# jcribeiro98/V-GAN

Hardware: AMD Instinct MI355X
Metric: V-GAN train steps/sec (batch=1024, d=784) (higher is better)
Workload: dtype f32; MMD contractions of `value`: split-bf16 x3 on the bf16 MFMA with fp32 accumulation (centred operand); the same step with the fp32 MFMA is timed in `fp32_mode`; 1 GPU; configs[2]: MNIST-pixels-as-features stand-in, d=784, batch=1024 (VGAN_no_kl step); global_batch=1024, features=784, latent=49, rows_per_gpu=1024, parallelism=dp1 (row-sharded Gram, replicated front), hip_graph=True, generator=collapsed, chain_association=depth, mmd_precision=bf16x3, gram_tile=64

## Files before the change

include/vgan_hip.h:

```cpp
#ifndef VGAN_HIP_H
#define VGAN_HIP_H

#include <stdint.h>

#ifdef __cplusplus
extern "C" {
#endif

#define VGAN_OK 0
#define VGAN_ERR_ARG 1
#define VGAN_ERR_HIP 2

#define VGAN_ABI_VERSION 11

typedef void* vgan_stream_t;

int vgan_abi_version(void);
const char* vgan_last_error(void);

int vgan_linear_forward(const float* x, int ldx, int x_nslabs, int64_t x_slab_stride, const float* W,
                        int ldw, const float* b, float* y, int ldy, int n, int in, int out,
                        vgan_stream_t stream);
int vgan_linear_backward_input(const float* dy, int lddy, const float* W, int ldw,
                               float* dx, int lddx, int n, int in, int out, vgan_stream_t stream);
int vgan_linear_backward_params(const float* dy, int lddy, const float* x, int ldx, int x_nslabs,
                                int64_t x_slab_stride, float* dW, int lddw, float* db, int n, int in,
                                int out, int splits, int64_t slab_stride, vgan_stream_t stream);
struct vgan_xx_job;
int vgan_linear_backward_params_xx_supported(int n, int in, int out);
int vgan_linear_backward_params_xx(const float* dy, int lddy, const float* x, int ldx, float* dW, int lddw, int n, int in,
                                   int out, const struct vgan_xx_job* xx, vgan_stream_t stream);
int vgan_reduce_slabs(const float* src, int64_t slab_stride, int nslabs, float* dst, int64_t count,
                      vgan_stream_t stream);

typedef struct vgan_logits_chain {
    const float* za;
    const float* At4;
    int32_t ldza, ldat, e0, pad;
} vgan_logits_chain;
int vgan_mask_project_forward(const float* logits, int ldl, const float* data, int ldd,
                              const int32_t* rows, const uint64_t* row_cursor, int row_batches,
                              int row_stride, int row_offset, float* S, float* U, float* Zx, float* Zy,
                              int ldz, float* sqx, float* sqy, int n, int d, const float* center,
                              int norm_split, const vgan_logits_chain* chain, vgan_stream_t stream);
int vgan_col_mean(const float* data, int ldd, int rows, int d, float* out, vgan_stream_t stream);
int vgan_gather_rows(const float* data, int ldd, const int32_t* rows, const uint64_t* row_cursor,
                     int row_batches, int row_stride, int row_offset, float* out, int ldo,
                     float* sq, int n, int d, vgan_stream_t stream);
int vgan_gather_rows_split(const float* data, int ldd, const int32_t* rows, const uint64_t* row_cursor,
                           int row_batches, int row_stride, int row_offset, const float* center, float* out,
                           int ldo, float* sq, int norm_split, uint16_t* Zh, uint16_t* Zl, int kp, int n, int d,
                           vgan_stream_t stream);
int vgan_mask_backward(const float* gU, int ldg, int nslabs, int64_t slab_stride, const float* S,
                       int lds, const uint64_t* colkey, float pen_weight, int row_offset,
                       float* dlogits, int ldo, int n, int d, vgan_stream_t stream);
int vgan_colmax_chunks(int n);
int vgan_colmax(const float* S, int lds, int from_softmax, int row_offset, uint64_t* part,
                uint64_t* colkey, int n, int d, vgan_stream_t stream);
int vgan_colmax_partial(const float* S, int lds, int from_softmax, int row_offset, uint64_t* part,
                        int n, int d, vgan_stream_t stream);
int vgan_mask_from_softmax(const float* S, int lds, float* U, int ldu, int n, int d, vgan_stream_t stream);
int vgan_upper_softmax_forward(const float* logits, int ldl, float* S, float* U, int n, int d,
                               vgan_stream_t stream);

#define VGAN_TILE 64
#define VGAN_TILE_INTS 8
#define VGAN_TF_SLOT_MASK 3
#define VGAN_TF_TWICE 4
#define VGAN_TF_STORE 8
#define VGAN_TF_MIRROR 16
#define VGAN_TF_NEG 32

int vgan_mmd_build_tiles(int n, int grad_mode, int rank, int world, int tile, int32_t* out, int cap);
int vgan_mmd_order_tiles(int32_t* tiles, int count, int tile);

int vgan_mmd_gram(const float* Z, int ldz, const float* sq, int n, int p, const float* bw,
                  const int32_t* tiles, int ntiles, int calibrate,
                  float* Wg, int ldw, int wrow0, float* partial, vgan_stream_t stream);
#define VGAN_RBF_MAX_KERNELS 8
int vgan_mmd_gram_general(const float* Z, int ldz, const float* sq, int n, int p, const float* bw,
                          const int32_t* tiles, int ntiles, const float* multipliers, int n_kernels,
                          float* Wg, int ldw, int wrow0, float* partial, vgan_stream_t stream);
int vgan_mmd_gram_colmax(const float* Z, int ldz, const float* sq, int n, int p, const float* bw,
                         const int32_t* tiles, int ntiles, float* Wg, int ldw, int wrow0, float* partial,
                         const float* S, int lds, int from_softmax, int row_offset, uint64_t* colpart,
                         int nrows, int d, vgan_stream_t stream);
int vgan_mmd_reduce(const float* partial, const int32_t* tiles, int ntiles, double* stats,
                    int zero_first, vgan_stream_t stream);
int vgan_mmd_set_bandwidth(const double* stats, int n, float* bw, vgan_stream_t stream);
int vgan_mmd_loss(const double* stats, const uint64_t* colkey, int n, int d, float weight,
                  float* loss, float* loss_accum, float accum_scale, uint64_t* step_counter,
                  vgan_stream_t stream);
int vgan_mmd_finalize(const float* partial, const int32_t* tiles, int ntiles, const uint64_t* colpart,
                      int chunks, uint64_t* colkey, int n, int d, float weight, double* stats,
                      float* loss, float* loss_accum, float accum_scale, uint64_t* step_counter,
                      vgan_stream_t stream);
typedef struct vgan_finalize_job {
    const float* partial;
    const int32_t* tiles;
    const uint64_t* colpart;
    uint64_t* colkey;
    double* stats;
    float* loss;
    float* loss_accum;
    uint64_t* step_counter;
    int32_t ntiles, chunks, n, d;
    float weight, accum_scale;
    int32_t mode, ntiles_main;
} vgan_finalize_job;
int vgan_mmd_backward(const float* Wg, int ldw, const float* Z, int ldz, int wrow0, int nr,
                      int ncols, int p, const float* mul, int ldmul, const float* mul_shift, float* out,
                      int ldo, int splits, int64_t slab_stride, const vgan_finalize_job* finalize,
                      vgan_stream_t stream);
int vgan_mmd_bf3_prepare(const float* Z, int ldz, int rows, int p, uint16_t* Zh, uint16_t* Zl, int kp,
                         uint16_t* ZTh, uint16_t* ZTl, int kn, vgan_stream_t stream);
int64_t vgan_mmd_gram_bf3_tail_ws_bytes(void);
int vgan_mmd_gram_bf3(const uint16_t* Zh, const uint16_t* Zl, int kp, const float* sq, int n, const float* bw,
                      const int32_t* tiles, int ntiles, int tile, uint16_t* Wh, uint16_t* Wl, int ldw,
                      int wrow0, float* partial, const float* S, int lds, int from_softmax, int row_offset,
                      uint64_t* colpart, int nrows, int d, void* tail_ws, int64_t tail_ws_bytes,
                      float* rs_part, int ldrs, vgan_stream_t stream);
int vgan_mmd_backward_bf3_tile(int nr, int p, int splits, int tile);
int vgan_mmd_backward_bf3(const uint16_t* Wh, const uint16_t* Wl, int ldw, const uint16_t* ZTh,
                          const uint16_t* ZTl, int kn, int kp, const float* Z, int ldz, int wrow0, int nr,
                          int p, const float* mul, int ldmul, const float* mul_shift, float* out, int ldo,
                          int splits, int64_t slab_stride, int tile, const vgan_finalize_job* finalize,
                          vgan_stream_t stream);
int vgan_mmd_backward_bf3_rm(const uint16_t* Wh, const uint16_t* Wl, int ldw, int kn, const uint16_t* Zh,
                             const uint16_t* Zl, int kp, int zrows, const float* Z, int ldz, int wrow0, int nr,
                             int p, const float* mul, int ldmul, const float* mul_shift, float* out, int ldo,
                             int splits, int64_t slab_stride, int tile, const vgan_finalize_job* finalize,
                             const float* rs_part, int ldrs, vgan_stream_t stream);
int vgan_mmd_backward_bf3_rm_xx(const uint16_t* Wh, const uint16_t* Wl, int ldw, int kn, const uint16_t* Zh,
                                const uint16_t* Zl, int kp, int zrows, const float* Z, int ldz, int wrow0, int nr,
                                int p, const float* mul, int ldmul, const float* mul_shift, float* out, int ldo,
                                int splits, int64_t slab_stride, const vgan_finalize_job* finalize,
                                const struct vgan_xx_job* xx, vgan_stream_t stream);
typedef struct vgan_bwd_rebuild {
    const float* data;
    const int32_t* xrow;
    const float* S;
    const float* center;
    int32_t ldd, lds;
} vgan_bwd_rebuild;
int vgan_mmd_backward_bf3_rm_rebuild(const uint16_t* Wh, const uint16_t* Wl, int ldw, int kn, const uint16_t* Zh,
                                     const uint16_t* Zl, int kp, int zrows, int nr, int p,
                                     const vgan_bwd_rebuild* rebuild, float* out, int ldo, int splits,
                                     int64_t slab_stride, const vgan_finalize_job* finalize,
                                     const struct vgan_xx_job* xx, vgan_stream_t stream);
#define VGAN_GEMM_MAX_GROUP 4
#define VGAN_GEMM_NN 0
#define VGAN_GEMM_NT 1
#define VGAN_GEMM_TN 2
#define VGAN_GEMM_NT_NT 3
typedef struct vgan_gemm_problem {
    const float* a;
    const float* b;
    float* c;
    int32_t kind, m, n, k, lda, ldb, ldc, splitk;
    const float* d;
    float* scratch;
    int32_t ldd, k2;
} vgan_gemm_problem;
int vgan_gemm_grouped(const vgan_gemm_problem* problems, int count, vgan_stream_t stream);
typedef struct vgan_adadelta_layer {
    float* w_packed;
    int64_t off_w, off_b;
    int32_t ldp, out, in, pad;
} vgan_adadelta_layer;
typedef struct vgan_grouped_extras {
    const float* copy_src;
    float* copy_dst;
    int64_t copy_count;
    int32_t adadelta, pad;
    float* p;
    float* sq_avg;
    float* acc_delta;
    float lr, rho, eps, weight_decay, grad_scale;
    int32_t ld_extra;
    vgan_adadelta_layer layer[VGAN_GEMM_MAX_GROUP + 1];
    const float* g_extra;
    float* next_noise;
    int32_t noise_rows, noise_cols, noise_ld, noise_ones_col;
    uint64_t seed;
    const uint64_t* step_counter;
    const vgan_finalize_job* fold;
} vgan_grouped_extras;
int vgan_gemm_grouped_ex(const vgan_gemm_problem* problems, int count, const vgan_grouped_extras* extras,
                         vgan_stream_t stream);

typedef struct vgan_xx_job {
    const uint16_t* Dh;
    const uint16_t* Dl;
    const float* dsq;
    const int32_t* tiles;
    const float* bw;
    float* partial;
    int32_t ldd, ntiles;
} vgan_xx_job;
int vgan_mask_project_forward_bf3(const float* logits, int ldl, const float* data, int ldd, const int32_t* rows,
                                  const uint64_t* row_cursor, int row_batches, int row_stride, float* S, float* Z,
                                  int ldz, float* sq, uint16_t* Zh, uint16_t* Zl, int kp, uint16_t* ZTh,
                                  uint16_t* ZTl, int kn, int n, int d, const float* center, int write_x,
                                  const vgan_xx_job* xx, const vgan_logits_chain* chain, vgan_stream_t stream);
int vgan_mask_project_forward_bf3_ex(const float* logits, int ldl, const float* data, int ldd, const int32_t* rows,
                                     const uint64_t* row_cursor, int row_batches, int row_stride, float* S, float* Z,
                                     int ldz, float* sq, uint16_t* Zh, uint16_t* Zl, int kp, uint16_t* ZTh,
                                     uint16_t* ZTl, int kn, int n, int d, const float* center, int write_x,
                                     const vgan_xx_job* xx, const vgan_logits_chain* chain, int write_z, int32_t* xrow,
                                     vgan_stream_t stream);
int vgan_row_sqnorm(const float* Z, int ldz, float* sq, int rows, int p, vgan_stream_t stream);

int vgan_adadelta_step(float* p, const float* g, int nslabs, int64_t slab_stride, float* sq_avg,
                       float* acc_delta, int64_t count, float lr, float rho, float eps,
                       float weight_decay, float grad_scale, vgan_stream_t stream);

int vgan_noise_normal(float* z, int rows, int cols, int ld, int ones_col, uint64_t seed,
                      const uint64_t* step_counter, uint64_t stream_id, vgan_stream_t stream);

int vgan_homogeneous_pack(const int64_t* desc, int count, int max_elems, int unpack, vgan_stream_t stream);
int vgan_adadelta_step_packed(float* p, const int32_t* pmap, const float* g_packed, float* w_packed,
                              float* sq_avg, float* acc_delta, int64_t count, float lr, float rho,
                              float eps, float weight_decay, float grad_scale, float* next_noise,
                              int noise_rows, int noise_cols, int noise_ld, int noise_ones_col,
                              uint64_t seed, const uint64_t* step_counter, vgan_stream_t stream);

int vgan_mse(const float* a, int lda, const float* b, int ldb, int n, int d, float scale,
             float* out, int accumulate, vgan_stream_t stream);

int vgan_mse_grad(const float* target, int ldt, const float* pred, int ldp, int n, int d, float gscale,
                  double* part, float* g, int ldg, vgan_stream_t stream);
int vgan_sum_f64(const double* in, int count, double scale, float* out, int accumulate, vgan_stream_t stream);

#define VGAN_DP_ID_BYTES 128
typedef struct vgan_dp_comm vgan_dp_comm;
int vgan_dp_unique_id(uint8_t* id );
int vgan_dp_comm_create(vgan_dp_comm** comm, int nranks, const uint8_t* id, int rank);
int vgan_dp_allreduce_sum(vgan_dp_comm* comm, float* buf, int64_t count, vgan_stream_t stream);
int vgan_dp_allgather(vgan_dp_comm* comm, void* buf, int64_t bytes_per_rank, vgan_stream_t stream);
int vgan_dp_comm_destroy(vgan_dp_comm* comm);

int vgan_shuffle_epoch(int32_t* perm, int64_t count, int64_t train_size, uint64_t seed, uint64_t epoch,
                       vgan_stream_t stream);
int64_t vgan_shuffle_index(int64_t i, int64_t train_size, uint64_t seed, uint64_t epoch);
int vgan_mask_unique(const uint8_t* masks, int ldm, int n, int d, uint64_t* keys, int32_t* work,
                     int32_t* out_row, int32_t* out_count, vgan_stream_t stream);

int vgan_rbf_kernel_matrix(const float* Z, int ldz, int m, int p, const float* sq, float alpha, float* K, int ldk,
                           vgan_stream_t stream);
int vgan_rbf_multi_kernel_matrix(const float* Z, int ldz, int m, int p, const float* sq, const float* bw,
                                 const float* multipliers, int n_kernels, float* K, int ldk, float* dK, int lddk,
                                 vgan_stream_t stream);
int vgan_rows_dot(const float* A, int lda, const float* B, int ldb, double* out, int rows, int cols,
                  vgan_stream_t stream);

#define VGAN_OUTLIER_MAX_K 32
#define VGAN_OUTLIER_ENGINE_EXACT 0
#define VGAN_OUTLIER_ENGINE_GRAM 1
#define VGAN_OUTLIER_KNN_LARGEST 0
#define VGAN_OUTLIER_KNN_MEAN 1
#define VGAN_OUTLIER_KNN_MEDIAN 2
#define VGAN_OUTLIER_LRD 3
#define VGAN_OUTLIER_LOF 4
#define VGAN_OUTLIER_KDE_MAX_ROWS 8388607
int vgan_outlier_pack(const float* X, int ldx, int n, int d, const float* center, const int32_t* feat,
                      const int32_t* feat_off, const int64_t* col_off, int first, int count, float* packed, float* sq,
                      vgan_stream_t stream);
int vgan_outlier_knn(const float* Pq, const float* sq_q, int nq, const float* Pr, const float* sq_r, int nr,
                     const int32_t* feat_off, const int64_t* col_off, int first, int count, int k, int exclude_self,
                     int engine, int splits, float* part_d, int32_t* part_i, int32_t* nbr, vgan_stream_t stream);
int vgan_outlier_refine(const float* Xq, int ldq, int nq, const float* Xr, int ldr, int nr, int d, const int32_t* feat,
                        const int32_t* feat_off, int first, int count, const int32_t* nbr, int k, int32_t* out_idx,
                        float* out_dist, float* kdist, vgan_stream_t stream);
int vgan_outlier_score(const int32_t* idx, const float* dist, int nq, int k, int count, int method, const float* kdist_ref,
                       const double* lrd_ref, int nr, float* score, const int32_t* score_row, int ld_score, double* lrd_out,
                       vgan_stream_t stream);
int vgan_outlier_kde(const float* Pq, const float* sq_q, int nq, const float* Pr, const float* sq_r, int nr,
                     const int32_t* feat_off, const int64_t* col_off, int first, int count, const double* bandwidth,
                     int exclude_self, int engine, int splits, uint32_t* pivot, uint64_t* acc, float* score,
                     const int32_t* score_row, int ld_score, vgan_stream_t stream);
int vgan_outlier_combine(const float* score, int ld, int S, int n, const double* weights, double* out,
                         vgan_stream_t stream);
int vgan_outlier_abod(const float* Xq, int ldq, int nq, const float* Xr, int ldr, int nr, int d, const int32_t* feat,
                      const int32_t* feat_off, int first, int count, const int32_t* idx, int k, float* score,
                      const int32_t* score_row, int ld_score, vgan_stream_t stream);
int vgan_outlier_abod_floor(float* score, int ld, int S, int n, int fit, double* score_floor, int32_t* n_degenerate,
                            vgan_stream_t stream);
#define VGAN_OUTLIER_NORM_ZSCORE 1
#define VGAN_OUTLIER_NORM_ROBUST 2
#define VGAN_OUTLIER_NORM_MINMAX 3
#define VGAN_OUTLIER_COMBINE_SUM 0
#define VGAN_OUTLIER_COMBINE_MAX 1
int64_t vgan_outlier_score_stats_ws_bytes(int S, int n, int mode);
int vgan_outlier_score_stats(const float* score, int ld, int S, int n, int mode, double* center, double* scale,
                             void* workspace, int64_t workspace_bytes, vgan_stream_t stream);
int vgan_outlier_combine_normalized(const float* score, int ld, int S, int n, const double* center, const double* scale,
                                    const double* weights, int combination, double* out, vgan_stream_t stream);

#define VGAN_CLUSTER_MAX_CLUSTERS 64
#define VGAN_CLUSTER_SLICE_ROWS 1024
int64_t vgan_cluster_lloyd_ws_bytes(int n, int n_clusters, int count, int total_dims);
int vgan_cluster_image(const double* centers, int n_clusters, const int32_t* feat, const int32_t* feat_off,
                       const int64_t* col_off, int first, int count, const float* col_center, float* img, float* img_sq,
                       vgan_stream_t stream);
int vgan_cluster_lloyd(const float* Pq, const float* sq_q, const float* X, int ldx, int n, int d, const int32_t* feat,
                       const int32_t* feat_off, const int64_t* col_off, int first, int count, int total_dims, int max_dims,
                       int n_clusters, int engine, const float* col_center, const double* tol_var, double* centers,
                       float* img, float* img_sq, int32_t* label, int32_t* changed, int32_t* done, int32_t* n_iter,
                       void* workspace, int64_t workspace_bytes, int iterations, vgan_stream_t stream);
int vgan_cluster_final(const float* Xq, int ldq, int nq, int d, const int32_t* feat, const int32_t* feat_off, int S,
                       int n_clusters, const double* centers, const int32_t* large, int64_t* sizes, int use_weights,
                       int32_t* label, double* inertia_part, double* inertia, float* score, const int32_t* score_row,
                       int ld_score, vgan_stream_t stream);

#ifdef __cplusplus
}
#endif
#endif
```

v-gan_amd/csrc/gemm_core.hpp:

```cpp
#pragma once
#include <type_traits>

#include "vgan_common.hpp"

namespace vgan {

enum : int { KC = 0, MC = 1 };

constexpr int kPad = 4;

typedef __attribute__((address_space(3))) float lds_f;
typedef __attribute__((address_space(3))) f32x4 lds_f4;

template <int BMN, int BK, int LAYOUT, int VEC, bool SL = false, int NTH = kBlock>
struct Stager;

template <int BMN, int BK, bool SL, int NTH>
struct Stager<BMN, BK, KC, 4, SL, NTH> {
    int nslabs = 1;
    long slab_stride = 0;
    static constexpr int NV = BMN * BK / 4 / NTH;
    static_assert(NV >= 1, "tile too small");
    float4 v[NV];
    const float* rowp[NV];
    int lofs[NV];
    bool rowok[NV], ok[NV];
    int kq4, K;
    __device__ __forceinline__ void init(const float* __restrict__ p, long ld, int mn0, int MN, int K_, int tid) {
        K = K_;
        kq4 = 4 * (tid % (BK / 4));
#pragma unroll
        for (int r = 0; r < NV; ++r) {
            const int m = (tid + NTH * r) / (BK / 4);
            rowok[r] = mn0 + m < MN;
            rowp[r] = p + (long)min(mn0 + m, MN - 1) * ld;
            lofs[r] = m * (BK + kPad) + kq4;
        }
    }
    __device__ __forceinline__ void load(int k0) {
        const int k = k0 + kq4;
        const int kc = min(k, K - 4);
#pragma unroll
        for (int r = 0; r < NV; ++r) {
            ok[r] = rowok[r] && (k < K);
            v[r] = *reinterpret_cast<const float4*>(rowp[r] + kc);
            if constexpr (SL)
                for (int sl = 1; sl < nslabs; ++sl) {
                    const float4 t = *reinterpret_cast<const float4*>(rowp[r] + sl * slab_stride + kc);
                    v[r].x += t.x; v[r].y += t.y; v[r].z += t.z; v[r].w += t.w;
                }
        }
    }
    __device__ __forceinline__ void store(lds_f* lds) {
#pragma unroll
        for (int r = 0; r < NV; ++r) {
            if (!ok[r]) v[r] = make_float4(0.f, 0.f, 0.f, 0.f);
            *(lds_f4*)(lds + lofs[r]) = f32x4{v[r].x, v[r].y, v[r].z, v[r].w};
        }
    }
    typedef float4 Side;
    __device__ __forceinline__ void side_add(Side (&s)[NV]) const {
#pragma unroll
        for (int r = 0; r < NV; ++r) { s[r].x += v[r].x; s[r].y += v[r].y; s[r].z += v[r].z; s[r].w += v[r].w; }
    }
    __device__ static __forceinline__ void side_reduce(const Side (&s)[NV], lds_f* , lds_f* out, int tid) {
#pragma unroll
        for (int r = 0; r < NV; ++r) {
            float t = (s[r].x + s[r].y) + (s[r].z + s[r].w);
#pragma unroll
            for (int o = 1; o < BK / 4; o <<= 1) t += __shfl_xor(t, o, 64);
            int f = tid + NTH * r;
            if (f % (BK / 4) == 0) out[f / (BK / 4)] = t;
        }
    }
};

template <int BMN, int BK, bool SL, int NTH>
struct Stager<BMN, BK, KC, 1, SL, NTH> {
    int nslabs = 1;
    long slab_stride = 0;
    static constexpr int NV = BMN * BK / NTH;
    float v[NV];
    const float* rowp[NV];
    int lofs[NV];
    bool rowok[NV], ok[NV];
    int kk, K;
    __device__ __forceinline__ void init(const float* __restrict__ p, long ld, int mn0, int MN, int K_, int tid) {
        K = K_;
        kk = tid % BK;
#pragma unroll
        for (int r = 0; r < NV; ++r) {
            const int m = (tid + NTH * r) / BK;
            rowok[r] = mn0 + m < MN;
            rowp[r] = p + (long)min(mn0 + m, MN - 1) * ld;
            lofs[r] = m * (BK + kPad) + kk;
        }
    }
    __device__ __forceinline__ void load(int k0) {
        const int k = k0 + kk;
        const int kc = min(k, K - 1);
#pragma unroll
        for (int r = 0; r < NV; ++r) {
            ok[r] = rowok[r] && (k < K);
            v[r] = rowp[r][kc];
            if constexpr (SL)
                for (int sl = 1; sl < nslabs; ++sl) v[r] += rowp[r][sl * slab_stride + kc];
        }
    }
    __device__ __forceinline__ void store(lds_f* lds) {
#pragma unroll
        for (int r = 0; r < NV; ++r) {
            if (!ok[r]) v[r] = 0.f;
            lds[lofs[r]] = v[r];
        }
    }
    typedef float Side;
    __device__ __forceinline__ void side_add(Side (&s)[NV]) const {
#pragma unroll
        for (int r = 0; r < NV; ++r) s[r] += v[r];
    }
    __device__ static __forceinline__ void side_reduce(const Side (&s)[NV], lds_f* , lds_f* out, int tid) {
#pragma unroll
        for (int r = 0; r < NV; ++r) {
            float t = s[r];
#pragma unroll
            for (int o = 1; o < BK; o <<= 1) t += __shfl_xor(t, o, 64);
            int f = tid + NTH * r;
            if (f % BK == 0) out[f / BK] = t;
        }
    }
};

template <int BMN, int BK, bool SL, int NTH>
struct Stager<BMN, BK, MC, 4, SL, NTH> {
    int nslabs = 1;
    long slab_stride = 0;
    static constexpr int NV = BMN * BK / 4 / NTH;
    static_assert(NV >= 1, "tile too small");
    static_assert(NTH % (BMN / 4) == 0, "mq must be fixed per thread");
    float4 v[NV];
    const float* colp;
    long ld;
    int krow[NV], lofs[NV];
    bool colok, ok[NV];
    int K;
    __device__ __forceinline__ void init(const float* __restrict__ p, long ld_, int mn0, int MN, int K_, int tid) {
        K = K_;
        ld = ld_;
        const int m = mn0 + 4 * (tid % (BMN / 4));
        colok = m < MN;
        colp = p + min(m, MN - 4);
#pragma unroll
        for (int r = 0; r < NV; ++r) {
            krow[r] = (tid + NTH * r) / (BMN / 4);
            lofs[r] = krow[r] * (BMN + kPad) + 4 * (tid % (BMN / 4));
        }
    }
    __device__ __forceinline__ void load(int k0) {
#pragma unroll
        for (int r = 0; r < NV; ++r) {
            const int k = k0 + krow[r];
            ok[r] = colok && (k < K);
            v[r] = *reinterpret_cast<const float4*>(colp + (long)min(k, K - 1) * ld);
            if constexpr (SL)
                for (int sl = 1; sl < nslabs; ++sl) {
                    const float4 t = *reinterpret_cast<const float4*>(colp + sl * slab_stride + (long)min(k, K - 1) * ld);
                    v[r].x += t.x; v[r].y += t.y; v[r].z += t.z; v[r].w += t.w;
                }
        }
    }
    __device__ __forceinline__ void store(lds_f* lds) {
#pragma unroll
        for (int r = 0; r < NV; ++r) {
            if (!ok[r]) v[r] = make_float4(0.f, 0.f, 0.f, 0.f);
            *(lds_f4*)(lds + lofs[r]) = f32x4{v[r].x, v[r].y, v[r].z, v[r].w};
        }
    }
    typedef float4 Side;
    __device__ __forceinline__ void side_add(Side (&s)[NV]) const {
#pragma unroll
        for (int r = 0; r < NV; ++r) { s[r].x += v[r].x; s[r].y += v[r].y; s[r].z += v[r].z; s[r].w += v[r].w; }
    }
    __device__ static __forceinline__ void side_reduce(const Side (&s)[NV], lds_f* scratch, lds_f* out, int tid) {
        constexpr int ROWS = NTH / (BMN / 4);
        float4 t = s[0];
#pragma unroll
        for (int r = 1; r < NV; ++r) { t.x += s[r].x; t.y += s[r].y; t.z += s[r].z; t.w += s[r].w; }
        *(lds_f4*)(scratch + (tid / (BMN / 4)) * BMN + 4 * (tid % (BMN / 4))) = f32x4{t.x, t.y, t.z, t.w};
        __syncthreads();
        if (tid < BMN) {
            float a = 0.f;
#pragma unroll
            for (int q = 0; q < ROWS; ++q) a += scratch[q * BMN + tid];
            out[tid] = a;
        }
    }
};

template <int BMN, int BK, bool SL, int NTH>
struct Stager<BMN, BK, MC, 1, SL, NTH> {
    int nslabs = 1;
    long slab_stride = 0;
    static constexpr int NV = BMN * BK / NTH;
    static_assert(NTH % BMN == 0, "m must be fixed per thread");
    float v[NV];
    const float* colp;
    long ld;
    int krow[NV], lofs[NV];
    bool colok, ok[NV];
    int K;
    __device__ __forceinline__ void init(const float* __restrict__ p, long ld_, int mn0, int MN, int K_, int tid) {
        K = K_;
        ld = ld_;
        const int m = mn0 + tid % BMN;
        colok = m < MN;
        colp = p + min(m, MN - 1);
#pragma unroll
        for (int r = 0; r < NV; ++r) {
            krow[r] = (tid + NTH * r) / BMN;
            lofs[r] = krow[r] * (BMN + kPad) + tid % BMN;
        }
    }
    __device__ __forceinline__ void load(int k0) {
#pragma unroll
        for (int r = 0; r < NV; ++r) {
            const int k = k0 + krow[r];
            ok[r] = colok && (k < K);
            v[r] = colp[(long)min(k, K - 1) * ld];
            if constexpr (SL)
                for (int sl = 1; sl < nslabs; ++sl) v[r] += colp[sl * slab_stride + (long)min(k, K - 1) * ld];
        }
    }
    __device__ __forceinline__ void store(lds_f* lds) {
#pragma unroll
        for (int r = 0; r < NV; ++r) {
            if (!ok[r]) v[r] = 0.f;
            lds[lofs[r]] = v[r];
        }
    }
    typedef float Side;
    __device__ __forceinline__ void side_add(Side (&s)[NV]) const {
#pragma unroll
        for (int r = 0; r < NV; ++r) s[r] += v[r];
    }
    __device__ static __forceinline__ void side_reduce(const Side (&s)[NV], lds_f* scratch, lds_f* out, int tid) {
        constexpr int ROWS = NTH / BMN;
        float t = s[0];
#pragma unroll
        for (int r = 1; r < NV; ++r) t += s[r];
        scratch[(tid / BMN) * BMN + (tid % BMN)] = t;
        __syncthreads();
        if (tid < BMN) {
            float a = 0.f;
#pragma unroll
            for (int q = 0; q < ROWS; ++q) a += scratch[q * BMN + tid];
            out[tid] = a;
        }
    }
};

template <int BM, int BN, int BK, int LA, int LB, int VEC, int SLABS = 0, int KW = 1>
struct GemmTile {
    static constexpr int NTH = kBlock * KW;
    static constexpr int WM = BM / 64, WN = BN / 64;
    static_assert(KW == 1 || (KW == 2 && BM == 64 && BN == 64 && (BK / 8) % 2 == 0), "K-split needs one sub-tile per wave");
    static constexpr int kImgA = (LA == KC) ? BM * (BK + kPad) : BK * (BM + kPad);
    static constexpr int kImgB = (LB == KC) ? BN * (BK + kPad) : BK * (BN + kPad);
    static constexpr int kLdsFloats = 2 * (kImgA + kImgB);
    static_assert(BM % 64 == 0 && BN % 64 == 0 && BK % 8 == 0, "tile shape");

    template <int LAYOUT, int BMN>
    __device__ static __forceinline__ f32x4 frag(const lds_f* img, int mn, int c, int fh) {
        if constexpr (LAYOUT == KC) {
            return *(const lds_f4*)(img + mn * (BK + kPad) + 8 * c + 4 * fh);
        } else {
            const lds_f* q = img + (8 * c + 4 * fh) * (BMN + kPad) + mn;
            return f32x4{q[0], q[BMN + kPad], q[2 * (BMN + kPad)], q[3 * (BMN + kPad)]};
        }
    }

    template <bool SIDE_A>
    __device__ static __forceinline__ void run(const float* __restrict__ A, long lda, const float* __restrict__ B, long ldb,
                                               int m0, int n0, int M, int N, int K, float* lds_generic, float* side_generic,
                                               f32x16 (&acc)[WM][WN], int nslabs = 1, long slab_stride = 0) {
        lds_f* lds = (lds_f*)lds_generic;
        lds_f* side_lds = (lds_f*)side_generic;
        const int tid = threadIdx.x;
        const int lane = tid & 63, wave = (tid >> 6) & 3, kp = tid >> 8;
        const int wm0 = (wave >> 1) * (BM / 2), wn0 = (wave & 1) * (BN / 2);
        const int fi = lane & 31, fh = lane >> 5;
        lds_f* const sA0 = lds;
        lds_f* const sB0 = lds + 2 * kImgA;
        constexpr int GC = BK / 8 / KW;

        using SG = Stager<BM, BK, LA, VEC, (SLABS & 1) != 0, NTH>;
        SG ga;
        Stager<BN, BK, LB, VEC, (SLABS & 2) != 0, NTH> gb;
        ga.init(A, lda, m0, M, K, tid);
        gb.init(B, ldb, n0, N, K, tid);
        if constexpr (SLABS & 1) { ga.nslabs = nslabs; ga.slab_stride = slab_stride; }
        if constexpr (SLABS & 2) { gb.nslabs = nslabs; gb.slab_stride = slab_stride; }
        typename SG::Side side[SG::NV];
        if constexpr (SIDE_A) {
#pragma unroll
            for (int r = 0; r < SG::NV; ++r) side[r] = typename SG::Side{};
        }

        const int nk = (K + BK - 1) / BK;
        ga.load(0);
        gb.load(0);
        ga.store(sA0);
        gb.store(sB0);
        if constexpr (SIDE_A) ga.side_add(side);
        if (nk > 1) {
            ga.load(BK);
            gb.load(BK);
        }
        __syncthreads();

        auto body = [&](int kt, auto store_next, auto load_next2) {
            const int cur = kt & 1;
            const lds_f* imgA = sA0 + cur * kImgA;
            const lds_f* imgB = sB0 + cur * kImgB;
            f32x4 a[GC][WM], b[GC][WN];
#pragma unroll
            for (int c = 0; c < GC; ++c) {
#pragma unroll
                for (int i = 0; i < WM; ++i) a[c][i] = frag<LA, BM>(imgA, wm0 + i * 32 + fi, kp * GC + c, fh);
#pragma unroll
                for (int j = 0; j < WN; ++j) b[c][j] = frag<LB, BN>(imgB, wn0 + j * 32 + fi, kp * GC + c, fh);
            }
#ifndef VGAN_ABLATE_NO_LDS_STORE
            if constexpr (decltype(store_next)::value) {
                ga.store(sA0 + (cur ^ 1) * kImgA);
                gb.store(sB0 + (cur ^ 1) * kImgB);
                if constexpr (SIDE_A) ga.side_add(side);
            }
#endif
#ifndef VGAN_ABLATE_NO_GLOBAL
            if constexpr (decltype(load_next2)::value) {
                ga.load((kt + 2) * BK);
                gb.load((kt + 2) * BK);
            }
#endif
#pragma unroll
            for (int c = 0; c < GC; ++c)
#pragma unroll
                for (int st = 0; st < 4; ++st)
#pragma unroll
                    for (int i = 0; i < WM; ++i)
#pragma unroll
                        for (int j = 0; j < WN; ++j)
#ifndef VGAN_ABLATE_NO_MFMA
                            acc[i][j] = __builtin_amdgcn_mfma_f32_32x32x2f32(a[c][i][st], b[c][j][st], acc[i][j], 0, 0, 0);
#else
                            acc[i][j][st] += a[c][i][st] * b[c][j][st];
#endif
#if !defined(VGAN_SCHED_NONE)
            __builtin_amdgcn_iglp_opt(0);
#endif
#ifndef VGAN_ABLATE_NO_BARRIER
            __syncthreads();
#endif
        };
        using T = std::true_type;
        using F = std::false_type;
        int kt = 0;
        for (; kt + 2 < nk; ++kt) body(kt, T{}, T{});
        if (kt + 1 < nk) {
            body(kt, T{}, F{});
            ++kt;
        }
        body(kt, F{}, F{});

        if constexpr (SIDE_A) {
            SG::side_reduce(side, lds, side_lds, tid);
            __syncthreads();
        }
        if constexpr (KW == 2) {
            lds_f* xch = lds;
#pragma unroll
            for (int r = 0; r < 8; ++r) xch[((kp * 4 + wave) * 8 + r) * 64 + lane] = acc[0][0][8 * (1 - kp) + r];
            __syncthreads();
#pragma unroll
            for (int r = 0; r < 8; ++r) acc[0][0][8 * kp + r] += xch[(((1 - kp) * 4 + wave) * 8 + r) * 64 + lane];
            __syncthreads();
        }
    }
    __device__ static __forceinline__ int first_reg() { return KW == 2 ? 8 * (threadIdx.x >> 8) : 0; }
    static constexpr int kNumRegs = 16 / KW;

    __device__ static __forceinline__ int sub_row(int wm, int r) {
        const int lane = threadIdx.x & 63, wave = (threadIdx.x >> 6) & 3;
        return (wave >> 1) * (BM / 2) + wm * 32 + (r & 3) + 8 * (r >> 2) + 4 * (lane >> 5);
    }
    __device__ static __forceinline__ int sub_col(int wn) {
        const int lane = threadIdx.x & 63, wave = (threadIdx.x >> 6) & 3;
        return (wave & 1) * (BN / 2) + wn * 32 + (lane & 31);
    }
};


template <int BK, int LA, int LB, int VEC, int NW = 4>
struct GemmTileKS {
    static constexpr int T = 32;
    static constexpr int NTH = 64 * NW;
    static constexpr int NR = 16 / NW;
    static constexpr int kImgA = (LA == KC) ? T * (BK + kPad) : BK * (T + kPad);
    static constexpr int kImgB = (LB == KC) ? T * (BK + kPad) : BK * (T + kPad);
    static constexpr int kLdsFloats = 2 * (kImgA + kImgB);
    static constexpr int GW = BK / (8 * NW);
    static_assert(GW >= 1 && BK % (8 * NW) == 0 && kLdsFloats >= NW * 16 * 64, "K tile / reduction scratch");

    template <int LAYOUT>
    __device__ static __forceinline__ f32x4 frag(const lds_f* img, int mn, int c, int fh) {
        if constexpr (LAYOUT == KC) {
            return *(const lds_f4*)(img + mn * (BK + kPad) + 8 * c + 4 * fh);
        } else {
            const lds_f* q = img + (8 * c + 4 * fh) * (T + kPad) + mn;
            return f32x4{q[0], q[T + kPad], q[2 * (T + kPad)], q[3 * (T + kPad)]};
        }
    }

    __device__ static __forceinline__ void run(const float* __restrict__ A, long lda, const float* __restrict__ B, long ldb, int m0,
                                               int n0, int M, int N, int K, float* lds_generic, float (&out)[NR]) {
        lds_f* lds = (lds_f*)lds_generic;
        const int tid = threadIdx.x, lane = tid & 63, wave = tid >> 6;
        const int fi = lane & 31, fh = lane >> 5;
        lds_f* const sA0 = lds;
        lds_f* const sB0 = lds + 2 * kImgA;
        f32x16 acc;
#pragma unroll
        for (int r = 0; r < 16; ++r) acc[r] = 0.f;
        const int nk = (K + BK - 1) / BK;
        Stager<T, BK, LA, VEC, false, NTH> ga;
        Stager<T, BK, LB, VEC, false, NTH> gb;
        ga.init(A, lda, m0, M, K, tid);
        gb.init(B, ldb, n0, N, K, tid);
        ga.load(0);
        gb.load(0);
        ga.store(sA0);
        gb.store(sB0);
        if (nk > 1) {
            ga.load(BK);
            gb.load(BK);
        }
        __syncthreads();
        auto body = [&](int kt, auto store_next, auto load_next2) {
            const int cur = kt & 1;
            const lds_f* imgA = sA0 + cur * kImgA;
            const lds_f* imgB = sB0 + cur * kImgB;
            f32x4 a[GW], b[GW];
#pragma unroll
            for (int c = 0; c < GW; ++c) {
                a[c] = frag<LA>(imgA, fi, wave * GW + c, fh);
                b[c] = frag<LB>(imgB, fi, wave * GW + c, fh);
            }
            if constexpr (decltype(store_next)::value) {
                ga.store(sA0 + (cur ^ 1) * kImgA);
                gb.store(sB0 + (cur ^ 1) * kImgB);
            }
            if constexpr (decltype(load_next2)::value) {
                ga.load((kt + 2) * BK);
                gb.load((kt + 2) * BK);
            }
#pragma unroll
            for (int c = 0; c < GW; ++c)
#pragma unroll
                for (int st = 0; st < 4; ++st) acc = __builtin_amdgcn_mfma_f32_32x32x2f32(a[c][st], b[c][st], acc, 0, 0, 0);
            __builtin_amdgcn_iglp_opt(0);
            __syncthreads();
        };
        using Tt = std::true_type;
        using Ff = std::false_type;
        int kt = 0;
        for (; kt + 2 < nk; ++kt) body(kt, Tt{}, Tt{});
        if (kt + 1 < nk) {
            body(kt, Tt{}, Ff{});
            ++kt;
        }
        body(kt, Ff{}, Ff{});
#pragma unroll
        for (int r = 0; r < 16; ++r) lds[(wave * 16 + r) * 64 + lane] = acc[r];
        __syncthreads();
#pragma unroll
        for (int rr = 0; rr < NR; ++rr) {
            const int r = NR * wave + rr;
            if constexpr (NW == 4) {
                out[rr] = (lds[(0 * 16 + r) * 64 + lane] + lds[(1 * 16 + r) * 64 + lane]) +
                          (lds[(2 * 16 + r) * 64 + lane] + lds[(3 * 16 + r) * 64 + lane]);
            } else {
                float q[NW / 4];
#pragma unroll
                for (int w4 = 0; w4 < NW / 4; ++w4)
                    q[w4] = (lds[((4 * w4 + 0) * 16 + r) * 64 + lane] + lds[((4 * w4 + 1) * 16 + r) * 64 + lane]) +
                            (lds[((4 * w4 + 2) * 16 + r) * 64 + lane] + lds[((4 * w4 + 3) * 16 + r) * 64 + lane]);
                float t = q[0];
#pragma unroll
                for (int w4 = 1; w4 < NW / 4; ++w4) t += q[w4];
                out[rr] = t;
            }
        }
    }
    __device__ static __forceinline__ int row_of(int rr) {
        const int lane = threadIdx.x & 63, r = NR * (threadIdx.x >> 6) + rr;
        return (r & 3) + 8 * (r >> 2) + 4 * (lane >> 5);
    }
    __device__ static __forceinline__ int col_of() { return threadIdx.x & 31; }
};

template <int WM, int WN>
__device__ __forceinline__ void zero_acc(f32x16 (&acc)[WM][WN]) {
#pragma unroll
    for (int i = 0; i < WM; ++i)
#pragma unroll
        for (int j = 0; j < WN; ++j)
#pragma unroll
            for (int r = 0; r < 16; ++r) acc[i][j][r] = 0.f;
}

}
```

v-gan_amd/csrc/grouped.hip:

```cpp
#include "gemm_core.hpp"
#include "mmd_common.hpp"
#include "optim_common.hpp"

namespace vgan {

constexpr int QBM = 64, QBK = 32, QKS = 128;

struct GroupedArgs {
    vgan_gemm_problem p[VGAN_GEMM_MAX_GROUP];
    int tile_start[VGAN_GEMM_MAX_GROUP + 1];
    int ks[VGAN_GEMM_MAX_GROUP];
    int split[VGAN_GEMM_MAX_GROUP];
    int kchunk[VGAN_GEMM_MAX_GROUP];
    int count;
};

__device__ __forceinline__ vgan_gemm_problem k_slice(vgan_gemm_problem q, int slice, int kchunk) {
    const int k0 = slice * kchunk;
    q.c += (long)slice * q.m * q.ldc;
    if (q.kind == VGAN_GEMM_NN) { q.a += k0; q.b += (long)k0 * q.ldb; }
    else if (q.kind == VGAN_GEMM_NT) { q.a += k0; q.b += k0; }
    else { q.a += (long)k0 * q.lda; q.b += (long)k0 * q.ldb; }
    q.k = min(kchunk, q.k - k0);
    return q;
}

struct GroupedExtras {
    const float* copy_src;
    float* copy_dst;
    long copy_count;
    int copy_blocks, extra_blocks, noise_blocks, adadelta;
    float *p, *sq, *acc;
    float lr, rho, eps, wd, gs;
    vgan_adadelta_layer layer[VGAN_GEMM_MAX_GROUP + 1];
    const float* g_extra;
    int ld_extra;
    float* z;
    int zrows, zcols, zld, zones;
    unsigned long long seed;
    const unsigned long long* step_counter;
    int fold_blocks;
    vgan_finalize_job fold;
};

__device__ __forceinline__ void adadelta_packed_element(const GroupedExtras& x, const vgan_adadelta_layer& L, int row, int col, float g) {
    if (row >= L.out || col > L.in) return;
    const long idx = col < L.in ? L.off_w + (long)row * L.in + col : L.off_b + row;
    float pv = x.p[idx], v = x.sq[idx], a = x.acc[idx];
    adadelta_one(pv, g, v, a, x.lr, x.rho, x.eps, x.wd, x.gs);
    x.p[idx] = pv;
    x.sq[idx] = v;
    x.acc[idx] = a;
    L.w_packed[(long)row * L.ldp + col] = pv;
}

template <int NE>
struct AdadeltaTile {
    long idx[NE];
    float pv[NE], v[NE], a[NE];
    bool ok[NE];
    template <typename RowOf>
    __device__ __forceinline__ void prefetch(const GroupedExtras& x, const vgan_adadelta_layer& L, int col, RowOf row_of) {
#pragma unroll
        for (int r = 0; r < NE; ++r) {
            const int row = row_of(r);
            ok[r] = row < L.out && col <= L.in;
            idx[r] = ok[r] ? (col < L.in ? L.off_w + (long)row * L.in + col : L.off_b + row) : L.off_w;
            pv[r] = x.p[idx[r]];
            v[r] = x.sq[idx[r]];
            a[r] = x.acc[idx[r]];
        }
    }
    template <typename RowOf>
    __device__ __forceinline__ void finish(const GroupedExtras& x, const vgan_adadelta_layer& L, int col, const float (&g)[NE], RowOf row_of) {
#pragma unroll
        for (int r = 0; r < NE; ++r) adadelta_one(pv[r], g[r], v[r], a[r], x.lr, x.rho, x.eps, x.wd, x.gs);
#pragma unroll
        for (int r = 0; r < NE; ++r)
            if (ok[r]) {
                x.p[idx[r]] = pv[r];
                x.sq[idx[r]] = v[r];
                x.acc[idx[r]] = a[r];
                L.w_packed[(long)row_of(r) * L.ldp + col] = pv[r];
            }
    }
};

__device__ __forceinline__ void grouped_extra_jobs(const GroupedExtras& x, int b, int layer_index) {
    if (b < x.copy_blocks) {
        for (long i = (long)b * blockDim.x + threadIdx.x; i < x.copy_count; i += (long)x.copy_blocks * blockDim.x) x.copy_dst[i] = x.copy_src[i];
        return;
    }
    b -= x.copy_blocks;
    if (b < x.extra_blocks) {
        const vgan_adadelta_layer& L = x.layer[layer_index];
        const long total = (long)L.out * (L.in + 1);
        for (long i = (long)b * blockDim.x + threadIdx.x; i < total; i += (long)x.extra_blocks * blockDim.x) {
            const int row = (int)(i / (L.in + 1)), col = (int)(i % (L.in + 1));
            adadelta_packed_element(x, L, row, col, x.g_extra[(long)row * x.ld_extra + col]);
        }
        return;
    }
    b -= x.extra_blocks;
    if (b < x.noise_blocks) {
        noise_normal_body(x.z, x.zrows, x.zcols, x.zld, x.zones, x.seed, x.step_counter, 0ull, b, x.noise_blocks);
        return;
    }
    b -= x.noise_blocks;
    if (b < x.fold_blocks) finalize_body(x.fold);
}

template <int LA, int LB, int VEC, bool EPI>
__device__ __forceinline__ void tile64(const vgan_gemm_problem& q, int t, float* lds, const GroupedExtras& x, int qi) {
    using G = GemmTile<QBM, QBM, QBK, LA, LB, VEC>;
    const int gx = (q.n + QBM - 1) / QBM;
    const int m0 = (t / gx) * QBM, n0 = (t % gx) * QBM;
    const int col = n0 + G::sub_col(0);
    auto row_of = [&](int r) { return m0 + G::sub_row(0, r); };
    AdadeltaTile<EPI ? 16 : 1> upd;
    if constexpr (EPI) upd.prefetch(x, x.layer[qi], col, row_of);
    f32x16 acc[1][1];
    zero_acc(acc);
    G::template run<false>(q.a, q.lda, q.b, q.ldb, m0, n0, q.m, q.n, q.k, lds, nullptr, acc);
#pragma unroll
    for (int r = 0; r < 16; ++r) {
        const int row = m0 + G::sub_row(0, r);
        if (row < q.m && col < q.n) q.c[(long)row * q.ldc + col] = acc[0][0][r];
    }
    if constexpr (EPI) {
        float g[16];
#pragma unroll
        for (int r = 0; r < 16; ++r) g[r] = acc[0][0][r];
        upd.finish(x, x.layer[qi], col, g, row_of);
    }
}

template <int LA, int LB, int VEC, int NW = 4, bool EPI = false>
__device__ __forceinline__ void tile_ks(const vgan_gemm_problem& q, int t, float* lds, const GroupedExtras& x, int qi) {
    using G = GemmTileKS<QKS, LA, LB, VEC, NW>;
    const int gx = (q.n + 31) / 32;
    const int m0 = (t / gx) * 32, n0 = (t % gx) * 32;
    const int col = n0 + G::col_of();
    auto row_of = [&](int rr) { return m0 + G::row_of(rr); };
    AdadeltaTile<EPI ? G::NR : 1> upd;
    if constexpr (EPI) upd.prefetch(x, x.layer[qi], col, row_of);
    float o[G::NR];
    G::run(q.a, q.lda, q.b, q.ldb, m0, n0, q.m, q.n, q.k, lds, o);
#pragma unroll
    for (int rr = 0; rr < G::NR; ++rr) {
        const int row = m0 + G::row_of(rr);
        if (row < q.m && col < q.n) q.c[(long)row * q.ldc + col] = o[rr];
    }
    if constexpr (EPI) upd.finish(x, x.layer[qi], col, o, row_of);
}

template <int VEC>
__device__ __forceinline__ void tile64_two_stage(const vgan_gemm_problem& q, int t, float* lds) {
    using G = GemmTile<QBM, QBM, QBK, KC, KC, VEC>;
    const int gx = (q.n + QBM - 1) / QBM;
    const int m0 = (t / gx) * QBM, n0 = (t % gx) * QBM;
    const int ldh = (q.k2 + 3) / 4 * 4;
    float* H = q.scratch + (long)t * QBM * ldh;
    const int rows = min(QBM, q.m - m0);
    for (int c0 = 0; c0 < q.k2; c0 += QBM) {
        f32x16 acc[1][1];
        zero_acc(acc);
        G::template run<false>(q.a, q.lda, q.b, q.ldb, m0, c0, q.m, q.k2, q.k, lds, nullptr, acc);
        const int col = c0 + G::sub_col(0);
#pragma unroll
        for (int r = 0; r < 16; ++r) {
            const int row = G::sub_row(0, r);
            if (row < rows && col < ldh) H[(long)row * ldh + col] = col < q.k2 ? acc[0][0][r] : 0.f;
        }
    }
    __syncthreads();
    f32x16 acc[1][1];
    zero_acc(acc);
    G::template run<false>(H, ldh, q.d, q.ldd, 0, n0, rows, q.n, q.k2, lds, nullptr, acc);
    const int col = n0 + G::sub_col(0);
#pragma unroll
    for (int r = 0; r < 16; ++r) {
        const int row = m0 + G::sub_row(0, r);
        if (row < q.m && col < q.n) q.c[(long)row * q.ldc + col] = acc[0][0][r];
    }
}

constexpr int cmax(int a, int b) { return a > b ? a : b; }

template <int VEC, bool EPI>
__global__ __launch_bounds__(kBlock, 2) void gemm_grouped_kernel(GroupedArgs g, GroupedExtras x) {
    constexpr int kLds = cmax(cmax(GemmTile<QBM, QBM, QBK, KC, MC, VEC>::kLdsFloats, GemmTile<QBM, QBM, QBK, MC, MC, VEC>::kLdsFloats),
                              cmax(cmax(GemmTileKS<QKS, KC, MC, VEC>::kLdsFloats, GemmTileKS<QKS, MC, MC, VEC>::kLdsFloats),
                                   cmax(GemmTile<QBM, QBM, QBK, KC, KC, VEC>::kLdsFloats, GemmTileKS<QKS, KC, KC, VEC>::kLdsFloats)));
    __shared__ __attribute__((aligned(16))) float lds[kLds];
    if ((int)blockIdx.x >= g.tile_start[VGAN_GEMM_MAX_GROUP]) {
        grouped_extra_jobs(x, blockIdx.x - g.tile_start[VGAN_GEMM_MAX_GROUP], g.count);
        return;
    }
    int qi = 0;
#pragma unroll
    for (int i = 1; i < VGAN_GEMM_MAX_GROUP; ++i)
        if (i < g.count && (int)blockIdx.x >= g.tile_start[i]) qi = i;
    vgan_gemm_problem q = g.p[qi];
    int t = blockIdx.x - g.tile_start[qi];
    if (g.split[qi] > 1) {
        const int per = (g.tile_start[qi + 1] - g.tile_start[qi]) / g.split[qi];
        q = k_slice(q, t / per, g.kchunk[qi]);
        t %= per;
    }
    if (q.kind == VGAN_GEMM_NN) {
        if (g.ks[qi]) tile_ks<KC, MC, VEC, 4, EPI>(q, t, lds, x, qi); else tile64<KC, MC, VEC, EPI>(q, t, lds, x, qi);
    } else if (q.kind == VGAN_GEMM_NT) {
        if (g.ks[qi]) tile_ks<KC, KC, VEC, 4, EPI>(q, t, lds, x, qi); else tile64<KC, KC, VEC, EPI>(q, t, lds, x, qi);
    } else if (q.kind == VGAN_GEMM_NT_NT) {
        tile64_two_stage<VEC>(q, t, lds);
    } else {
        if (g.ks[qi]) tile_ks<MC, MC, VEC, 4, EPI>(q, t, lds, x, qi); else tile64<MC, MC, VEC, EPI>(q, t, lds, x, qi);
    }
}

__global__ __launch_bounds__(1024, 1) void gemm_grouped_ks16_kernel(GroupedArgs g, GroupedExtras x) {
    constexpr int kLds = cmax(cmax(GemmTileKS<QKS, KC, MC, 4, 16>::kLdsFloats, GemmTileKS<QKS, MC, MC, 4, 16>::kLdsFloats),
                              GemmTileKS<QKS, KC, KC, 4, 16>::kLdsFloats);
    __shared__ __attribute__((aligned(16))) float lds[kLds];
    if ((int)blockIdx.x >= g.tile_start[VGAN_GEMM_MAX_GROUP]) {
        grouped_extra_jobs(x, blockIdx.x - g.tile_start[VGAN_GEMM_MAX_GROUP], g.count);
        return;
    }
    int qi = 0;
#pragma unroll
    for (int i = 1; i < VGAN_GEMM_MAX_GROUP; ++i)
        if (i < g.count && (int)blockIdx.x >= g.tile_start[i]) qi = i;
    const vgan_gemm_problem& q = g.p[qi];
    const int t = blockIdx.x - g.tile_start[qi];
    if (q.kind == VGAN_GEMM_NN) tile_ks<KC, MC, 4, 16>(q, t, lds, x, qi);
    else if (q.kind == VGAN_GEMM_NT) tile_ks<KC, KC, 4, 16>(q, t, lds, x, qi);
    else tile_ks<MC, MC, 4, 16>(q, t, lds, x, qi);
}

}

using namespace vgan;

static inline int extra_grid(long work_items) {
    long g = (work_items + kBlock - 1) / kBlock;
    return (int)(g < 1 ? 1 : (g > 256 ? 256 : g));
}

extern "C" int vgan_gemm_grouped_ex(const vgan_gemm_problem* problems, int count, const vgan_grouped_extras* extras,
                                    vgan_stream_t stream) {
    VGAN_CHECK_ARG(problems && count >= 1 && count <= VGAN_GEMM_MAX_GROUP);
    GroupedArgs g{};
    GroupedExtras x{};
    g.count = count;
    bool vec = true, any_split = false;
    int tiles = 0;
    for (int i = 0; i < count; ++i) {
        const vgan_gemm_problem& q = problems[i];
        VGAN_CHECK_ARG(q.a && q.b && q.c && q.m > 0 && q.n > 0 && q.k > 0 && q.ldc >= q.n);
        VGAN_CHECK_ARG(q.kind == VGAN_GEMM_NN || q.kind == VGAN_GEMM_NT || q.kind == VGAN_GEMM_TN || q.kind == VGAN_GEMM_NT_NT);
        const bool two = q.kind == VGAN_GEMM_NT_NT;
        VGAN_CHECK_ARG(q.lda >= (q.kind == VGAN_GEMM_TN ? q.m : q.k) && q.ldb >= ((q.kind == VGAN_GEMM_NT || two) ? q.k : q.n));
        if (two) {
            VGAN_CHECK_ARG(q.d && q.scratch && q.k2 > 0 && q.ldd >= q.k2 && q.splitk <= 1 && aligned16(q.scratch));
            vec = vec && (q.k2 % 4 == 0) && (q.ldd % 4 == 0) && aligned16(q.d);
            any_split = true;
        }
        vec = vec && (q.m % 4 == 0) && (q.n % 4 == 0) && (q.k % 4 == 0) && (q.lda % 4 == 0) && (q.ldb % 4 == 0) && aligned16(q.a) &&
              aligned16(q.b);
        const long t64 = (long)((q.m + 63) / 64) * ((q.n + 63) / 64);
        const long t32 = (long)((q.m + 31) / 32) * ((q.n + 31) / 32);
        g.ks[i] = (q.k >= 128 && t32 <= 512 && !two) ? 1 : 0;
        g.p[i] = q;
        g.tile_start[i] = tiles;
        g.split[i] = q.splitk > 1 ? q.splitk : 1;
        if (g.split[i] > 1) {
            g.kchunk[i] = ((q.k + g.split[i] - 1) / g.split[i] + QBK - 1) / QBK * QBK;
            VGAN_CHECK_ARG(g.split[i] <= 64 && (long)(g.split[i] - 1) * g.kchunk[i] < q.k);
            g.ks[i] = 0;
            any_split = true;
        }
        tiles += g.ks[i] ? ((q.m + 31) / 32) * ((q.n + 31) / 32) : (int)t64 * g.split[i];
    }
    for (int i = count; i <= VGAN_GEMM_MAX_GROUP; ++i) g.tile_start[i] = tiles;
    bool epi = false;
    if (extras != nullptr) {
        const vgan_grouped_extras& e = *extras;
        if (e.copy_src != nullptr) {
            VGAN_CHECK_ARG(e.copy_dst && e.copy_count > 0);
            x.copy_src = e.copy_src;
            x.copy_dst = e.copy_dst;
            x.copy_count = (long)e.copy_count;
            x.copy_blocks = extra_grid(e.copy_count);
        }
        if (e.adadelta) {
            VGAN_CHECK_ARG(e.p && e.sq_avg && e.acc_delta && !any_split);
            epi = true;
            x.adadelta = 1;
            x.p = e.p; x.sq = e.sq_avg; x.acc = e.acc_delta;
            x.lr = e.lr; x.rho = e.rho; x.eps = e.eps; x.wd = e.weight_decay; x.gs = e.grad_scale;
            const int nl = count + (e.g_extra != nullptr ? 1 : 0);
            for (int i = 0; i < nl; ++i) {
                const vgan_adadelta_layer& L = e.layer[i];
                VGAN_CHECK_ARG(L.w_packed && L.out > 0 && L.in > 0 && L.ldp >= L.in + 1 && L.off_w >= 0 && L.off_b >= 0);
                if (i < count) VGAN_CHECK_ARG(problems[i].m >= L.out && problems[i].n >= L.in + 1);
                x.layer[i] = L;
            }
            if (e.g_extra != nullptr) {
                VGAN_CHECK_ARG(e.ld_extra >= e.layer[count].in + 1);
                x.g_extra = e.g_extra;
                x.ld_extra = e.ld_extra;
                x.extra_blocks = extra_grid((long)e.layer[count].out * (e.layer[count].in + 1));
            }
        }
        if (e.next_noise != nullptr) {
            VGAN_CHECK_ARG(e.noise_rows > 0 && e.noise_cols > 0 && e.noise_ld >= e.noise_cols && e.noise_ones_col < e.noise_ld);
            x.z = e.next_noise;
            x.zrows = e.noise_rows; x.zcols = e.noise_cols; x.zld = e.noise_ld; x.zones = e.noise_ones_col;
            x.seed = (unsigned long long)e.seed;
            x.step_counter = reinterpret_cast<const unsigned long long*>(e.step_counter);
            x.noise_blocks = extra_grid(((long)e.noise_rows * e.noise_cols + 3) / 4);
        }
        if (e.fold != nullptr) {
            VGAN_CHECK_ARG(finalize_job_ok(*e.fold));
            x.fold = *e.fold;
            x.fold_blocks = 1;
        }
    }
    const int surplus = x.copy_blocks + x.extra_blocks + x.noise_blocks + x.fold_blocks;
    int kmin = problems[0].k, t32 = 0;
    for (int i = 0; i < count; ++i) {
        kmin = problems[i].k < kmin ? problems[i].k : kmin;
        t32 += ((problems[i].m + 31) / 32) * ((problems[i].n + 31) / 32);
    }
    if (vec && kmin >= 96 && t32 <= 256 && !epi && x.noise_blocks == 0 && !any_split) {
        int acc = 0;
        for (int i = 0; i < count; ++i) {
            g.ks[i] = 1;
            g.tile_start[i] = acc;
            acc += ((problems[i].m + 31) / 32) * ((problems[i].n + 31) / 32);
        }
        for (int i = count; i <= VGAN_GEMM_MAX_GROUP; ++i) g.tile_start[i] = acc;
        hipLaunchKernelGGL(gemm_grouped_ks16_kernel, dim3(acc + surplus), dim3(1024), 0, (hipStream_t)stream, g, x);
        VGAN_CHECK_LAUNCH();
        return VGAN_OK;
    }
    const dim3 grid(tiles + surplus), block(kBlock);
    hipStream_t st = (hipStream_t)stream;
    if (vec && epi) hipLaunchKernelGGL((gemm_grouped_kernel<4, true>), grid, block, 0, st, g, x);
    else if (vec) hipLaunchKernelGGL((gemm_grouped_kernel<4, false>), grid, block, 0, st, g, x);
    else if (epi) hipLaunchKernelGGL((gemm_grouped_kernel<1, true>), grid, block, 0, st, g, x);
    else hipLaunchKernelGGL((gemm_grouped_kernel<1, false>), grid, block, 0, st, g, x);
    VGAN_CHECK_LAUNCH();
    return VGAN_OK;
}

extern "C" int vgan_gemm_grouped(const vgan_gemm_problem* problems, int count, vgan_stream_t stream) {
    return vgan_gemm_grouped_ex(problems, count, nullptr, stream);
}
```

v-gan_amd/csrc/linear.hip:

```cpp
#include "gemm_core.hpp"
#include "mmd_xx.hpp"

namespace vgan {

constexpr int LBM = 64, LBN = 64, LBK = 32;

template <int VEC, bool XSL>
__global__ __launch_bounds__(kBlock, 2) void linear_fwd_kernel(const float* __restrict__ x, int ldx, const float* __restrict__ W,
                                                              int ldw, const float* __restrict__ b, float* __restrict__ y,
                                                              int ldy, int n, int in, int out, int x_nslabs, long x_slab_stride) {
    using G = GemmTile<LBM, LBN, LBK, KC, KC, VEC, XSL ? 1 : 0>;
    __shared__ __attribute__((aligned(16))) float lds[G::kLdsFloats];
    const int m0 = blockIdx.y * LBM, n0 = blockIdx.x * LBN;
    const int col = n0 + G::sub_col(0);
    const float bias = (b != nullptr) ? b[min(col, out - 1)] : 0.f;
    f32x16 acc[G::WM][G::WN];
    zero_acc(acc);
    G::template run<false>(x, ldx, W, ldw, m0, n0, n, out, in, lds, nullptr, acc, x_nslabs, x_slab_stride);
#pragma unroll
    for (int r = 0; r < 16; ++r) {
        const int row = m0 + G::sub_row(0, r);
        if (row < n && col < out) y[(long)row * ldy + col] = acc[0][0][r] + bias;
    }
}

template <int VEC>
__global__ __launch_bounds__(kBlock, 2) void linear_bwd_input_kernel(const float* __restrict__ dy, int lddy,
                                                                    const float* __restrict__ W, int ldw, float* __restrict__ dx,
                                                                    int lddx, int n, int in, int out) {
    using G = GemmTile<LBM, LBN, LBK, KC, MC, VEC>;
    __shared__ __attribute__((aligned(16))) float lds[G::kLdsFloats];
    const int m0 = blockIdx.y * LBM, n0 = blockIdx.x * LBN;
    f32x16 acc[G::WM][G::WN];
    zero_acc(acc);
    G::template run<false>(dy, lddy, W, ldw, m0, n0, n, in, out, lds, nullptr, acc);
    const int col = n0 + G::sub_col(0);
#pragma unroll
    for (int r = 0; r < 16; ++r) {
        const int row = m0 + G::sub_row(0, r);
        if (row < n && col < in) dx[(long)row * lddx + col] = acc[0][0][r];
    }
}

template <int VEC, bool XSL>
__global__ __launch_bounds__(kBlock, 2) void linear_bwd_params_kernel(const float* __restrict__ dy, int lddy,
                                                                     const float* __restrict__ x, int ldx, float* __restrict__ dW,
                                                                     int lddw, float* __restrict__ db, int n, int in, int out,
                                                                     int kchunk, long slab_stride, int x_nslabs, long x_slab_stride) {
    using G = GemmTile<LBM, LBN, LBK, MC, MC, VEC, XSL ? 2 : 0>;
    __shared__ __attribute__((aligned(16))) float lds[G::kLdsFloats];
    __shared__ float side[LBM];
    const int m0 = blockIdx.y * LBM, n0 = blockIdx.x * LBN;
    const int k0 = blockIdx.z * kchunk;
    const int klen = min(kchunk, n - k0);
    dy += (long)k0 * lddy;
    x += (long)k0 * ldx;
    dW += blockIdx.z * slab_stride;
    if (db != nullptr) db += blockIdx.z * slab_stride;
    n = klen;
    f32x16 acc[G::WM][G::WN];
    zero_acc(acc);
    const bool do_bias = (db != nullptr) && (blockIdx.x == 0);
    if (klen <= 0) {
        if (threadIdx.x < LBM) side[threadIdx.x] = 0.f;
        __syncthreads();
    } else if (do_bias)
        G::template run<true>(dy, lddy, x, ldx, m0, n0, out, in, n, lds, side, acc, x_nslabs, x_slab_stride);
    else
        G::template run<false>(dy, lddy, x, ldx, m0, n0, out, in, n, lds, side, acc, x_nslabs, x_slab_stride);
    const int col = n0 + G::sub_col(0);
#pragma unroll
    for (int r = 0; r < 16; ++r) {
        const int row = m0 + G::sub_row(0, r);
        if (row < out && col < in) dW[(long)row * lddw + col] = acc[0][0][r];
    }
    if (do_bias && threadIdx.x < LBM && m0 + threadIdx.x < out) db[m0 + threadIdx.x] = side[threadIdx.x];
}

constexpr int KSBK = 128;
template <int VEC, int NW>
__global__ __launch_bounds__(64 * NW, NW == 4 ? 2 : 1) void linear_fwd_ks_kernel(const float* __restrict__ x, int ldx,
                                                                               const float* __restrict__ W, int ldw,
                                                                               const float* __restrict__ b, float* __restrict__ y,
                                                                               int ldy, int n, int in, int out) {
    using G = GemmTileKS<KSBK, KC, KC, VEC, NW>;
    __shared__ __attribute__((aligned(16))) float lds[G::kLdsFloats];
    const int m0 = blockIdx.y * 32, n0 = blockIdx.x * 32;
    const int col = n0 + G::col_of();
    const float bias = (b != nullptr) ? b[min(col, out - 1)] : 0.f;
    float o[G::NR];
    G::run(x, ldx, W, ldw, m0, n0, n, out, in, lds, o);
#pragma unroll
    for (int rr = 0; rr < G::NR; ++rr) {
        const int row = m0 + G::row_of(rr);
        if (row < n && col < out) y[(long)row * ldy + col] = o[rr] + bias;
    }
}
template <int VEC>
__global__ __launch_bounds__(kBlock, 2) void linear_bwd_input_ks_kernel(const float* __restrict__ dy, int lddy,
                                                                       const float* __restrict__ W, int ldw, float* __restrict__ dx,
                                                                       int lddx, int n, int in, int out, int in_staged) {
    using G = GemmTileKS<KSBK, KC, MC, VEC>;
    __shared__ __attribute__((aligned(16))) float lds[G::kLdsFloats];
    const int m0 = blockIdx.y * 32, n0 = blockIdx.x * 32;
    float o[G::NR];
    G::run(dy, lddy, W, ldw, m0, n0, n, in_staged, out, lds, o);
    const int col = n0 + G::col_of();
#pragma unroll
    for (int rr = 0; rr < G::NR; ++rr) {
        const int row = m0 + G::row_of(rr);
        if (row < n && col < in) dx[(long)row * lddx + col] = o[rr];
    }
}
template <int VEC, int NW>
__global__ __launch_bounds__(64 * NW, NW == 4 ? 2 : 1) void linear_bwd_params_ks_kernel(const float* __restrict__ dy, int lddy,
                                                                                      const float* __restrict__ x, int ldx,
                                                                                      float* __restrict__ dW, int lddw, int n, int in,
                                                                                      int out) {
    using G = GemmTileKS<KSBK, MC, MC, VEC, NW>;
    __shared__ __attribute__((aligned(16))) float lds[G::kLdsFloats];
    const int m0 = blockIdx.y * 32, n0 = blockIdx.x * 32;
    float o[G::NR];
    G::run(dy, lddy, x, ldx, m0, n0, out, in, n, lds, o);
    const int col = n0 + G::col_of();
#pragma unroll
    for (int rr = 0; rr < G::NR; ++rr) {
        const int row = m0 + G::row_of(rr);
        if (row < out && col < in) dW[(long)row * lddw + col] = o[rr];
    }
}
__global__ __launch_bounds__(1024, 1) void linear_bwd_params_ks_xx_kernel(const float* __restrict__ dy, int lddy, const float* __restrict__ x,
                                                                         int ldx, float* __restrict__ dW, int lddw, int n, int in, int out,
                                                                         int gx, int ptiles, XXJob xx) {
    using G = GemmTileKS<KSBK, MC, MC, 4, 16>;
    constexpr int kBytes = G::kLdsFloats * 4 > GemmBF3<64>::kLdsBytes ? G::kLdsFloats * 4 : GemmBF3<64>::kLdsBytes;
    __shared__ __attribute__((aligned(16))) char raw[kBytes];
    __shared__ float xx_red[4];
    if ((int)blockIdx.x >= ptiles) {
        xx_tile_body(xx, blockIdx.x - ptiles, raw, xx_red);
        return;
    }
    float* lds = reinterpret_cast<float*>(raw);
    const int m0 = (blockIdx.x / gx) * 32, n0 = (blockIdx.x % gx) * 32;
    float o[G::NR];
    G::run(dy, lddy, x, ldx, m0, n0, out, in, n, lds, o);
    const int col = n0 + G::col_of();
#pragma unroll
    for (int rr = 0; rr < G::NR; ++rr) {
        const int row = m0 + G::row_of(rr);
        if (row < out && col < in) dW[(long)row * lddw + col] = o[rr];
    }
}

static inline bool use_ks(int rows, int cols, int k) {
    const long tiles64 = (long)((rows + 63) / 64) * ((cols + 63) / 64);
    return tiles64 <= 32 && k >= 128;
}

static inline bool use_ks_params(int rows, int cols, int k) {
    const long tiles64 = (long)((rows + 63) / 64) * ((cols + 63) / 64);
    return use_ks(rows, cols, k) || (tiles64 <= 512 && k >= 2048);
}

static inline dim3 grid_for(int rows, int cols) { return dim3((cols + LBN - 1) / LBN, (rows + LBM - 1) / LBM, 1); }

}

using namespace vgan;

extern "C" int vgan_linear_forward(const float* x, int ldx, int x_nslabs, int64_t x_slab_stride, const float* W, int ldw,
                                   const float* b, float* y, int ldy, int n, int in, int out, vgan_stream_t stream) {
    VGAN_CHECK_ARG(x && W && y && n > 0 && in > 0 && out > 0 && ldx >= in && ldw >= in && ldy >= out && x_nslabs >= 1);
    hipStream_t s = (hipStream_t)stream;
    const bool vec = (in % 4 == 0) && (ldx % 4 == 0) && (ldw % 4 == 0) && aligned16(x) && aligned16(W) && (x_slab_stride % 4 == 0);
    const long xs = (long)x_slab_stride;
    if (x_nslabs == 1 && use_ks(n, out, in)) {
        dim3 g((out + 31) / 32, (n + 31) / 32);
        if (vec && in >= 512)
            hipLaunchKernelGGL((linear_fwd_ks_kernel<4, 16>), g, dim3(1024), 0, s, x, ldx, W, ldw, b, y, ldy, n, in, out);
        else if (vec)
            hipLaunchKernelGGL((linear_fwd_ks_kernel<4, 4>), g, dim3(kBlock), 0, s, x, ldx, W, ldw, b, y, ldy, n, in, out);
        else
            hipLaunchKernelGGL((linear_fwd_ks_kernel<1, 4>), g, dim3(kBlock), 0, s, x, ldx, W, ldw, b, y, ldy, n, in, out);
        VGAN_CHECK_LAUNCH();
        return VGAN_OK;
    }
#define VGAN_FWD(V, S) hipLaunchKernelGGL((linear_fwd_kernel<V, S>), grid_for(n, out), dim3(kBlock), 0, s, x, ldx, W, ldw, b, y, ldy, n, in, out, x_nslabs, xs)
    if (x_nslabs > 1) { if (vec) VGAN_FWD(4, true); else VGAN_FWD(1, true); }
    else { if (vec) VGAN_FWD(4, false); else VGAN_FWD(1, false); }
#undef VGAN_FWD
    VGAN_CHECK_LAUNCH();
    return VGAN_OK;
}

extern "C" int vgan_linear_backward_input(const float* dy, int lddy, const float* W, int ldw, float* dx, int lddx, int n, int in,
                                          int out, vgan_stream_t stream) {
    VGAN_CHECK_ARG(dy && W && dx && n > 0 && in > 0 && out > 0 && lddy >= out && ldw >= in && lddx >= in);
    hipStream_t s = (hipStream_t)stream;
    const bool vec_but_in = (out % 4 == 0) && (lddy % 4 == 0) && (ldw % 4 == 0) && aligned16(dy) && aligned16(W);
    const bool vec = vec_but_in && (in % 4 == 0);
    if (use_ks(n, in, out)) {
        dim3 g((in + 31) / 32, (n + 31) / 32);
        const int in4 = (in + 3) / 4 * 4;
        if (vec_but_in && ldw >= in4)
            hipLaunchKernelGGL(linear_bwd_input_ks_kernel<4>, g, dim3(kBlock), 0, s, dy, lddy, W, ldw, dx, lddx, n, in, out, in4);
        else
            hipLaunchKernelGGL(linear_bwd_input_ks_kernel<1>, g, dim3(kBlock), 0, s, dy, lddy, W, ldw, dx, lddx, n, in, out, in);
    } else if (vec)
        hipLaunchKernelGGL(linear_bwd_input_kernel<4>, grid_for(n, in), dim3(kBlock), 0, s, dy, lddy, W, ldw, dx, lddx, n, in, out);
    else
        hipLaunchKernelGGL(linear_bwd_input_kernel<1>, grid_for(n, in), dim3(kBlock), 0, s, dy, lddy, W, ldw, dx, lddx, n, in, out);
    VGAN_CHECK_LAUNCH();
    return VGAN_OK;
}

extern "C" int vgan_linear_backward_params(const float* dy, int lddy, const float* x, int ldx, int x_nslabs, int64_t x_slab_stride,
                                           float* dW, int lddw, float* db, int n, int in, int out, int splits, int64_t slab_stride,
                                           vgan_stream_t stream) {
    VGAN_CHECK_ARG(dy && x && dW && n > 0 && in > 0 && out > 0 && lddy >= out && ldx >= in && lddw >= in && x_nslabs >= 1);
    VGAN_CHECK_ARG(splits >= 1 && splits <= 64 && (splits == 1 || slab_stride > 0));
    hipStream_t s = (hipStream_t)stream;
    int kchunk = (n + splits - 1) / splits;
    kchunk = (kchunk + 3) / 4 * 4;
    const int nz = (n + kchunk - 1) / kchunk;
    const bool vec = (out % 4 == 0) && (lddy % 4 == 0) && (in % 4 == 0) && (ldx % 4 == 0) && aligned16(dy) && aligned16(x) &&
                     (x_slab_stride % 4 == 0);
    dim3 grid = grid_for(out, in);
    grid.z = splits;
    (void)nz;
    const long xs = (long)x_slab_stride;
    if (splits == 1 && x_nslabs == 1 && db == nullptr && use_ks_params(out, in, n)) {
        dim3 g((in + 31) / 32, (out + 31) / 32);
        if (vec && n >= 256)
            hipLaunchKernelGGL((linear_bwd_params_ks_kernel<4, 16>), g, dim3(1024), 0, s, dy, lddy, x, ldx, dW, lddw, n, in, out);
        else if (vec)
            hipLaunchKernelGGL((linear_bwd_params_ks_kernel<4, 4>), g, dim3(kBlock), 0, s, dy, lddy, x, ldx, dW, lddw, n, in, out);
        else
            hipLaunchKernelGGL((linear_bwd_params_ks_kernel<1, 4>), g, dim3(kBlock), 0, s, dy, lddy, x, ldx, dW, lddw, n, in, out);
        VGAN_CHECK_LAUNCH();
        return VGAN_OK;
    }
#define VGAN_BWP(V, S) hipLaunchKernelGGL((linear_bwd_params_kernel<V, S>), grid, dim3(kBlock), 0, s, dy, lddy, x, ldx, dW, lddw, db, n, in, out, kchunk, (long)slab_stride, x_nslabs, xs)
    if (x_nslabs > 1) { if (vec) VGAN_BWP(4, true); else VGAN_BWP(1, true); }
    else { if (vec) VGAN_BWP(4, false); else VGAN_BWP(1, false); }
#undef VGAN_BWP
    VGAN_CHECK_LAUNCH();
    return VGAN_OK;
}

extern "C" int vgan_linear_backward_params_xx_supported(int n, int in, int out) {
    return (n >= 256 && in > 0 && out > 0 && in % 4 == 0 && out % 4 == 0 && use_ks(out, in, n)) ? 1 : 0;
}

extern "C" int vgan_linear_backward_params_xx(const float* dy, int lddy, const float* x, int ldx, float* dW, int lddw, int n, int in,
                                              int out, const vgan_xx_job* xxjob, vgan_stream_t stream) {
    VGAN_CHECK_ARG(dy && x && dW && xxjob && n > 0 && in > 0 && out > 0 && lddy >= out && ldx >= in && lddw >= in);
    const vgan_xx_job& j = *xxjob;
    VGAN_CHECK_ARG(j.Dh && j.Dl && j.dsq && j.tiles && j.bw && j.partial && j.ntiles > 0 && j.ldd % 64 == 0 && aligned16(j.Dh) && aligned16(j.Dl) &&
                   (reinterpret_cast<uintptr_t>(j.partial) & 15) == 0);
    VGAN_CHECK_ARG((out % 4 == 0) && (lddy % 4 == 0) && (in % 4 == 0) && (ldx % 4 == 0) && aligned16(dy) && aligned16(x) && n >= 256 &&
                   use_ks(out, in, n));
    const int gx = (in + 31) / 32, gy = (out + 31) / 32;
    const XXJob xx{j.Dh, j.Dl, j.dsq, nullptr, nullptr, reinterpret_cast<const TileDesc*>(j.tiles), j.bw, j.partial, j.ldd, 1, 0, j.ntiles, 0};
    hipLaunchKernelGGL(linear_bwd_params_ks_xx_kernel, dim3(gx * gy + j.ntiles), dim3(1024), 0, (hipStream_t)stream, dy, lddy, x, ldx, dW, lddw, n,
                       in, out, gx, gx * gy, xx);
    VGAN_CHECK_LAUNCH();
    return VGAN_OK;
}
```

v-gan_amd/lib.py:

```python
import ctypes
import os

_HERE = os.path.dirname(os.path.abspath(__file__))
LIB_PATH = os.path.join(_HERE, "libvgan_hip.so")

_p = ctypes.c_void_p
_i = ctypes.c_int
_f = ctypes.c_float
_i64 = ctypes.c_int64
_u64 = ctypes.c_uint64

class FinalizeJob(ctypes.Structure):
    _fields_ = [("partial", _p), ("tiles", _p), ("colpart", _p), ("colkey", _p), ("stats", _p), ("loss", _p), ("loss_accum", _p),
                ("step_counter", _p), ("ntiles", ctypes.c_int32), ("chunks", ctypes.c_int32), ("n", ctypes.c_int32),
                ("d", ctypes.c_int32), ("weight", _f), ("accum_scale", _f), ("mode", ctypes.c_int32), ("ntiles_main", ctypes.c_int32)]


class GemmProblem(ctypes.Structure):
    _fields_ = [("a", _p), ("b", _p), ("c", _p), ("kind", ctypes.c_int32), ("m", ctypes.c_int32), ("n", ctypes.c_int32),
                ("k", ctypes.c_int32), ("lda", ctypes.c_int32), ("ldb", ctypes.c_int32), ("ldc", ctypes.c_int32), ("splitk", ctypes.c_int32),
                ("d", _p), ("scratch", _p), ("ldd", ctypes.c_int32), ("k2", ctypes.c_int32)]


class LogitsChain(ctypes.Structure):
    _fields_ = [("za", _p), ("At4", _p), ("ldza", ctypes.c_int32), ("ldat", ctypes.c_int32), ("e0", ctypes.c_int32), ("pad", ctypes.c_int32)]


class XXJob(ctypes.Structure):
    _fields_ = [("Dh", _p), ("Dl", _p), ("dsq", _p), ("tiles", _p), ("bw", _p), ("partial", _p), ("ldd", ctypes.c_int32),
                ("ntiles", ctypes.c_int32)]


class BwdRebuild(ctypes.Structure):
    _fields_ = [("data", _p), ("xrow", _p), ("S", _p), ("center", _p), ("ldd", ctypes.c_int32), ("lds", ctypes.c_int32)]


class AdadeltaLayer(ctypes.Structure):
    _fields_ = [("w_packed", _p), ("off_w", _i64), ("off_b", _i64), ("ldp", ctypes.c_int32), ("out", ctypes.c_int32),
                ("inp", ctypes.c_int32), ("pad", ctypes.c_int32)]


class GroupedExtras(ctypes.Structure):
    _fields_ = [("copy_src", _p), ("copy_dst", _p), ("copy_count", _i64), ("adadelta", ctypes.c_int32), ("pad", ctypes.c_int32),
                ("p", _p), ("sq_avg", _p), ("acc_delta", _p), ("lr", _f), ("rho", _f), ("eps", _f), ("weight_decay", _f),
                ("grad_scale", _f), ("ld_extra", ctypes.c_int32), ("layer", AdadeltaLayer * 5), ("g_extra", _p), ("next_noise", _p),
                ("noise_rows", ctypes.c_int32), ("noise_cols", ctypes.c_int32), ("noise_ld", ctypes.c_int32),
                ("noise_ones_col", ctypes.c_int32), ("seed", _u64), ("step_counter", _p), ("fold", _p)]


GEMM_NN, GEMM_NT, GEMM_TN, GEMM_NT_NT = 0, 1, 2, 3
GEMM_MAX_GROUP = 4

SIGNATURES = {
    "vgan_abi_version": (_i, []),
    "vgan_last_error": (ctypes.c_char_p, []),
    "vgan_linear_forward": (_i, [_p, _i, _i, _i64, _p, _i, _p, _p, _i, _i, _i, _i, _p]),
    "vgan_linear_backward_input": (_i, [_p, _i, _p, _i, _p, _i, _i, _i, _i, _p]),
    "vgan_linear_backward_params": (_i, [_p, _i, _p, _i, _i, _i64, _p, _i, _p, _i, _i, _i, _i, _i64, _p]),
    "vgan_linear_backward_params_xx_supported": (_i, [_i, _i, _i]),
    "vgan_linear_backward_params_xx": (_i, [_p, _i, _p, _i, _p, _i, _i, _i, _i, _p, _p]),
    "vgan_reduce_slabs": (_i, [_p, _i64, _i, _p, _i64, _p]),
    "vgan_mask_project_forward": (_i, [_p, _i, _p, _i, _p, _p, _i, _i, _i, _p, _p, _p, _p, _i, _p, _p, _i, _i, _p, _i, _p, _p]),
    "vgan_col_mean": (_i, [_p, _i, _i, _i, _p, _p]),
    "vgan_gather_rows": (_i, [_p, _i, _p, _p, _i, _i, _i, _p, _i, _p, _i, _i, _p]),
    "vgan_gather_rows_split": (_i, [_p, _i, _p, _p, _i, _i, _i, _p, _p, _i, _p, _i, _p, _p, _i, _i, _i, _p]),
    "vgan_mask_backward": (_i, [_p, _i, _i, _i64, _p, _i, _p, _f, _i, _p, _i, _i, _i, _p]),
    "vgan_colmax_partial": (_i, [_p, _i, _i, _i, _p, _i, _i, _p]),
    "vgan_mmd_finalize": (_i, [_p, _p, _i, _p, _i, _p, _i, _i, _f, _p, _p, _p, _f, _p, _p]),
    "vgan_colmax_chunks": (_i, [_i]),
    "vgan_colmax": (_i, [_p, _i, _i, _i, _p, _p, _i, _i, _p]),
    "vgan_mask_from_softmax": (_i, [_p, _i, _p, _i, _i, _i, _p]),
    "vgan_upper_softmax_forward": (_i, [_p, _i, _p, _p, _i, _i, _p]),
    "vgan_mmd_build_tiles": (_i, [_i, _i, _i, _i, _i, _p, _i]),
    "vgan_mmd_order_tiles": (_i, [_p, _i, _i]),
    "vgan_mmd_gram": (_i, [_p, _i, _p, _i, _i, _p, _p, _i, _i, _p, _i, _i, _p, _p]),
    "vgan_mmd_gram_general": (_i, [_p, _i, _p, _i, _i, _p, _p, _i, _p, _i, _p, _i, _i, _p, _p]),
    "vgan_mmd_gram_colmax": (_i, [_p, _i, _p, _i, _i, _p, _p, _i, _p, _i, _i, _p, _p, _i, _i, _i, _p, _i, _i, _p]),
    "vgan_mmd_reduce": (_i, [_p, _p, _i, _p, _i, _p]),
    "vgan_mmd_set_bandwidth": (_i, [_p, _i, _p, _p]),
    "vgan_mmd_loss": (_i, [_p, _p, _i, _i, _f, _p, _p, _f, _p, _p]),
    "vgan_mmd_backward": (_i, [_p, _i, _p, _i, _i, _i, _i, _i, _p, _i, _p, _p, _i, _i, _i64, _p, _p]),
    "vgan_mmd_bf3_prepare": (_i, [_p, _i, _i, _i, _p, _p, _i, _p, _p, _i, _p]),
    "vgan_mmd_gram_bf3": (_i, [_p, _p, _i, _p, _i, _p, _p, _i, _i, _p, _p, _i, _i, _p, _p, _i, _i, _i, _p, _i, _i, _p, _i64, _p, _i, _p]),
    "vgan_mmd_gram_bf3_tail_ws_bytes": (_i64, []),
    "vgan_mmd_backward_bf3": (_i, [_p, _p, _i, _p, _p, _i, _i, _p, _i, _i, _i, _i, _p, _i, _p, _p, _i, _i, _i64, _i, _p, _p]),
    "vgan_mmd_backward_bf3_tile": (_i, [_i, _i, _i, _i]),
    "vgan_mmd_backward_bf3_rm": (_i, [_p, _p, _i, _i, _p, _p, _i, _i, _p, _i, _i, _i, _i, _p, _i, _p, _p, _i, _i, _i64, _i, _p, _p, _i, _p]),
    "vgan_mmd_backward_bf3_rm_xx": (_i, [_p, _p, _i, _i, _p, _p, _i, _i, _p, _i, _i, _i, _i, _p, _i, _p, _p, _i, _i, _i64, _p, _p, _p]),
    "vgan_mmd_backward_bf3_rm_rebuild": (_i, [_p, _p, _i, _i, _p, _p, _i, _i, _i, _i, _p, _p, _i, _i, _i64, _p, _p, _p]),
    "vgan_row_sqnorm": (_i, [_p, _i, _p, _i, _i, _p]),
    "vgan_adadelta_step": (_i, [_p, _p, _i, _i64, _p, _p, _i64, _f, _f, _f, _f, _f, _p]),
    "vgan_noise_normal": (_i, [_p, _i, _i, _i, _i, _u64, _p, _u64, _p]),
    "vgan_homogeneous_pack": (_i, [_p, _i, _i, _i, _p]),
    "vgan_adadelta_step_packed": (_i, [_p, _p, _p, _p, _p, _p, _i64, _f, _f, _f, _f, _f, _p, _i, _i, _i, _i, _u64, _p, _p]),
    "vgan_gemm_grouped": (_i, [_p, _i, _p]),
    "vgan_gemm_grouped_ex": (_i, [_p, _i, _p, _p]),
    "vgan_mask_project_forward_bf3": (_i, [_p, _i, _p, _i, _p, _p, _i, _i, _p, _p, _i, _p, _p, _p, _i, _p, _p, _i, _i, _i, _p, _i, _p, _p, _p]),
    "vgan_mask_project_forward_bf3_ex": (_i, [_p, _i, _p, _i, _p, _p, _i, _i, _p, _p, _i, _p, _p, _p, _i, _p, _p, _i, _i, _i, _p, _i, _p, _p, _i, _p,
                                              _p]),
    "vgan_mse_grad": (_i, [_p, _i, _p, _i, _i, _i, _f, _p, _p, _i, _p]),
    "vgan_sum_f64": (_i, [_p, _i, ctypes.c_double, _p, _i, _p]),
    "vgan_rbf_kernel_matrix": (_i, [_p, _i, _i, _i, _p, _f, _p, _i, _p]),
    "vgan_rbf_multi_kernel_matrix": (_i, [_p, _i, _i, _i, _p, _p, _p, _i, _p, _i, _p, _i, _p]),
    "vgan_rows_dot": (_i, [_p, _i, _p, _i, _p, _i, _i, _p]),
    "vgan_shuffle_epoch": (_i, [_p, _i64, _i64, _u64, _u64, _p]),
    "vgan_shuffle_index": (_i64, [_i64, _i64, _u64, _u64]),
    "vgan_mask_unique": (_i, [_p, _i, _i, _i, _p, _p, _p, _p, _p]),
    "vgan_dp_unique_id": (_i, [_p]),
    "vgan_dp_comm_create": (_i, [_p, _i, _p, _i]),
    "vgan_dp_allreduce_sum": (_i, [_p, _p, _i64, _p]),
    "vgan_dp_allgather": (_i, [_p, _p, _i64, _p]),
    "vgan_dp_comm_destroy": (_i, [_p]),
    "vgan_mse": (_i, [_p, _i, _p, _i, _i, _i, _f, _p, _i, _p]),
    "vgan_outlier_pack": (_i, [_p, _i, _i, _i, _p, _p, _p, _p, _i, _i, _p, _p, _p]),
    "vgan_outlier_knn": (_i, [_p, _p, _i, _p, _p, _i, _p, _p, _i, _i, _i, _i, _i, _i, _p, _p, _p, _p]),
    "vgan_outlier_refine": (_i, [_p, _i, _i, _p, _i, _i, _i, _p, _p, _i, _i, _p, _i, _p, _p, _p, _p]),
    "vgan_outlier_score": (_i, [_p, _p, _i, _i, _i, _i, _p, _p, _i, _p, _p, _i, _p, _p]),
    "vgan_outlier_kde": (_i, [_p, _p, _i, _p, _p, _i, _p, _p, _i, _i, _p, _i, _i, _i, _p, _p, _p, _p, _i, _p]),
    "vgan_outlier_combine": (_i, [_p, _i, _i, _i, _p, _p, _p]),
    "vgan_outlier_abod": (_i, [_p, _i, _i, _p, _i, _i, _i, _p, _p, _i, _i, _p, _i, _p, _p, _i, _p]),
    "vgan_outlier_abod_floor": (_i, [_p, _i, _i, _i, _i, _p, _p, _p]),
    "vgan_outlier_score_stats_ws_bytes": (_i64, [_i, _i, _i]),
    "vgan_outlier_score_stats": (_i, [_p, _i, _i, _i, _i, _p, _p, _p, _i64, _p]),
    "vgan_outlier_combine_normalized": (_i, [_p, _i, _i, _i, _p, _p, _p, _i, _p, _p]),
    "vgan_cluster_lloyd_ws_bytes": (_i64, [_i, _i, _i, _i]),
    "vgan_cluster_image": (_i, [_p, _i, _p, _p, _p, _i, _i, _p, _p, _p, _p]),
    "vgan_cluster_lloyd": (_i, [_p, _p, _p, _i, _i, _i, _p, _p, _p, _i, _i, _i, _i, _i, _i, _p, _p, _p, _p, _p, _p, _p, _p, _p,
                                _p, _i64, _i, _p]),
    "vgan_cluster_final": (_i, [_p, _i, _i, _i, _p, _p, _i, _i, _p, _p, _p, _i, _p, _p, _p, _p, _p, _i, _p]),
}

ABI_VERSION = 11
_lib = None


class VganHipError(RuntimeError):
    pass


def load():
    global _lib
    if _lib is not None:
        return _lib
    if not os.path.exists(LIB_PATH):
        raise VganHipError(
            f"{LIB_PATH} is missing: build it with `python -c 'import __graft_entry__ as g; g.build()'` "
            "(or `make -C v-gan_amd/csrc`).  vgan_amd has no CPU fallback.")
    lib = ctypes.CDLL(LIB_PATH)
    for name, (res, args) in SIGNATURES.items():
        fn = getattr(lib, name)
        fn.restype = res
        fn.argtypes = args
    if lib.vgan_abi_version() != ABI_VERSION:
        raise VganHipError(f"ABI mismatch: library {lib.vgan_abi_version()} vs binding {ABI_VERSION}")
    _lib = lib
    return lib


def check(rc, what=""):
    if rc != 0:
        msg = load().vgan_last_error().decode(errors="replace")
        raise VganHipError(f"{what} failed (code {rc}): {msg}")


def build_tiles(n, grad_mode, rank=0, world=1, tile=64):
    lib = load()
    cnt = lib.vgan_mmd_build_tiles(n, grad_mode, rank, world, tile, None, 0)
    if cnt < 0:
        raise VganHipError("vgan_mmd_build_tiles: " + lib.vgan_last_error().decode())
    buf = (ctypes.c_int32 * (cnt * 8))()
    got = lib.vgan_mmd_build_tiles(n, grad_mode, rank, world, tile, ctypes.cast(buf, ctypes.c_void_p), cnt)
    if got != cnt:
        raise VganHipError("vgan_mmd_build_tiles: inconsistent tile count")
    return list(buf), cnt


def split_tiles(table, tile=64, yy_last=False):
    import torch
    lib = load()
    slot = table[:, 4] & 3
    first = (slot != 2) if yy_last else (slot != 0)
    parts = []
    for keep in (first, ~first):
        sub = table[keep].contiguous()
        if sub.shape[0] > 1:
            buf = (ctypes.c_int32 * sub.numel())(*sub.reshape(-1).tolist())
            if lib.vgan_mmd_order_tiles(ctypes.cast(buf, ctypes.c_void_p), sub.shape[0], tile) != 0:
                raise VganHipError("vgan_mmd_order_tiles: " + lib.vgan_last_error().decode())
            sub = torch.tensor(list(buf), dtype=torch.int32).view(-1, 8)
        parts.append(sub)
    return parts
```

v-gan_amd/ops.py:

```python
import ctypes

import torch

from . import lib as _lib

_f32 = torch.float32


def _round4(v):
    return (int(v) + 3) // 4 * 4


def _ptr(t):
    return ctypes.c_void_p(t.data_ptr()) if t is not None else None


def _mat(t, name):
    if not (t.is_cuda and t.dtype == _f32 and t.dim() == 2 and t.stride(1) == 1):
        raise ValueError(f"{name}: need a float32 HIP matrix with unit inner stride, got "
                         f"{t.dtype} {tuple(t.shape)} strides {t.stride()} on {t.device}")
    return t


def _vec(t, name, dtype=_f32):
    if not (t.is_cuda and t.dtype == dtype and t.is_contiguous()):
        raise ValueError(f"{name}: need a contiguous {dtype} HIP tensor, got {t.dtype} on {t.device}")
    return t


class HipOps:

    name = "hip"

    def __init__(self):
        self.lib = _lib.load()
        if not torch.cuda.is_available():
            raise _lib.VganHipError("vgan_amd needs a HIP device (torch.cuda.is_available() is False); "
                                    "there is no CPU fallback")

    @staticmethod
    def _stream():
        return ctypes.c_void_p(torch.cuda.current_stream().cuda_stream)

    def build_tiles(self, n, grad_mode, rank=0, world=1, device=None, tile=64, split_xx=False, split=None):
        flat, cnt = _lib.build_tiles(n, grad_mode, rank, world, tile)
        table = torch.tensor(flat, dtype=torch.int32).view(cnt, 8)
        if split_xx or split:
            first, second = _lib.split_tiles(table, tile, yy_last=(split == "yy_last"))
            return torch.cat([first, second]).to(device or "cuda"), first.shape[0]
        return table.to(device or "cuda")

    def colmax_chunks(self, n):
        return self.lib.vgan_colmax_chunks(n)

    def linear_forward(self, x, W, b, y, x_nslabs=1, x_slab_stride=0):
        _mat(x, "x"), _mat(W, "W"), _mat(y, "y")
        n, kin = x.shape
        out = W.shape[0]
        assert W.shape[1] == kin and y.shape == (n, out)
        _lib.check(self.lib.vgan_linear_forward(_ptr(x), x.stride(0), int(x_nslabs), int(x_slab_stride), _ptr(W), W.stride(0),
                                                _ptr(b), _ptr(y), y.stride(0), n, kin, out, self._stream()), "vgan_linear_forward")

    def linear_backward_input(self, dy, W, dx):
        _mat(dy, "dy"), _mat(W, "W"), _mat(dx, "dx")
        n, out = dy.shape
        kin = W.shape[1]
        assert W.shape[0] == out and dx.shape == (n, kin)
        _lib.check(self.lib.vgan_linear_backward_input(_ptr(dy), dy.stride(0), _ptr(W), W.stride(0), _ptr(dx), dx.stride(0),
                                                       n, kin, out, self._stream()), "vgan_linear_backward_input")

    def linear_backward_params(self, dy, x, dW, db, splits=1, slab_stride=0, x_nslabs=1, x_slab_stride=0):
        _mat(dy, "dy"), _mat(x, "x"), _mat(dW, "dW")
        n, out = dy.shape
        kin = x.shape[1]
        assert x.shape[0] == n and dW.shape == (out, kin)
        _lib.check(self.lib.vgan_linear_backward_params(_ptr(dy), dy.stride(0), _ptr(x), x.stride(0), int(x_nslabs), int(x_slab_stride),
                                                        _ptr(dW), dW.stride(0), _ptr(db), n, kin, out, int(splits), int(slab_stride),
                                                        self._stream()), "vgan_linear_backward_params")

    def linear_backward_params_xx_supported(self, n, kin, out):
        return bool(self.lib.vgan_linear_backward_params_xx_supported(int(n), int(kin), int(out)))

    def linear_backward_params_xx(self, dy, x, dW, xx):
        _mat(dy, "dy"), _mat(x, "x"), _mat(dW, "dW")
        n, out = dy.shape
        kin = x.shape[1]
        assert x.shape[0] == n and dW.shape == (out, kin)
        _lib.check(self.lib.vgan_linear_backward_params_xx(_ptr(dy), dy.stride(0), _ptr(x), x.stride(0), _ptr(dW), dW.stride(0), n, kin, out,
                                                           ctypes.byref(xx), self._stream()), "vgan_linear_backward_params_xx")

    def reduce_slabs(self, src, slab_stride, nslabs, dst):
        _vec(dst, "dst")
        _lib.check(self.lib.vgan_reduce_slabs(_ptr(src), int(slab_stride), int(nslabs), _ptr(dst), dst.numel(), self._stream()),
                   "vgan_reduce_slabs")

    def col_mean(self, data, out):
        _mat(data, "data"), _vec(out, "out")
        rows, d = data.shape
        assert out.numel() >= d
        _lib.check(self.lib.vgan_col_mean(_ptr(data), data.stride(0), rows, d, _ptr(out), self._stream()), "vgan_col_mean")

    @staticmethod
    def logits_chain(za, At4):
        _mat(za, "za"), _mat(At4, "At4")
        assert za.shape[1] == At4.shape[1]
        return _lib.LogitsChain(_ptr(za), _ptr(At4), za.stride(0), At4.stride(0), za.shape[1], 0)

    @staticmethod
    def chain_fusable(n, d, *lds):
        return d % 4 == 0 and d <= 1024 and all(int(v) % 4 == 0 for v in lds)

    def mask_project_forward(self, logits, data, rows, S, U, Zx, Zy, sqx, sqy, row_cursor=None, row_batches=1, row_stride=0,
                             row_offset=0, center=None, norm_split=False, chain=None):
        _mat(data, "data"), _mat(Zy, "Zy"), _mat(S, "S")
        n, d = S.shape
        if logits is not None:
            _mat(logits, "logits")
            assert tuple(logits.shape) == (n, d)
        assert S.is_contiguous() and S.shape == (n, d) and (U is None or (U.is_contiguous() and U.shape == (n, d)))
        assert Zx is None or Zx.stride(0) == Zy.stride(0)
        if rows is not None:
            _vec(rows, "rows", torch.int32)
        _lib.check(self.lib.vgan_mask_project_forward(_ptr(logits), logits.stride(0) if logits is not None else 0, _ptr(data), data.stride(0), _ptr(rows),
                                                      _ptr(row_cursor), int(row_batches), int(row_stride), int(row_offset), _ptr(S), _ptr(U), _ptr(Zx), _ptr(Zy), Zy.stride(0), _ptr(sqx), _ptr(sqy),
                                                      n, d, _ptr(center), int(bool(norm_split)),
                                                      ctypes.byref(chain) if chain is not None else None, self._stream()), "vgan_mask_project_forward")

    bf3_rebuild = True

    def xx_job(self, Dh, Dl, dsq, tiles, bw, partial):
        assert tiles.is_contiguous() and partial.is_contiguous() and Dh.stride(0) == Dl.stride(0)
        return _lib.XXJob(_ptr(Dh), _ptr(Dl), _ptr(dsq), _ptr(tiles), _ptr(bw), _ptr(partial), Dh.stride(0), tiles.shape[0])

    def bwd_rebuild(self, data, xrow, S, center):
        _mat(data, "data"), _mat(S, "S")
        assert xrow.dtype == torch.int32 and xrow.is_contiguous() and center.is_contiguous()
        return _lib.BwdRebuild(_ptr(data), _ptr(xrow), _ptr(S), _ptr(center), data.stride(0), S.stride(0))

    def mask_project_forward_bf3(self, logits, data, rows, S, Z, sq, Zh, Zl, ZTh, ZTl, row_cursor=None, row_batches=1, row_stride=0,
                                 center=None, write_x=True, xx=None, chain=None, write_z=True, xrow=None):
        _mat(data, "data"), _mat(Z, "Z"), _mat(S, "S")
        n, d = S.shape
        if logits is not None:
            _mat(logits, "logits")
        if not write_z or xrow is not None:
            _lib.check(self.lib.vgan_mask_project_forward_bf3_ex(_ptr(logits), logits.stride(0) if logits is not None else 0, _ptr(data),
                                                                 data.stride(0), _ptr(rows), _ptr(row_cursor), int(row_batches),
                                                                 int(row_stride), _ptr(S), _ptr(Z), Z.stride(0), _ptr(sq), _ptr(Zh), _ptr(Zl),
                                                                 Zh.stride(0), _ptr(ZTh), _ptr(ZTl), ZTh.stride(0) if ZTh is not None else 0,
                                                                 n, d, _ptr(center), int(bool(write_x)),
                                                                 ctypes.byref(xx) if xx is not None else None,
                                                                 ctypes.byref(chain) if chain is not None else None, int(bool(write_z)),
                                                                 _ptr(xrow), self._stream()), "vgan_mask_project_forward_bf3_ex")
            return
        _lib.check(self.lib.vgan_mask_project_forward_bf3(_ptr(logits), logits.stride(0) if logits is not None else 0, _ptr(data), data.stride(0), _ptr(rows),
                                                          _ptr(row_cursor), int(row_batches), int(row_stride), _ptr(S), _ptr(Z), Z.stride(0),
                                                          _ptr(sq), _ptr(Zh), _ptr(Zl), Zh.stride(0), _ptr(ZTh), _ptr(ZTl),
                                                          ZTh.stride(0) if ZTh is not None else 0,
                                                          n, d, _ptr(center), int(bool(write_x)),
                                                          ctypes.byref(xx) if xx is not None else None,
                                                          ctypes.byref(chain) if chain is not None else None, self._stream()),
                   "vgan_mask_project_forward_bf3")

    @staticmethod
    def bf3_fusable(n, d, *lds):
        return d % 4 == 0 and d <= 1024 and n % 8 == 0 and all(int(v) % 4 == 0 for v in lds)

    def gather_rows(self, data, rows, out, sq, row_cursor=None, row_batches=1, row_stride=0, row_offset=0):
        _mat(data, "data"), _mat(out, "out")
        n, d = out.shape[0], data.shape[1]
        _lib.check(self.lib.vgan_gather_rows(_ptr(data), data.stride(0), _ptr(rows), _ptr(row_cursor), int(row_batches),
                                             int(row_stride), int(row_offset), _ptr(out), out.stride(0), _ptr(sq), n, d,
                                             self._stream()), "vgan_gather_rows")

    def gather_rows_split(self, data, rows, center, out, sq, norm_split=False, Zh=None, Zl=None, row_cursor=None, row_batches=1,
                          row_stride=0, row_offset=0, n=None):
        _mat(data, "data")
        d = data.shape[1]
        n = int(n if n is not None else (out.shape[0] if out is not None else sq.numel()))
        _lib.check(self.lib.vgan_gather_rows_split(_ptr(data), data.stride(0), _ptr(rows), _ptr(row_cursor), int(row_batches),
                                                   int(row_stride), int(row_offset), _ptr(center), _ptr(out),
                                                   out.stride(0) if out is not None else 0, _ptr(sq), int(bool(norm_split)), _ptr(Zh),
                                                   _ptr(Zl), Zh.stride(0) if Zh is not None else 0, n, d, self._stream()),
                   "vgan_gather_rows_split")

    def upper_softmax_forward(self, logits, S, U):
        _mat(logits, "logits")
        n, d = logits.shape
        assert S.is_contiguous() and (U is None or U.is_contiguous())
        _lib.check(self.lib.vgan_upper_softmax_forward(_ptr(logits), logits.stride(0), _ptr(S), _ptr(U), n, d, self._stream()),
                   "vgan_upper_softmax_forward")

    def mask_backward(self, gU, S, colkey, pen_weight, row_offset, dlogits, nslabs=1, slab_stride=0):
        _mat(gU, "gU"), _mat(S, "S"), _mat(dlogits, "dlogits")
        n, d = S.shape
        _lib.check(self.lib.vgan_mask_backward(_ptr(gU), gU.stride(0), int(nslabs), int(slab_stride), _ptr(S), S.stride(0),
                                               _ptr(colkey), float(pen_weight),
                                               int(row_offset), _ptr(dlogits), dlogits.stride(0), n, d, self._stream()),
                   "vgan_mask_backward")

    def colmax(self, S, row_offset, part, colkey, from_softmax=True):
        _mat(S, "S")
        n, d = S.shape
        assert part.dtype == torch.int64 and colkey.dtype == torch.int64 and part.numel() >= self.colmax_chunks(n) * d
        _lib.check(self.lib.vgan_colmax(_ptr(S), S.stride(0), int(bool(from_softmax)), int(row_offset), _ptr(part), _ptr(colkey), n, d, self._stream()),
                   "vgan_colmax")

    def colmax_partial(self, S, row_offset, part, from_softmax=True):
        _mat(S, "S")
        n, d = S.shape
        assert part.dtype == torch.int64 and part.numel() >= self.colmax_chunks(n) * d
        _lib.check(self.lib.vgan_colmax_partial(_ptr(S), S.stride(0), int(bool(from_softmax)), int(row_offset), _ptr(part), n, d,
                                                self._stream()), "vgan_colmax_partial")

    def mmd_finalize(self, partial, tiles, colpart, chunks, colkey, n, d, weight, stats, loss, loss_accum=None, accum_scale=1.0,
                     step_counter=None):
        _lib.check(self.lib.vgan_mmd_finalize(_ptr(partial), _ptr(tiles), tiles.shape[0], _ptr(colpart), int(chunks), _ptr(colkey),
                                              int(n), int(d), float(weight), _ptr(stats), _ptr(loss), _ptr(loss_accum),
                                              float(accum_scale), _ptr(step_counter), self._stream()), "vgan_mmd_finalize")

    def finalize_job(self, partial, tiles, colpart, chunks, colkey, n, d, weight, stats, loss, loss_accum=None, accum_scale=1.0,
                     step_counter=None, mode=0, ntiles_main=0):
        return _lib.FinalizeJob(_ptr(partial), _ptr(tiles), _ptr(colpart), _ptr(colkey), _ptr(stats), _ptr(loss), _ptr(loss_accum),
                                _ptr(step_counter), tiles.shape[0], int(chunks), int(n), int(d), float(weight), float(accum_scale),
                                int(mode), int(ntiles_main))

    def mask_from_softmax(self, S, U):
        _mat(S, "S"), _mat(U, "U")
        n, d = S.shape
        _lib.check(self.lib.vgan_mask_from_softmax(_ptr(S), S.stride(0), _ptr(U), U.stride(0), n, d, self._stream()),
                   "vgan_mask_from_softmax")

    def row_sqnorm(self, Z, sq, p):
        _mat(Z, "Z")
        _lib.check(self.lib.vgan_row_sqnorm(_ptr(Z), Z.stride(0), _ptr(sq), Z.shape[0], int(p), self._stream()), "vgan_row_sqnorm")

    def mmd_gram(self, Z, sq, n, p, bw, tiles, calibrate, Wg, wrow0, partial):
        _mat(Z, "Z")
        assert (calibrate or Z.shape[0] >= 2 * n) and tiles.dtype == torch.int32 and tiles.is_contiguous()
        ntiles = tiles.shape[0]
        assert partial.numel() >= 4 * ntiles
        ldw = Wg.stride(0) if Wg is not None else 0
        _lib.check(self.lib.vgan_mmd_gram(_ptr(Z), Z.stride(0), _ptr(sq), int(n), int(p), _ptr(bw), _ptr(tiles), ntiles,
                                          int(bool(calibrate)), _ptr(Wg), ldw, int(wrow0), _ptr(partial), self._stream()),
                   "vgan_mmd_gram")

    @staticmethod
    def _mults(multipliers):
        vals = [float(v) for v in multipliers]
        return (ctypes.c_float * len(vals))(*vals), len(vals)

    def mmd_gram_general(self, Z, sq, n, p, bw, tiles, multipliers, Wg, wrow0, partial):
        _mat(Z, "Z")
        ntiles = tiles.shape[0]
        assert partial.numel() >= 4 * ntiles
        arr, nk = self._mults(multipliers)
        ldw = Wg.stride(0) if Wg is not None else 0
        _lib.check(self.lib.vgan_mmd_gram_general(_ptr(Z), Z.stride(0), _ptr(sq), int(n), int(p), _ptr(bw), _ptr(tiles), ntiles, arr, nk,
                                                  _ptr(Wg), ldw, int(wrow0), _ptr(partial), self._stream()), "vgan_mmd_gram_general")

    def rbf_multi_kernel_matrix(self, Z, sq, bw, multipliers, K, dK=None):
        _mat(Z, "Z"), _mat(K, "K")
        m, p = Z.shape
        arr, nk = self._mults(multipliers)
        _lib.check(self.lib.vgan_rbf_multi_kernel_matrix(_ptr(Z), Z.stride(0), m, p, _ptr(sq), _ptr(bw), arr, nk, _ptr(K), K.stride(0),
                                                         _ptr(dK), dK.stride(0) if dK is not None else 0, self._stream()),
                   "vgan_rbf_multi_kernel_matrix")

    def mmd_gram_colmax(self, Z, sq, n, p, bw, tiles, Wg, wrow0, partial, S, row_offset, colpart, from_softmax=True):
        _mat(Z, "Z"), _mat(S, "S")
        ntiles = tiles.shape[0]
        nrows, d = S.shape
        assert partial.numel() >= 4 * ntiles and colpart.dtype == torch.int64 and colpart.numel() >= self.colmax_chunks(nrows) * d
        ldw = Wg.stride(0) if Wg is not None else 0
        _lib.check(self.lib.vgan_mmd_gram_colmax(_ptr(Z), Z.stride(0), _ptr(sq), int(n), int(p), _ptr(bw), _ptr(tiles), ntiles,
                                                 _ptr(Wg), ldw, int(wrow0), _ptr(partial), _ptr(S), S.stride(0),
                                                 int(bool(from_softmax)), int(row_offset), _ptr(colpart), nrows, d, self._stream()),
                   "vgan_mmd_gram_colmax")

    def mmd_reduce(self, partial, tiles, stats, zero_first=True):
        assert stats.dtype == torch.float64 and stats.numel() >= 4
        _lib.check(self.lib.vgan_mmd_reduce(_ptr(partial), _ptr(tiles), tiles.shape[0], _ptr(stats), int(bool(zero_first)),
                                            self._stream()), "vgan_mmd_reduce")

    def mmd_set_bandwidth(self, stats, n, bw):
        _lib.check(self.lib.vgan_mmd_set_bandwidth(_ptr(stats), int(n), _ptr(bw), self._stream()), "vgan_mmd_set_bandwidth")

    def mmd_loss(self, stats, colkey, n, d, weight, loss, loss_accum=None, accum_scale=1.0, step_counter=None):
        _lib.check(self.lib.vgan_mmd_loss(_ptr(stats), _ptr(colkey), int(n), int(d), float(weight), _ptr(loss), _ptr(loss_accum),
                                          float(accum_scale), _ptr(step_counter), self._stream()), "vgan_mmd_loss")

    def mmd_backward(self, Wg, Z, wrow0, nr, ncols, p, mul, out, splits=1, slab_stride=0, finalize=None, mul_shift=None):
        _mat(Wg, "Wg"), _mat(Z, "Z"), _mat(out, "out")
        ldmul = mul.stride(0) if mul is not None else 0
        _lib.check(self.lib.vgan_mmd_backward(_ptr(Wg), Wg.stride(0), _ptr(Z), Z.stride(0), int(wrow0), int(nr), int(ncols), int(p),
                                              _ptr(mul), ldmul, _ptr(mul_shift), _ptr(out), out.stride(0), int(splits), int(slab_stride),
                                              ctypes.byref(finalize) if finalize is not None else None, self._stream()),
                   "vgan_mmd_backward")

    def mmd_bf3_prepare(self, Z, rows, p, Zh, Zl, ZTh=None, ZTl=None):
        _mat(Z, "Z")
        for t in (Zh, Zl, ZTh, ZTl):
            assert t is None or (t.dtype == torch.int16 and t.is_cuda and t.stride(1) == 1)
        kn = ZTh.stride(0) if ZTh is not None else 0
        _lib.check(self.lib.vgan_mmd_bf3_prepare(_ptr(Z), Z.stride(0), int(rows), int(p), _ptr(Zh), _ptr(Zl), Zh.stride(0),
                                                 _ptr(ZTh), _ptr(ZTl), kn, self._stream()), "vgan_mmd_bf3_prepare")

    def gram_tail_workspace(self, device):
        return torch.zeros(int(self.lib.vgan_mmd_gram_bf3_tail_ws_bytes()) // 4, dtype=torch.int32, device=device)

    def mmd_gram_bf3(self, Zh, Zl, sq, n, bw, tiles, Wh, Wl, wrow0, partial, S=None, row_offset=0, colpart=None, from_softmax=True,
                     tile=64, tail_ws=None, rs_part=None):
        ntiles = tiles.shape[0]
        nrows, d = (S.shape if S is not None else (0, 0))
        ldw = Wh.stride(0) if Wh is not None else 0
        _lib.check(self.lib.vgan_mmd_gram_bf3(_ptr(Zh), _ptr(Zl), Zh.stride(0), _ptr(sq), int(n), _ptr(bw), _ptr(tiles), ntiles,
                                              int(tile), _ptr(Wh), _ptr(Wl), ldw, int(wrow0), _ptr(partial), _ptr(S),
                                              S.stride(0) if S is not None else 0, int(bool(from_softmax)), int(row_offset),
                                              _ptr(colpart), nrows, d, _ptr(tail_ws), tail_ws.numel() * 4 if tail_ws is not None else 0,
                                              _ptr(rs_part), rs_part.stride(0) if rs_part is not None else 0, self._stream()),
                   "vgan_mmd_gram_bf3")

    def mmd_backward_bf3(self, Wh, Wl, ZTh, ZTl, Z, wrow0, nr, p, mul, out, splits=1, slab_stride=0, finalize=None, mul_shift=None,
                         tile=0):
        _mat(Z, "Z"), _mat(out, "out")
        ldmul = mul.stride(0) if mul is not None else 0
        _lib.check(self.lib.vgan_mmd_backward_bf3(_ptr(Wh), _ptr(Wl), Wh.stride(0), _ptr(ZTh), _ptr(ZTl), ZTh.stride(0),
                                                  ZTh.shape[0], _ptr(Z), Z.stride(0), int(wrow0), int(nr), int(p), _ptr(mul), ldmul,
                                                  _ptr(mul_shift), _ptr(out), out.stride(0), int(splits), int(slab_stride), int(tile),
                                                  ctypes.byref(finalize) if finalize is not None else None, self._stream()),
                   "vgan_mmd_backward_bf3")

    def mmd_backward_bf3_rm(self, Wh, Wl, Zh, Zl, zrows, Z, wrow0, nr, p, mul, out, splits=1, slab_stride=0, finalize=None, mul_shift=None,
                            tile=0, xx=None, rs_part=None):
        _mat(Z, "Z"), _mat(out, "out")
        ldmul = mul.stride(0) if mul is not None else 0
        kn = (int(zrows) + 63) // 64 * 64
        assert Wh.stride(0) >= kn and Zh.shape[0] >= zrows
        if xx is not None:
            assert tile in (0, 64)
            _lib.check(self.lib.vgan_mmd_backward_bf3_rm_xx(_ptr(Wh), _ptr(Wl), Wh.stride(0), kn, _ptr(Zh), _ptr(Zl), Zh.stride(0), int(zrows),
                                                            _ptr(Z), Z.stride(0), int(wrow0), int(nr), int(p), _ptr(mul), ldmul, _ptr(mul_shift),
                                                            _ptr(out), out.stride(0), int(splits), int(slab_stride),
                                                            ctypes.byref(finalize) if finalize is not None else None, ctypes.byref(xx),
                                                            self._stream()), "vgan_mmd_backward_bf3_rm_xx")
            return
        _lib.check(self.lib.vgan_mmd_backward_bf3_rm(_ptr(Wh), _ptr(Wl), Wh.stride(0), kn, _ptr(Zh), _ptr(Zl), Zh.stride(0), int(zrows),
                                                     _ptr(Z), Z.stride(0), int(wrow0), int(nr), int(p), _ptr(mul), ldmul, _ptr(mul_shift),
                                                     _ptr(out), out.stride(0), int(splits), int(slab_stride), int(tile),
                                                     ctypes.byref(finalize) if finalize is not None else None, _ptr(rs_part),
                                                     rs_part.stride(0) if rs_part is not None else 0, self._stream()),
                   "vgan_mmd_backward_bf3_rm")

    def mmd_backward_bf3_rm_rebuild(self, Wh, Wl, Zh, Zl, zrows, nr, p, rebuild, out, splits=1, slab_stride=0, finalize=None, xx=None):
        _mat(out, "out")
        kn = (int(zrows) + 63) // 64 * 64
        assert Wh.stride(0) >= kn and Zh.shape[0] >= zrows
        _lib.check(self.lib.vgan_mmd_backward_bf3_rm_rebuild(_ptr(Wh), _ptr(Wl), Wh.stride(0), kn, _ptr(Zh), _ptr(Zl), Zh.stride(0), int(zrows),
                                                             int(nr), int(p), ctypes.byref(rebuild), _ptr(out), out.stride(0), int(splits),
                                                             int(slab_stride), ctypes.byref(finalize) if finalize is not None else None,
                                                             ctypes.byref(xx) if xx is not None else None, self._stream()),
                   "vgan_mmd_backward_bf3_rm_rebuild")

    def mmd_backward_bf3_tile(self, nr, p, splits=1, tile=0):
        return int(self.lib.vgan_mmd_backward_bf3_tile(int(nr), int(p), int(splits), int(tile)))

    def gemm_grouped(self, problems, copy=None, adadelta=None, noise=None, fold=None):
        assert 1 <= len(problems) <= _lib.GEMM_MAX_GROUP
        arr = (_lib.GemmProblem * len(problems))()
        for q, (kind, A, B, C, *rest) in zip(arr, problems):
            if kind == "NT2":
                D, scratch = rest
                _mat(A, "A"), _mat(B, "B"), _mat(C, "C"), _mat(D, "D")
                (m, k), (k2, kb), (n, k2d) = A.shape, B.shape, D.shape
                assert k == kb and k2 == k2d and tuple(C.shape) == (m, n)
                tiles = ((m + 63) // 64) * ((n + 63) // 64)
                assert scratch.is_cuda and scratch.dtype == _f32 and scratch.is_contiguous() and scratch.numel() >= tiles * 64 * _round4(k2)
                q.a, q.b, q.c, q.d, q.scratch = A.data_ptr(), B.data_ptr(), C.data_ptr(), D.data_ptr(), scratch.data_ptr()
                q.kind, q.m, q.n, q.k, q.k2, q.splitk = _lib.GEMM_NT_NT, m, n, k, k2, 1
                q.lda, q.ldb, q.ldc, q.ldd = A.stride(0), B.stride(0), C.stride(0), D.stride(0)
                continue
            q.splitk = int(rest[0]) if rest else 1
            if q.splitk > 1:
                assert C.dim() == 3 and C.shape[0] == q.splitk and C.is_contiguous()
                C = C[0]
            _mat(A, "A"), _mat(B, "B"), _mat(C, "C")
            if kind == "NN":
                (m, k), (k2, n), code = A.shape, B.shape, _lib.GEMM_NN
            elif kind == "NT":
                (m, k), (n, k2), code = A.shape, B.shape, _lib.GEMM_NT
            elif kind == "TN":
                (k, m), (k2, n), code = A.shape, B.shape, _lib.GEMM_TN
            else:
                raise ValueError(kind)
            assert k == k2 and tuple(C.shape) == (m, n), (kind, tuple(A.shape), tuple(B.shape), tuple(C.shape))
            q.a, q.b, q.c, q.kind, q.m, q.n, q.k = A.data_ptr(), B.data_ptr(), C.data_ptr(), code, m, n, k
            q.lda, q.ldb, q.ldc = A.stride(0), B.stride(0), C.stride(0)
        if copy is None and adadelta is None and noise is None and fold is None:
            _lib.check(self.lib.vgan_gemm_grouped(arr, len(problems), self._stream()), "vgan_gemm_grouped")
            return
        x = _lib.GroupedExtras()
        if copy is not None:
            src, dst = copy
            _vec(src, "copy src"), _vec(dst, "copy dst")
            assert src.numel() == dst.numel()
            x.copy_src, x.copy_dst, x.copy_count = src.data_ptr(), dst.data_ptr(), src.numel()
        if adadelta is not None:
            a = adadelta
            for nm in ("p", "sq", "acc"):
                _vec(a[nm], nm)
            x.adadelta, x.p, x.sq_avg, x.acc_delta = 1, a["p"].data_ptr(), a["sq"].data_ptr(), a["acc"].data_ptr()
            x.lr, x.rho, x.eps, x.weight_decay, x.grad_scale = (float(a["lr"]), float(a.get("rho", 0.9)), float(a.get("eps", 1e-6)),
                                                                float(a.get("weight_decay", 0.0)), float(a.get("grad_scale", 1.0)))
            extra = a.get("extra_grad")
            assert len(a["layers"]) == len(problems) + (1 if extra is not None else 0)
            for L, (w, off_w, off_b, out, inp) in zip(x.layer, a["layers"]):
                _mat(w, "w_packed")
                L.w_packed, L.off_w, L.off_b, L.ldp, L.out, L.inp = w.data_ptr(), int(off_w), int(off_b), w.stride(0), int(out), int(inp)
            if extra is not None:
                _mat(extra, "extra_grad")
                x.g_extra, x.ld_extra = extra.data_ptr(), extra.stride(0)
        if noise is not None:
            z = noise["next_noise"]
            x.next_noise, x.noise_rows, x.noise_ld = z.data_ptr(), z.shape[0], z.stride(0)
            x.noise_cols, x.noise_ones_col = int(noise["noise_cols"]), int(noise["noise_ones_col"])
            x.seed, x.step_counter = int(noise["seed"]) & 0xFFFFFFFFFFFFFFFF, noise["step_counter"].data_ptr()
        if fold is not None:
            x.fold = ctypes.addressof(fold)
        _lib.check(self.lib.vgan_gemm_grouped_ex(arr, len(problems), ctypes.byref(x), self._stream()), "vgan_gemm_grouped_ex")

    def mse_grad(self, target, pred, gscale, part, g):
        _mat(target, "target"), _mat(pred, "pred"), _mat(g, "g")
        n, d = pred.shape
        assert part.dtype == torch.float64 and part.numel() >= (n + 3) // 4
        _lib.check(self.lib.vgan_mse_grad(_ptr(target), target.stride(0), _ptr(pred), pred.stride(0), n, d, float(gscale), _ptr(part),
                                          _ptr(g), g.stride(0), self._stream()), "vgan_mse_grad")

    def sum_f64(self, src, count, scale, out, accumulate=False):
        assert src.dtype == torch.float64
        _lib.check(self.lib.vgan_sum_f64(_ptr(src), int(count), float(scale), _ptr(out), int(bool(accumulate)), self._stream()),
                   "vgan_sum_f64")

    def rbf_kernel_matrix(self, Z, sq, alpha, K):
        _mat(Z, "Z"), _mat(K, "K")
        m, p = Z.shape
        _lib.check(self.lib.vgan_rbf_kernel_matrix(_ptr(Z), Z.stride(0), m, p, _ptr(sq), float(alpha), _ptr(K), K.stride(0),
                                                   self._stream()), "vgan_rbf_kernel_matrix")

    def rows_dot(self, A, B, out, broadcast_b=False):
        _mat(A, "A")
        rows, cols = A.shape
        assert out.dtype == torch.float64 and out.numel() >= rows
        ldb = 0 if broadcast_b else B.stride(0)
        _lib.check(self.lib.vgan_rows_dot(_ptr(A), A.stride(0), _ptr(B), ldb, _ptr(out), rows, cols, self._stream()), "vgan_rows_dot")

    def dp_unique_id(self):
        buf = (ctypes.c_uint8 * 128)()
        _lib.check(self.lib.vgan_dp_unique_id(ctypes.cast(buf, ctypes.c_void_p)), "vgan_dp_unique_id")
        return bytes(buf)

    def dp_comm_create(self, nranks, unique_id, rank):
        comm = ctypes.c_void_p()
        buf = (ctypes.c_uint8 * 128).from_buffer_copy(unique_id)
        _lib.check(self.lib.vgan_dp_comm_create(ctypes.byref(comm), int(nranks), ctypes.cast(buf, ctypes.c_void_p), int(rank)),
                   "vgan_dp_comm_create")
        return comm

    def dp_allreduce_sum(self, comm, t):
        _vec(t, "t")
        _lib.check(self.lib.vgan_dp_allreduce_sum(comm, _ptr(t), t.numel(), self._stream()), "vgan_dp_allreduce_sum")

    def dp_allgather(self, comm, t, nranks):
        assert t.is_cuda and t.is_contiguous() and t.shape[0] % nranks == 0
        _lib.check(self.lib.vgan_dp_allgather(comm, _ptr(t), t.numel() * t.element_size() // nranks, self._stream()), "vgan_dp_allgather")

    def dp_comm_destroy(self, comm):
        _lib.check(self.lib.vgan_dp_comm_destroy(comm), "vgan_dp_comm_destroy")

    def shuffle_epoch(self, perm, train_size, seed, epoch):
        _vec(perm, "perm", torch.int32)
        _lib.check(self.lib.vgan_shuffle_epoch(_ptr(perm), perm.numel(), int(train_size), int(seed) & 0xFFFFFFFFFFFFFFFF,
                                               int(epoch) & 0xFFFFFFFFFFFFFFFF, self._stream()), "vgan_shuffle_epoch")

    def shuffle_index(self, i, train_size, seed, epoch):
        return int(self.lib.vgan_shuffle_index(int(i), int(train_size), int(seed) & 0xFFFFFFFFFFFFFFFF, int(epoch) & 0xFFFFFFFFFFFFFFFF))

    def mask_unique(self, masks):
        assert masks.is_cuda and masks.dtype == torch.bool and masks.dim() == 2
        m8 = masks.contiguous().view(torch.uint8)
        n, d = m8.shape
        dev = masks.device
        keys = torch.empty(n * ((d + 63) // 64), dtype=torch.int64, device=dev)
        work = torch.empty(2 * n, dtype=torch.int32, device=dev)
        out_row = torch.zeros(n, dtype=torch.int32, device=dev)
        out_count = torch.zeros(n, dtype=torch.int32, device=dev)
        _lib.check(self.lib.vgan_mask_unique(_ptr(m8), m8.stride(0), n, d, _ptr(keys), _ptr(work), _ptr(out_row), _ptr(out_count),
                                             self._stream()), "vgan_mask_unique")
        cnt = out_count.cpu()
        m = int((cnt > 0).sum())
        return masks[out_row[:m].long()], cnt[:m].to(torch.int64)

    def adadelta_step(self, p, g, sq, acc, lr, rho=0.9, eps=1e-6, weight_decay=0.0, grad_scale=1.0, nslabs=1, slab_stride=0):
        for t, nm in ((p, "p"), (sq, "sq"), (acc, "acc")):
            _vec(t, nm)
        _lib.check(self.lib.vgan_adadelta_step(_ptr(p), _ptr(g), int(nslabs), int(slab_stride), _ptr(sq), _ptr(acc), p.numel(),
                                               float(lr), float(rho), float(eps),
                                               float(weight_decay), float(grad_scale), self._stream()), "vgan_adadelta_step")

    def adadelta_step_packed(self, p, pmap, g_packed, w_packed, sq, acc, lr, rho=0.9, eps=1e-6, weight_decay=0.0, grad_scale=1.0,
                             next_noise=None, noise_cols=0, noise_ones_col=-1, seed=0, step_counter=None):
        for t, nm in ((p, "p"), (sq, "sq"), (acc, "acc"), (g_packed, "g_packed"), (w_packed, "w_packed")):
            _vec(t, nm)
        _vec(pmap, "pmap", torch.int32)
        assert pmap.numel() == p.numel()
        zr, zld = (next_noise.shape[0], next_noise.stride(0)) if next_noise is not None else (0, 0)
        _lib.check(self.lib.vgan_adadelta_step_packed(_ptr(p), _ptr(pmap), _ptr(g_packed), _ptr(w_packed), _ptr(sq), _ptr(acc),
                                                      p.numel(), float(lr), float(rho), float(eps), float(weight_decay),
                                                      float(grad_scale), _ptr(next_noise), zr, int(noise_cols), zld,
                                                      int(noise_ones_col), int(seed) & 0xFFFFFFFFFFFFFFFF, _ptr(step_counter),
                                                      self._stream()), "vgan_adadelta_step_packed")

    def noise_normal(self, z, seed, step_counter, stream_id=0, cols=None, ones_col=-1):
        _mat(z, "z")
        rows, ld = z.shape[0], z.stride(0)
        cols = z.shape[1] if cols is None else int(cols)
        _lib.check(self.lib.vgan_noise_normal(_ptr(z), rows, cols, ld, int(ones_col), int(seed) & 0xFFFFFFFFFFFFFFFF,
                                              _ptr(step_counter), int(stream_id), self._stream()), "vgan_noise_normal")

    def homogeneous_pack(self, layers, unpack=False):
        key = tuple((W.data_ptr(), tuple(W.shape), W.stride(0), b.data_ptr(), P.data_ptr(), tuple(P.shape), P.stride(0)) for W, b, P in layers)
        cache = self.__dict__.setdefault("_pack_tables", {})
        if key not in cache:
            if len(cache) >= 16:
                cache.pop(next(iter(cache)))
            rows = []
            for W, b, P in layers:
                _mat(W, "W"), _vec(b, "b"), _mat(P, "P")
                out, kin = W.shape
                assert b.numel() == out and P.shape[0] >= out + 1 and P.shape[1] >= kin + 1
                rows.append([W.data_ptr(), b.data_ptr(), P.data_ptr(), out, kin, W.stride(0), P.stride(0), 0])
            cache[key] = (torch.tensor(rows, dtype=torch.int64, device=layers[0][0].device),
                          max((r[3] + 1) * (r[4] + 1) for r in rows))
        desc, max_elems = cache[key]
        _lib.check(self.lib.vgan_homogeneous_pack(_ptr(desc), desc.shape[0], int(max_elems), int(bool(unpack)), self._stream()),
                   "vgan_homogeneous_pack")

    def mse(self, a, b, scale, out, accumulate=False):
        _mat(a, "a"), _mat(b, "b")
        n, d = a.shape
        _lib.check(self.lib.vgan_mse(_ptr(a), a.stride(0), _ptr(b), b.stride(0), n, d, float(scale), _ptr(out),
                                     int(bool(accumulate)), self._stream()), "vgan_mse")

    def outlier_pack(self, X, center, table, first, count, packed, sq=None):
        _mat(X, "X"), _vec(packed, "packed")
        feat, feat_off, col_off = table
        n, d = X.shape
        _lib.check(self.lib.vgan_outlier_pack(_ptr(X), X.stride(0), n, d, _ptr(center), _ptr(feat), _ptr(feat_off), _ptr(col_off),
                                              int(first), int(count), _ptr(packed), _ptr(sq), self._stream()), "vgan_outlier_pack")

    def outlier_knn(self, Pq, sq_q, nq, Pr, sq_r, nr, table, first, count, k, exclude_self, engine, splits, nbr,
                    part_d=None, part_i=None):
        _vec(nbr, "nbr", torch.int32)
        _, feat_off, col_off = table
        _lib.check(self.lib.vgan_outlier_knn(_ptr(Pq), _ptr(sq_q), int(nq), _ptr(Pr), _ptr(sq_r), int(nr), _ptr(feat_off), _ptr(col_off),
                                             int(first), int(count), int(k), int(bool(exclude_self)), int(engine), int(splits),
                                             _ptr(part_d), _ptr(part_i), _ptr(nbr), self._stream()), "vgan_outlier_knn")

    def outlier_refine(self, Xq, Xr, table, first, count, nbr, k, out_idx, out_dist, kdist=None):
        _mat(Xq, "Xq"), _mat(Xr, "Xr"), _vec(out_idx, "out_idx", torch.int32), _vec(out_dist, "out_dist")
        feat, feat_off, _ = table
        assert Xq.shape[1] == Xr.shape[1]
        _lib.check(self.lib.vgan_outlier_refine(_ptr(Xq), Xq.stride(0), Xq.shape[0], _ptr(Xr), Xr.stride(0), Xr.shape[0], Xq.shape[1],
                                                _ptr(feat), _ptr(feat_off), int(first), int(count), _ptr(nbr), int(k), _ptr(out_idx),
                                                _ptr(out_dist), _ptr(kdist), self._stream()), "vgan_outlier_refine")

    def outlier_score(self, idx, dist, nq, k, count, method, score=None, score_row=None, kdist_ref=None, lrd_ref=None, nr=0,
                      lrd_out=None):
        ld = score.stride(0) if score is not None else nq
        _lib.check(self.lib.vgan_outlier_score(_ptr(idx), _ptr(dist), int(nq), int(k), int(count), int(method), _ptr(kdist_ref),
                                               _ptr(lrd_ref), int(nr), _ptr(score), _ptr(score_row), int(ld), _ptr(lrd_out),
                                               self._stream()), "vgan_outlier_score")

    def outlier_kde(self, Pq, sq_q, nq, Pr, sq_r, nr, table, first, count, bandwidth, exclude_self, engine, splits, pivot, acc,
                    score, score_row=None):
        _vec(bandwidth, "bandwidth", torch.float64), _vec(pivot, "pivot", torch.int32), _vec(acc, "acc", torch.int64)
        _mat(score, "score")
        assert pivot.numel() >= count * nq and acc.numel() >= count * nq
        _, feat_off, col_off = table
        _lib.check(self.lib.vgan_outlier_kde(_ptr(Pq), _ptr(sq_q), int(nq), _ptr(Pr), _ptr(sq_r), int(nr), _ptr(feat_off), _ptr(col_off),
                                             int(first), int(count), _ptr(bandwidth), int(bool(exclude_self)), int(engine), int(splits),
                                             _ptr(pivot), _ptr(acc), _ptr(score), _ptr(score_row), score.stride(0), self._stream()),
                   "vgan_outlier_kde")

    def outlier_combine(self, score, weights, out):
        _mat(score, "score"), _vec(weights, "weights", torch.float64), _vec(out, "out", torch.float64)
        S, n = score.shape
        _lib.check(self.lib.vgan_outlier_combine(_ptr(score), score.stride(0), S, n, _ptr(weights), _ptr(out), self._stream()),
                   "vgan_outlier_combine")

    def outlier_abod(self, Xq, Xr, table, first, count, idx, k, score, score_row=None):
        _mat(Xq, "Xq"), _mat(Xr, "Xr"), _vec(idx, "idx", torch.int32), _mat(score, "score")
        feat, feat_off, _ = table
        assert Xq.shape[1] == Xr.shape[1] and idx.numel() >= count * Xq.shape[0] * k
        _lib.check(self.lib.vgan_outlier_abod(_ptr(Xq), Xq.stride(0), Xq.shape[0], _ptr(Xr), Xr.stride(0), Xr.shape[0], Xq.shape[1],
                                              _ptr(feat), _ptr(feat_off), int(first), int(count), _ptr(idx), int(k), _ptr(score),
                                              _ptr(score_row), score.stride(0), self._stream()), "vgan_outlier_abod")

    def outlier_abod_floor(self, score, score_floor, n_degenerate=None):
        _mat(score, "score"), _vec(score_floor, "score_floor", torch.float64)
        S, n = score.shape
        assert score_floor.numel() >= S
        if n_degenerate is not None:
            _vec(n_degenerate, "n_degenerate", torch.int32)
            assert n_degenerate.numel() >= S
        _lib.check(self.lib.vgan_outlier_abod_floor(_ptr(score), score.stride(0), S, n, int(n_degenerate is not None),
                                                    _ptr(score_floor), _ptr(n_degenerate), self._stream()), "vgan_outlier_abod_floor")

    def outlier_score_stats(self, score, mode, center, scale):
        _mat(score, "score"), _vec(center, "center", torch.float64), _vec(scale, "scale", torch.float64)
        S, n = score.shape
        assert center.numel() >= S and scale.numel() >= S
        need = self.lib.vgan_outlier_score_stats_ws_bytes(S, n, int(mode))
        if need < 0:
            _lib.check(1, "vgan_outlier_score_stats_ws_bytes")
        ws = torch.empty((need + 7) // 8, dtype=torch.int64, device=score.device)
        _lib.check(self.lib.vgan_outlier_score_stats(_ptr(score), score.stride(0), S, n, int(mode), _ptr(center), _ptr(scale),
                                                     _ptr(ws), ws.numel() * 8, self._stream()), "vgan_outlier_score_stats")

    def outlier_combine_normalized(self, score, center, scale, weights, combination, out):
        _mat(score, "score"), _vec(out, "out", torch.float64)
        for name, v in (("center", center), ("scale", scale), ("weights", weights)):
            if v is not None:
                _vec(v, name, torch.float64)
        S, n = score.shape
        _lib.check(self.lib.vgan_outlier_combine_normalized(_ptr(score), score.stride(0), S, n, _ptr(center), _ptr(scale),
                                                            _ptr(weights), int(combination), _ptr(out), self._stream()),
                   "vgan_outlier_combine_normalized")

    def cluster_lloyd_ws_bytes(self, n, n_clusters, count, total_dims):
        need = self.lib.vgan_cluster_lloyd_ws_bytes(int(n), int(n_clusters), int(count), int(total_dims))
        if need < 0:
            _lib.check(1, "vgan_cluster_lloyd_ws_bytes")
        return need

    def cluster_image(self, centers, n_clusters, table, first, count, col_center, img, img_sq=None):
        _vec(centers, "centers", torch.float64), _vec(img, "img")
        feat, feat_off, col_off = table
        _lib.check(self.lib.vgan_cluster_image(_ptr(centers), int(n_clusters), _ptr(feat), _ptr(feat_off), _ptr(col_off), int(first),
                                               int(count), _ptr(col_center), _ptr(img), _ptr(img_sq), self._stream()),
                   "vgan_cluster_image")

    def cluster_lloyd(self, Pq, sq_q, X, table, first, count, total_dims, max_dims, n_clusters, engine, col_center, tol_var, centers,
                      img, img_sq, label, changed, done, n_iter, workspace, iterations):
        _mat(X, "X"), _vec(Pq, "Pq"), _vec(img, "img"), _vec(centers, "centers", torch.float64), _vec(tol_var, "tol_var", torch.float64)
        _vec(workspace, "workspace", torch.float64), _vec(label, "label", torch.int32)
        for name, v in (("changed", changed), ("done", done), ("n_iter", n_iter)):
            _vec(v, name, torch.int32)
        assert label.numel() >= count * X.shape[0]
        feat, feat_off, col_off = table
        n, d = X.shape
        _lib.check(self.lib.vgan_cluster_lloyd(_ptr(Pq), _ptr(sq_q), _ptr(X), X.stride(0), n, d, _ptr(feat), _ptr(feat_off), _ptr(col_off),
                                               int(first), int(count), int(total_dims), int(max_dims), int(n_clusters), int(engine),
                                               _ptr(col_center), _ptr(tol_var), _ptr(centers), _ptr(img), _ptr(img_sq), _ptr(label),
                                               _ptr(changed), _ptr(done), _ptr(n_iter), _ptr(workspace), workspace.numel() * 8,
                                               int(iterations), self._stream()), "vgan_cluster_lloyd")

    def cluster_final(self, Xq, table, S, n_clusters, centers, sizes, large=None, use_weights=False, label=None, inertia=None,
                      score=None, score_row=None):
        _mat(Xq, "Xq"), _vec(centers, "centers", torch.float64), _vec(sizes, "sizes", torch.int64)
        feat, feat_off, _ = table
        nq, d = Xq.shape
        part = None
        if large is None:
            _vec(label, "label", torch.int32), _vec(inertia, "inertia", torch.float64)
            assert label.numel() >= S * nq and inertia.numel() >= S
            part = torch.empty(S * ((nq + 63) // 64), dtype=torch.float64, device=Xq.device)
        else:
            _vec(large, "large", torch.int32), _mat(score, "score")
            assert large.numel() >= S * n_clusters and score.shape[0] >= S
        assert sizes.numel() >= S * n_clusters
        _lib.check(self.lib.vgan_cluster_final(_ptr(Xq), Xq.stride(0), nq, d, _ptr(feat), _ptr(feat_off), int(S), int(n_clusters),
                                               _ptr(centers), _ptr(large), _ptr(sizes), int(bool(use_weights)), _ptr(label), _ptr(part),
                                               _ptr(inertia), _ptr(score), _ptr(score_row), score.stride(0) if score is not None else 0,
                                               self._stream()), "vgan_cluster_final")


_default = None


def default_ops():
    global _default
    if _default is None:
        _default = HipOps()
    return _default
```

v-gan_amd/trainer.py:

```python
import os

import torch

ADADELTA_RHO = 0.9
ADADELTA_EPS = 1e-6


def _round4(v):
    return (v + 3) // 4 * 4


def _launch_rounds(tiles, slots, can_split):
    if tiles <= 0:
        return 0.0
    full, r = divmod(tiles, slots)
    if r == 0:
        return float(full)
    x = r / slots
    last = 0.55 if x <= 0.5 else 0.55 + 0.9 * (x - 0.5)
    if can_split and x <= 0.125:
        last = 0.25
    elif can_split and x <= 0.25:
        last = 0.4
    elif can_split and x <= 0.5:
        last = 0.5
    return full + last


def _best_boundary(n_main, total, slots, can_split):
    cost = lambda k: _launch_rounds(k, slots, can_split) + _launch_rounds(total - k, slots, can_split)
    best, best_cost = n_main, cost(n_main)
    for k in range(n_main - 1, max(n_main - slots, 0), -1):
        c = cost(k)
        if c < best_cost - 1e-9 and c <= cost(n_main) - 0.15:
            best, best_cost = k, c
    return best


class FlatParams:

    def __init__(self, params, device):
        self.shapes = [tuple(p.shape) for p in params]
        self.offsets = []
        off = 0
        for p in params:
            self.offsets.append(off)
            off += _round4(p.numel())
        self.total = off
        self.flat = torch.zeros(off, dtype=torch.float32, device=device)
        self.grad = torch.zeros_like(self.flat)
        self.sq = torch.zeros_like(self.flat)
        self.acc = torch.zeros_like(self.flat)
        for k, (p, o) in enumerate(zip(params, self.offsets)):
            self.flat[o:o + p.numel()].copy_(p.detach().reshape(-1).to(device=device, dtype=torch.float32))
            p.data = self.view(self.flat, k)

    def view(self, buf, k):
        o, shp = self.offsets[k], self.shapes[k]
        numel = 1
        for s in shp:
            numel *= s
        return buf[o:o + numel].view(shp)


class NoKLStepEngine:
    def __init__(self, ops, generator, data, batch_size, batches_per_epoch, lr=0.007, weight_decay=0.04, penalty_weight=10.0,
                 seed=777, noise="device", rank=0, world=1, group=None, use_graph=True, loss_accum_scale=None,
                 generator_mode=None, force_exchange=False, mmd_precision=None, center_operand=True, overlap_exchange=None,
                 fuse_update=None, front=None, chain_assoc=None):
        self.ops = ops
        self.dev = data.device
        self.rank, self.world, self.group = rank, world, group
        self.exchange = world > 1 or bool(force_exchange)
        n = self.n = int(batch_size)
        if n % world != 0:
            raise ValueError(f"global batch {n} must be divisible by the number of ranks {world}")
        nl = self.nl = n // world
        self.lo = rank * nl
        self.data = data
        d = self.d = data.shape[1]
        dp = self.dp = _round4(d)
        self.nb = int(batches_per_epoch)
        self.lr, self.wd, self.pen = float(lr), float(weight_decay), float(penalty_weight)
        self.seed = int(seed)
        self.noise_mode = noise
        self.use_graph = bool(use_graph) and data.is_cuda
        self.graph = None
        self.graph_multi = None
        self.graph_blocks = {}
        self.steps_per_graph = max(1, min(16, int(batches_per_epoch)))
        self.steps_done = 0
        self._xx_primed = False
        self._coalesce = None
        self.mode = generator_mode or os.environ.get("VGAN_GENERATOR", "collapsed")
        if self.mode not in ("collapsed", "layered"):
            raise ValueError(f"generator_mode must be 'collapsed' or 'layered', got {self.mode!r}")
        self.fuse_update = (os.environ.get("VGAN_FUSE_UPDATE", "0") == "1") if fuse_update is None else bool(fuse_update)
        want_front = front or os.environ.get("VGAN_DP_FRONT", "auto")
        if want_front not in ("auto", "replicated", "sharded"):
            raise ValueError(f"front must be 'auto', 'replicated' or 'sharded', got {want_front!r}")
        if want_front == "sharded" and not (self.exchange and self.mode == "collapsed"):
            raise ValueError("front='sharded' needs a data-parallel engine (world > 1 or force_exchange) with the collapsed generator")
        self.front_sharded = (self.exchange and self.mode == "collapsed" and
                              (want_front == "sharded" or (want_front == "auto" and n * data.shape[1] >= (1 << 22))))

        lin = [m for m in generator.main if isinstance(m, torch.nn.Linear)]
        assert len(lin) == 4
        L = self.L = lin[0].in_features
        self.widths = [L] + [m.out_features for m in lin]
        params = [q for m in lin for q in (m.weight, m.bias)]
        self.fp = FlatParams(params, self.dev)
        self.W = [self.fp.view(self.fp.flat, 2 * k) for k in range(4)]
        self.b = [self.fp.view(self.fp.flat, 2 * k + 1) for k in range(4)]

        f32 = dict(dtype=torch.float32, device=self.dev)
        self.splits = max(1, min(8, nl // 128))
        self.e = [_round4(w + 1) for w in self.widths]
        self.za = torch.zeros(n, self.e[0], **f32)
        self.za[:, L] = 1.0
        self.z_own = self.za[self.lo:self.lo + nl]
        self.logits = torch.zeros(n, d, **f32)
        self.chain_flops = False
        if self.mode == "layered":
            self.gslab = torch.zeros(self.splits, self.fp.total, **f32) if self.splits > 1 else None
            gbase = self.gslab[0] if self.splits > 1 else self.fp.grad
            self.dW = [self.fp.view(gbase, 2 * k) for k in range(4)]
            self.db = [self.fp.view(gbase, 2 * k + 1) for k in range(4)]
            self.acts = [self.za[:, :L]] + [torch.zeros(n, w, **f32) for w in self.widths[1:4]] + [self.logits]
            self.acts_own = [a[self.lo:self.lo + nl] for a in self.acts]
            self.dacts = [None] + [torch.zeros(nl, w, **f32) for w in self.widths[1:4]]
        else:
            e = self.e
            poff = [0]
            for k in range(1, 5):
                poff.append(poff[-1] + e[k] * e[k - 1])
            self.Wt_all = torch.zeros(poff[-1], **f32)
            self.Gt_all = torch.zeros(poff[-1], **f32)
            self.Wt = [None] + [self.Wt_all[poff[k - 1]:poff[k]].view(e[k], e[k - 1]) for k in range(1, 5)]
            self.Gt = [None] + [self.Gt_all[poff[k - 1]:poff[k]].view(e[k], e[k - 1]) for k in range(1, 5)]
            self.At = [None, self.Wt[1]] + [torch.zeros(e[k], e[0], **f32) for k in range(2, 5)]
            self.M = [None, self.Gt[1]] + [torch.zeros(e[k], e[0], **f32) for k in range(2, 5)]
            self.B3 = torch.zeros(e[4], e[2], **f32)
            self.B2 = torch.zeros(e[4], e[1], **f32)
            self.At1s = torch.zeros(e[1], e[0], **f32)
            want_assoc = chain_assoc or os.environ.get("VGAN_CHAIN_ASSOC", "auto")
            if want_assoc not in ("auto", "depth", "flops"):
                raise ValueError(f"chain_assoc must be 'auto', 'depth' or 'flops', got {want_assoc!r}")
            self.chain_flops = want_assoc == "flops" or (want_assoc == "auto" and 2.0 * e[4] * e[3] * e[2] >= 1e9)
            if self.chain_flops:
                self.fuse_update = False
                def split_of(m, n_, k):
                    t64 = ((m + 63) // 64) * ((n_ + 63) // 64)
                    return 1 if 2.0 * m * n_ * k < 2.5e8 else max(1, min(8, 1024 // t64, k // 256))
                self.fwd_split = {k: split_of(e[k], e[0], e[k - 1]) for k in (2, 3, 4)}
                self.bwd_split = {k: split_of(e[k - 1], e[0], e[k]) for k in (4, 3, 2)}
                if os.environ.get("VGAN_CHAIN_SPLITK", "1") != "1":
                    self.fwd_split, self.bwd_split = {k: 1 for k in (2, 3, 4)}, {k: 1 for k in (4, 3, 2)}
                need = max([self.fwd_split[k] * e[k] * e[0] for k in (2, 3, 4)] + [self.bwd_split[k] * e[k - 1] * e[0] for k in (4, 3, 2)])
                self.chain_ws = torch.zeros(need, **f32)
            pmap = torch.full((self.fp.total,), -1, dtype=torch.int32)
            for k in range(1, 5):
                wk, wk1 = self.widths[k], self.widths[k - 1]
                r = torch.arange(wk, dtype=torch.int32)[:, None] * e[k - 1]
                ow, ob = self.fp.offsets[2 * (k - 1)], self.fp.offsets[2 * (k - 1) + 1]
                pmap[ow:ow + wk * wk1] = (poff[k - 1] + r + torch.arange(wk1, dtype=torch.int32)[None, :]).reshape(-1)
                pmap[ob:ob + wk] = (poff[k - 1] + r + wk1).reshape(-1)
            self.pmap = pmap.to(self.dev)
            self.pack_layers = [(self.W[k - 1], self.b[k - 1], self.Wt[k]) for k in range(1, 5)]
            self.unpack_layers = [(self.fp.view(self.fp.grad, 2 * (k - 1)), self.fp.view(self.fp.grad, 2 * (k - 1) + 1), self.Gt[k])
                                  for k in range(1, 5)]
            ops.homogeneous_pack(self.pack_layers, unpack=False)

        self.precision = mmd_precision or os.environ.get("VGAN_MMD_PRECISION", "auto")
        if self.precision not in ("auto", "fp32", "bf16x3"):
            raise ValueError(f"mmd_precision must be 'auto', 'fp32' or 'bf16x3', got {self.precision!r}")
        if self.precision == "auto":
            self.precision = "bf16x3" if 2 * n * d >= (1 << 20) else "fp32"
        self.bf3 = self.precision == "bf16x3"
        self.center = torch.zeros(dp, **f32)
        if center_operand:
            ops.col_mean(data, self.center)
        self.bwd_tile = int(os.environ.get("VGAN_BWD_TILE", "0"))
        self._fin = None
        self.S = torch.zeros(n, d, **f32)
        self.S_own = self.S[self.lo:self.lo + nl]
        self.Z = torch.zeros(2 * n, dp, **f32)
        self.sqn = torch.zeros(2 * n, **f32)
        self.sq_cal = torch.zeros(2 * n, **f32) if self.bf3 else self.sqn
        self.Wg = torch.zeros(nl, 2 * n, **f32)
        out_tiles = ((nl + 63) // 64) * ((d + 63) // 64)
        auto_splits = max(2 if self.bf3 else 1, min(4, 256 // max(out_tiles, 1), max(1, (2 * n) // 64)))
        rm = self.front_sharded or os.environ.get("VGAN_BWD_OPERAND", "rowmajor") != "transposed"
        if self.bf3 and rm and self.bwd_tile in (0, 256) and ops.mmd_backward_bf3_tile(nl, d, 1, self.bwd_tile) == 256:
            auto_splits = 1
        self.bsplits = max(1, int(os.environ.get("VGAN_BWD_SPLITS", str(auto_splits))))
        self.gU_slabs = torch.zeros(self.bsplits, nl, dp, **f32)
        self.gU = self.gU_slabs[0]
        self.dlogits_pad = torch.zeros(nl, dp, **f32)
        self.dlogits = self.dlogits_pad[:, :d]
        self.rm_backward = True
        if self.precision == "bf16x3":
            i16 = dict(dtype=torch.int16, device=self.dev)
            self.kp, self.kn = (d + 63) // 64 * 64, (2 * n + 63) // 64 * 64
            self.Zh, self.Zl = torch.zeros(2 * n, self.kp, **i16), torch.zeros(2 * n, self.kp, **i16)
            self.rm_backward = self.front_sharded or os.environ.get("VGAN_BWD_OPERAND", "rowmajor") != "transposed"
            if self.rm_backward:
                self.ZTh = self.ZTl = None
            else:
                self.ZTh, self.ZTl = torch.zeros(self.kp, self.kn, **i16), torch.zeros(self.kp, self.kn, **i16)
            self.Wh, self.Wl = torch.zeros(nl, self.kn, **i16), torch.zeros(nl, self.kn, **i16)
        self.fused_prepare = (self.bf3 and not self.front_sharded and ops.bf3_fusable(n, d, self.logits.stride(0), data.stride(0), dp) and
                              os.environ.get("VGAN_FUSED_PREPARE", "1") == "1")
        self.chain_in_mask = (self.mode == "collapsed" and not self.front_sharded and ops.chain_fusable(n, d, data.stride(0), dp) and
                              (not self.bf3 or self.fused_prepare) and os.environ.get("VGAN_CHAIN_IN_MASK", "0") == "1")
        self._chain = None
        self.two_stage_logits = (self.mode == "collapsed" and not self.chain_flops and not self.chain_in_mask and not self.front_sharded and
                                 os.environ.get("VGAN_LOGITS_2STAGE", "0") == "1")
        if self.two_stage_logits:
            e2 = self.e[2]
            self.T = torch.zeros(n, e2, **f32)
            self.T_ws = torch.zeros(((n + 63) // 64) * ((e2 + 63) // 64) * 64 * _round4(self.e[1]), **f32)
        self.perm = torch.zeros(self.nb, n, dtype=torch.int32, device=self.dev)
        self.perm_next = torch.zeros_like(self.perm)
        self.epoch_staged = False
        self.gram_tile = 64
        want = os.environ.get("VGAN_GRAM_TILE", "auto")
        if self.bf3 and nl % 128 == 0 and want in ("auto", "128"):
            if want == "128" or len(ops.build_tiles(n, 1, rank, world, device=self.dev, tile=128)) >= 512:
                self.gram_tile = 128
        if self.bf3 and nl % 256 == 0 and want in ("auto", "256"):
            if want == "256" or len(ops.build_tiles(n, 1, rank, world, device=self.dev, tile=256)) >= 512:
                self.gram_tile = 256
        self.gram_tail_ws = (ops.gram_tail_workspace(self.dev)
                             if self.gram_tile == 256 and os.environ.get("VGAN_GRAM_TAIL", "1") != "0" else None)
        self.rs_part = None
        if (self.gram_tile == 256 and self.rm_backward and n % 128 == 0 and os.environ.get("VGAN_RS_FROM_GRAM", "1") != "0"
                and ops.mmd_backward_bf3_tile(nl, d, self.bsplits, self.bwd_tile) == 256):
            self.rs_part = torch.zeros((2 * n + 127) // 128, nl, **f32)
        if overlap_exchange is None and os.environ.get("VGAN_OVERLAP") is not None:
            overlap_exchange = {"1": True, "0": False}.get(os.environ["VGAN_OVERLAP"], os.environ["VGAN_OVERLAP"])
        self.overlap = False if overlap_exchange is None else bool(overlap_exchange)
        if self.front_sharded and self.overlap:
            raise ValueError("overlap_exchange and front='sharded' are two schedules of the same exchange: choose one")
        self._side = torch.cuda.Stream(device=self.dev) if (self.overlap and data.is_cuda and overlap_exchange != "serial") else None
        self.x_ahead = self.overlap and (not self.bf3 or self.rm_backward)
        self.xx_ride = False
        self._xx = None
        if (self.fused_prepare and self.gram_tile == 64 and not self.overlap and self.rm_backward and
                os.environ.get("VGAN_XX_RIDE", "0") == "1"):
            split, n_main = ops.build_tiles(n, 1, rank, world, device=self.dev, tile=64, split_xx=True)
            xx_tiles = split.shape[0] - n_main
            self.xx_ride = xx_tiles > 0 and 8 * ((n // 8 + 7) // 8) + xx_tiles <= 512
        if self.xx_ride:
            i16 = dict(dtype=torch.int16, device=self.dev)
            rows_total = data.shape[0]
            self.Dh, self.Dl = torch.zeros(rows_total, self.kp, **i16), torch.zeros(rows_total, self.kp, **i16)
            self.dsq = torch.zeros(rows_total, **f32)
            ops.gather_rows_split(data, None, self.center, None, self.dsq, True, self.Dh, self.Dl, n=rows_total)
        self.xx_in_m4 = (self.bf3 and self.mode == "collapsed" and self.gram_tile == 64 and not self.overlap and not self.xx_ride and
                         not self.front_sharded and
                         ops.linear_backward_params_xx_supported(nl, self.e[0], dp) and os.environ.get("VGAN_XX_IN_M4", "1") == "1")
        self._xx_m4 = self._fold = None
        if self.front_sharded:
            self.tiles, self.n_main = ops.build_tiles(n, 1, rank, world, device=self.dev, tile=self.gram_tile, split="yy_last")
            slots = 256 if self.gram_tile >= 128 else (512 if self.bf3 else 1024)
            self.n_main = _best_boundary(self.n_main, self.tiles.shape[0], slots, self.gram_tail_ws is not None)
        elif self.overlap or self.xx_ride or self.xx_in_m4:
            self.tiles, self.n_main = ops.build_tiles(n, 1, rank, world, device=self.dev, tile=self.gram_tile, split_xx=True)
            if self.xx_in_m4:
                slots = int(os.environ.get("VGAN_GRAM_SLOTS", "512"))
                self.n_main = min(self.tiles.shape[0], max(self.n_main, slots))
                if self.n_main == self.tiles.shape[0]:
                    self.xx_in_m4 = False
        else:
            self.tiles = ops.build_tiles(n, 1, rank, world, device=self.dev, tile=self.gram_tile)
            self.n_main = self.tiles.shape[0]
        self.xx_late_in_backward = False
        if self.xx_in_m4 and self.rm_backward and os.environ.get("VGAN_XX_LATE", "backward") == "backward":
            late = self.tiles.shape[0] - self.n_main
            bwd_wgs = ((d + 63) // 64) * ((nl + 63) // 64) * self.bsplits + 1
            self.xx_late_in_backward = (ops.mmd_backward_bf3_tile(nl, d, self.bsplits, self.bwd_tile) == 64 and late <= 512 - bwd_wgs)
        plain_bf3 = (getattr(ops, "bf3_rebuild", False) and self.bf3 and self.fused_prepare and self.gram_tile == 64 and
                     self.rm_backward and world == 1 and not self.overlap and not self.front_sharded and
                     ops.mmd_backward_bf3_tile(nl, d, self.bsplits, self.bwd_tile) == 64)
        self.lean = plain_bf3 and os.environ.get("VGAN_Z_FP32", "0") != "1"
        self.xrow = torch.zeros(n, dtype=torch.int32, device=self.dev) if self.lean else None
        self._rebuild = None
        self.tiles_cal = self.tiles if (world == 1 and self.gram_tile == 64 and not (self.overlap or self.xx_ride or self.xx_in_m4 or self.front_sharded)) else ops.build_tiles(n, 0, 0, 1, device=self.dev)
        self.partial = torch.zeros(max(self.tiles.shape[0], self.tiles_cal.shape[0]), 4, **f32)
        self.stats = torch.zeros(4, dtype=torch.float64, device=self.dev)
        self.bw = torch.zeros(1, **f32)
        self.has_bw = False
        self.loss = torch.zeros(1, **f32)
        self.loss_accum = torch.zeros(1, **f32)
        self._hist, self._hist_n, self._hist_events = None, 0, []
        self._read_stream, self._loss_host = None, None
        self.accum_scale = (1.0 / self.nb) if loss_accum_scale is None else float(loss_accum_scale)
        self.step_counter = torch.zeros(1, dtype=torch.int64, device=self.dev)
        self.col_chunks = (world * ops.colmax_chunks(nl)) if self.front_sharded else ops.colmax_chunks(n)
        self.colpart = torch.zeros(self.col_chunks * d, dtype=torch.int64, device=self.dev)
        own = ops.colmax_chunks(nl) * d
        self.colpart_own = self.colpart[rank * own:(rank + 1) * own] if self.front_sharded else self.colpart
        self.colkey = torch.zeros(d, dtype=torch.int64, device=self.dev)
        if self.front_sharded and data.is_cuda and self._collect().is_initialized():
            self._coalesce = self._probe_coalescing(self._collect())

    def set_epoch_batches(self, idx):
        if os.environ.get("VGAN_FEED_DIRECT") == "1":
            self.perm.copy_(idx.to(dtype=torch.int32), non_blocking=True)
            self._after_new_epoch_table()
            return
        self.stage_epoch_batches(idx)
        self.begin_epoch()

    def stage_epoch_batches(self, idx):
        self.perm_next.copy_(idx.to(dtype=torch.int32).view(self.nb, self.n), non_blocking=True)
        self.epoch_staged = True

    def begin_epoch(self):
        if not self.epoch_staged:
            raise RuntimeError("begin_epoch without a staged table (stage_epoch_batches)")
        self.perm.copy_(self.perm_next)
        self.epoch_staged = False
        self._after_new_epoch_table()

    def _after_new_epoch_table(self):
        if self.overlap and self.has_bw:
            self._prefetch_xx()

    def _prefetch_xx(self):
        self._prefetch_x_operand()
        self._xx_tiles()
        self._xx_primed = True

    def _prefetch_x_operand(self):
        ops, n = self.ops, self.n
        rowsel = dict(row_cursor=self.step_counter, row_batches=self.nb, row_stride=n)
        if self.bf3:
            ops.gather_rows_split(self.data, self.perm, self.center, self.Z[:n], self.sqn[:n], True, self.Zh[:n], self.Zl[:n], **rowsel)
        else:
            ops.gather_rows_split(self.data, self.perm, self.center, self.Z[:n], self.sqn[:n], False, **rowsel)

    def _xx_tiles(self):
        ops, n = self.ops, self.n
        ntx = self.tiles.shape[0] - self.n_main
        if ntx == 0:
            return
        tx, px = self.tiles[self.n_main:], self.partial[self.n_main:self.n_main + ntx]
        if self.bf3:
            ops.mmd_gram_bf3(self.Zh, self.Zl, self.sqn, n, self.bw, tx, None, None, 0, px, tile=self.gram_tile)
        else:
            ops.mmd_gram(self.Z, self.sqn, n, self.dp, self.bw, tx, False, None, 0, px)

    def _fork_prefetch(self):
        if not self.overlap:
            return
        if self._side is None:
            self._prefetch_xx()
            return
        self._side.wait_stream(torch.cuda.current_stream())
        with torch.cuda.stream(self._side):
            self._prefetch_xx()

    def _join_prefetch(self):
        if self.overlap and self._side is not None:
            torch.cuda.current_stream().wait_stream(self._side)

    def shuffle_epoch(self, epoch):
        self.ops.shuffle_epoch(self.perm, self.data.shape[0], self.seed, int(epoch))
        self._after_new_epoch_table()

    def set_bandwidth(self, value):
        self.bw.fill_(float(value))
        self.has_bw = True

    def set_noise(self, z):
        self.za[:, :self.L].copy_(z.to(dtype=torch.float32), non_blocking=True)

    def epoch_loss(self):
        v = float(self._sum_over_ranks(self.loss_accum).item())
        self.loss_accum.zero_()
        return v

    def close_epoch(self):
        if self._hist is None or self._hist_n == self._hist.numel():
            grown = torch.zeros(max(64, 2 * self._hist_n), dtype=torch.float32, device=self.dev)
            if self._hist is not None:
                grown[:self._hist_n].copy_(self._hist)
            self._hist = grown
        slot = self._hist_n
        cell = self._hist[slot:slot + 1]
        cell.copy_(self.loss_accum)
        self.loss_accum.zero_()
        if self.exchange:
            self._collect().all_reduce(cell, group=self.group)
        ev = None
        if self.data.is_cuda:
            ev = torch.cuda.Event()
            ev.record()
        self._hist_events.append(ev)
        self._hist_n += 1
        return slot

    def read_epoch_loss(self, slot):
        ev = self._hist_events[slot]
        if ev is None:
            return float(self._hist[slot])
        if self._read_stream is None:
            self._read_stream = torch.cuda.Stream(self.dev)
            self._loss_host = torch.zeros(1, dtype=torch.float32).pin_memory()
        self._read_stream.wait_event(ev)
        with torch.cuda.stream(self._read_stream):
            self._loss_host.copy_(self._hist[slot:slot + 1], non_blocking=True)
        self._read_stream.synchronize()
        return float(self._loss_host[0])

    def step_loss(self):
        return float(self._sum_over_ranks(self.loss).item())

    def _sum_over_ranks(self, t):
        if not self.exchange:
            return t
        t = t.clone()
        self._collect().all_reduce(t, group=self.group)
        return t

    def grad_view(self, k):
        if self.mode == "collapsed":
            self.ops.homogeneous_pack(self.unpack_layers, unpack=True)
        elif not self.exchange and self.splits > 1:
            return sum(self.fp.view(self.gslab[sl], k) for sl in range(self.splits))
        return self.fp.view(self.fp.grad, k)

    def _generator_forward(self, own_rows=False):
        ops = self.ops
        if self.mode == "layered":
            for k in range(4):
                ops.linear_forward(self.acts[k], self.W[k], self.b[k], self.acts[k + 1])
            return
        Wt, At = self.Wt, self.At
        if self.chain_flops:
            for k in (2, 3, 4):
                sp = self.fwd_split[k]
                if sp > 1:
                    ops.gemm_grouped([("NN", Wt[k], At[k - 1], self._slabs(sp, At[k]), sp)])
                    ops.reduce_slabs(self.chain_ws, At[k].numel(), sp, At[k])
                else:
                    ops.gemm_grouped([("NN", Wt[k], At[k - 1], At[k])])
        elif self.two_stage_logits:
            ops.gemm_grouped([("NN", Wt[2], At[1], At[2]), ("NN", Wt[4], Wt[3], self.B3), ("NT2", self.za, Wt[1], self.T, Wt[2], self.T_ws)])
            ops.gemm_grouped([("NN", Wt[3], At[2], At[3]), ("NN", self.B3, Wt[2], self.B2), ("NT", self.T, self.B3[:self.d], self.logits)])
            return
        else:
            ops.gemm_grouped([("NN", Wt[2], At[1], At[2]), ("NN", Wt[4], Wt[3], self.B3)])
            ops.gemm_grouped([("NN", Wt[3], At[2], At[3]), ("NN", self.B3, At[2], At[4]), ("NN", self.B3, Wt[2], self.B2)])
        if own_rows:
            ops.linear_forward(self.z_own, At[4][:self.d], None, self.logits[self.lo:self.lo + self.nl])
        elif not self.chain_in_mask:
            ops.linear_forward(self.za, At[4][:self.d], None, self.logits)

    def _slabs(self, splits, like):
        return self.chain_ws[:splits * like.numel()].view(splits, like.shape[0], like.shape[1])

    def _generator_backward_update(self, dist):
        ops = self.ops
        adadelta = dict(lr=self.lr, rho=ADADELTA_RHO, eps=ADADELTA_EPS, weight_decay=self.wd, grad_scale=1.0)
        if self.mode == "layered":
            g = self.dlogits
            for k in (3, 2, 1, 0):
                ops.linear_backward_params(g, self.acts_own[k], self.dW[k], self.db[k], self.splits, self.fp.total)
                if k:
                    ops.linear_backward_input(g, self.W[k], self.dacts[k])
                    g = self.dacts[k]
            if dist:
                if self.splits > 1:
                    ops.reduce_slabs(self.gslab, self.fp.total, self.splits, self.fp.grad)
                dist.all_reduce(self.fp.grad, group=self.group)
                ops.adadelta_step(self.fp.flat, self.fp.grad, self.fp.sq, self.fp.acc, **adadelta)
            elif self.splits > 1:
                ops.adadelta_step(self.fp.flat, self.gslab[0], self.fp.sq, self.fp.acc, nslabs=self.splits, slab_stride=self.fp.total,
                                  **adadelta)
            else:
                ops.adadelta_step(self.fp.flat, self.fp.grad, self.fp.sq, self.fp.acc, **adadelta)
            return
        e, d = self.e, self.d
        if self.xx_in_m4 and not self.xx_late_in_backward:
            ops.linear_backward_params_xx(self.dlogits_pad, self.z_own, self.M[4][:self.dp], self._late_xx_job())
        else:
            ops.linear_backward_params(self.dlogits_pad, self.z_own, self.M[4][:self.dp], None)
        if dist:
            dist.all_reduce(self.M[4], group=self.group)
        M, Gt, At = self.M, self.Gt, self.At
        fused_noise = dict(next_noise=self.za, noise_cols=self.L, noise_ones_col=self.L, seed=self.seed,
                           step_counter=self.step_counter) if self.noise_mode == "device" else {}
        if self.chain_flops:
            Wt = self.Wt
            for k in (4, 3, 2):
                sp = self.bwd_split[k]
                probs = [("TN", Wt[k], M[k], self._slabs(sp, M[k - 1]), sp) if sp > 1 else ("TN", Wt[k], M[k], M[k - 1])]
                if k < 4:
                    probs.append(("NT", M[k + 1], At[k], Gt[k + 1]))
                ops.gemm_grouped(probs, fold=self._fold if (self.xx_in_m4 and k == 4) else None)
                if sp > 1:
                    ops.reduce_slabs(self.chain_ws, M[k - 1].numel(), sp, M[k - 1])
            ops.gemm_grouped([("NT", M[2], At[1], Gt[2])])
            ops.adadelta_step_packed(self.fp.flat, self.pmap, self.Gt_all, self.Wt_all, self.fp.sq, self.fp.acc, **adadelta, **fused_noise)
            return
        if not self.fuse_update:
            ops.gemm_grouped([("TN", self.Wt[4], M[4], M[3]), ("TN", self.B3, M[4], M[2]), ("TN", self.B2, M[4], M[1])],
                             fold=self._fold if self.xx_in_m4 else None)
            ops.gemm_grouped([("NT", M[4], At[3], Gt[4]), ("NT", M[3], At[2], Gt[3]), ("NT", M[2], At[1], Gt[2])])
            ops.adadelta_step_packed(self.fp.flat, self.pmap, self.Gt_all, self.Wt_all, self.fp.sq, self.fp.acc, **adadelta, **fused_noise)
            return
        ops.gemm_grouped([("TN", self.Wt[4], M[4], M[3]), ("TN", self.B3, M[4], M[2]), ("TN", self.B2, M[4], M[1])],
                         copy=(self.Wt[1], self.At1s), fold=self._fold if self.xx_in_m4 else None)
        w, off = self.widths, self.fp.offsets
        layers = [(self.Wt[k], off[2 * (k - 1)], off[2 * (k - 1) + 1], w[k], w[k - 1]) for k in (4, 3, 2, 1)]
        ops.gemm_grouped([("NT", M[4], At[3], Gt[4]), ("NT", M[3], At[2], Gt[3]), ("NT", M[2], self.At1s, Gt[2])],
                         adadelta=dict(p=self.fp.flat, sq=self.fp.sq, acc=self.fp.acc, layers=layers, extra_grad=Gt[1], **adadelta),
                         noise=fused_noise or None)

    def _collect(self):
        import torch.distributed as dist
        return dist

    def _forward(self):
        ops, n, nl, lo = self.ops, self.n, self.nl, self.lo
        if self.noise_mode == "device" and (self.mode == "layered" or self.steps_done == 0):
            ops.noise_normal(self.za, self.seed, self.step_counter, 0, cols=self.L, ones_col=self.L)
        self._generator_forward()
        rowsel = dict(row_cursor=self.step_counter, row_batches=self.nb, row_stride=n)
        logits = self.logits
        if self.chain_in_mask:
            if self._chain is None:
                self._chain = ops.logits_chain(self.za, self.At[4][:self.d])
            rowsel["chain"] = self._chain
            logits = None
        if self.fused_prepare:
            xx = None
            if self.xx_ride and self.has_bw:
                if self._xx is None:
                    ntx = self.tiles.shape[0] - self.n_main
                    self._xx = ops.xx_job(self.Dh, self.Dl, self.dsq, self.tiles[self.n_main:], self.bw, self.partial[self.n_main:self.n_main + ntx])
                xx = self._xx
            if self.lean:
                ops.mask_project_forward_bf3(logits, self.data, self.perm, self.S, self.Z, self.sqn, self.Zh, self.Zl, None, None,
                                             center=self.center, xx=xx, write_z=not self.has_bw, xrow=self.xrow, **rowsel)
            else:
                ops.mask_project_forward_bf3(logits, self.data, self.perm, self.S, self.Z, self.sqn, self.Zh, self.Zl, self.ZTh, self.ZTl,
                                             center=self.center, write_x=not self.x_ahead, xx=xx, **rowsel)
            return
        if self.x_ahead:
            ops.mask_project_forward(logits, self.data, self.perm, self.S, None, None, self.Z[n:], None, self.sqn[n:],
                                     row_offset=0, center=self.center, norm_split=self.bf3, **rowsel)
        else:
            ops.mask_project_forward(logits, self.data, self.perm, self.S, None, self.Z[:n], self.Z[n:], self.sqn[:n], self.sqn[n:],
                                     row_offset=0, center=self.center, norm_split=self.bf3, **rowsel)

    def _calibrate(self):
        ops = self.ops
        if self.bf3:
            ops.row_sqnorm(self.Z, self.sq_cal, self.dp)
        ops.mmd_gram(self.Z, self.sq_cal, self.n, self.dp, None, self.tiles_cal, True, None, 0, self.partial)
        ops.mmd_reduce(self.partial, self.tiles_cal, self.stats, True)
        ops.mmd_set_bandwidth(self.stats, self.n, self.bw)
        self.has_bw = True

    def _loss_backward_update(self):
        ops, n, nl, lo, d = self.ops, self.n, self.nl, self.lo, self.d
        dist = self._collect() if self.exchange else None
        gstride = nl * self.dp
        bf3 = self.precision == "bf16x3"
        if bf3 and not self.fused_prepare:
            if self.x_ahead:
                ops.mmd_bf3_prepare(self.Z[n:], n, d, self.Zh[n:], self.Zl[n:])
            else:
                ops.mmd_bf3_prepare(self.Z, 2 * n, d, self.Zh, self.Zl, self.ZTh, self.ZTl)
        if bf3:
            ops.mmd_gram_bf3(self.Zh, self.Zl, self.sqn, n, self.bw, self.tiles[:self.n_main], self.Wh, self.Wl, n + lo, self.partial, self.S, 0,
                             self.colpart, True, tile=self.gram_tile, tail_ws=self.gram_tail_ws, rs_part=self.rs_part)
        else:
            ops.mmd_gram_colmax(self.Z, self.sqn, n, self.dp, self.bw, self.tiles[:self.n_main], self.Wg, n + lo, self.partial, self.S, 0,
                                self.colpart, True)
        if self._fin is None:
            fin_args = (self.partial, self.tiles, self.colpart, ops.colmax_chunks(n), self.colkey, n, d, self.pen if self.rank == 0 else 0.0,
                        self.stats, self.loss, self.loss_accum, self.accum_scale, self.step_counter)
            if self.xx_in_m4:
                self._fin = ops.finalize_job(*fin_args, mode=1, ntiles_main=self.n_main)
                self._fold = ops.finalize_job(*fin_args, mode=2, ntiles_main=self.n_main)
            else:
                self._fin = ops.finalize_job(*fin_args)
        fin = self._fin
        if bf3:
            if self.lean:
                if self._rebuild is None:
                    self._rebuild = ops.bwd_rebuild(self.data, self.xrow, self.S, self.center)
                ops.mmd_backward_bf3_rm_rebuild(self.Wh, self.Wl, self.Zh, self.Zl, 2 * n, nl, d, self._rebuild, self.gU, self.bsplits, gstride,
                                                fin, xx=self._late_xx_job() if self.xx_late_in_backward else None)
            elif self.rm_backward:
                ops.mmd_backward_bf3_rm(self.Wh, self.Wl, self.Zh, self.Zl, 2 * n, self.Z, n + lo, nl, d, self.Z[lo:lo + nl], self.gU,
                                        self.bsplits, gstride, fin, mul_shift=self.center, tile=self.bwd_tile,
                                        xx=self._late_xx_job() if self.xx_late_in_backward else None, rs_part=self.rs_part)
            else:
                ops.mmd_backward_bf3(self.Wh, self.Wl, self.ZTh, self.ZTl, self.Z, n + lo, nl, d, self.Z[lo:lo + nl], self.gU, self.bsplits,
                                     gstride, fin, mul_shift=self.center, tile=self.bwd_tile)
        else:
            ops.mmd_backward(self.Wg, self.Z, n + lo, nl, 2 * n, self.dp, self.Z[lo:lo + nl], self.gU, self.bsplits, gstride, fin,
                             mul_shift=self.center)
        self._fork_prefetch()
        ops.mask_backward(self.gU, self.S_own, self.colkey, self.pen, lo, self.dlogits, self.bsplits, gstride)
        self._generator_backward_update(dist)
        self._join_prefetch()

    def _forward_sharded(self):
        ops, n, nl, lo, d = self.ops, self.n, self.nl, self.lo, self.d
        if self.noise_mode == "device" and self.steps_done == 0:
            ops.noise_normal(self.za, self.seed, self.step_counter, 0, cols=self.L, ones_col=self.L)
        self._generator_forward(own_rows=True)
        rowsel = dict(row_cursor=self.step_counter, row_batches=self.nb, row_stride=n)
        own, yown = slice(lo, lo + nl), slice(n + lo, n + lo + nl)
        if self.bf3:
            ops.gather_rows_split(self.data, self.perm, self.center, None, self.sqn[:n], True, self.Zh[:n], self.Zl[:n], **rowsel)
        else:
            ops.gather_rows_split(self.data, self.perm, self.center, self.Z[:n], self.sqn[:n], False, **rowsel)
        ops.mask_project_forward(self.logits[own], self.data, self.perm, self.S_own, None, self.Z[own] if self.bf3 else None, self.Z[yown],
                                 None, self.sqn[yown], row_offset=lo, center=self.center, norm_split=self.bf3, **rowsel)
        if self.bf3:
            ops.mmd_bf3_prepare(self.Z[yown], nl, d, self.Zh[yown], self.Zl[yown])
        ops.colmax_partial(self.S_own, lo, self.colpart_own)

    def _all_gather(self, dist, out, own):
        size = dist.get_world_size(self.group) if dist.is_initialized() else 1
        if size != self.world:
            out = own
        if own.is_cuda and dist.get_backend(self.group) == "gloo":
            host = out.cpu()
            dist.all_gather_into_tensor(host, own.cpu(), group=self.group)
            out.copy_(host)
            return None
        return dist.all_gather_into_tensor(out, own, group=self.group, async_op=True)

    def _exchange_front(self, dist):
        n, nl, lo = self.n, self.nl, self.lo
        yown = slice(n + lo, n + lo + nl)
        pairs = []
        if self.bf3:
            pairs += [(img[n:2 * n].view(torch.int32), img[yown].view(torch.int32)) for img in (self.Zh, self.Zl)]
        else:
            pairs.append((self.Z[n:], self.Z[yown]))
        pairs += [(self.sqn[n:], self.sqn[yown]), (self.colpart, self.colpart_own)]
        if self._coalesce is None:
            self._coalesce = self._probe_coalescing(dist)
        if self._coalesce:
            emulated = dist.get_world_size(self.group) != self.world
            with dist._coalescing_manager(group=self.group, device=self.dev, async_ops=True) as cm:
                for out, own in pairs:
                    dist.all_gather_into_tensor(own if emulated else out, own, group=self.group)
            return [cm]
        return [self._all_gather(dist, out, own) for out, own in pairs]

    def _probe_coalescing(self, dist):
        if os.environ.get("VGAN_DP_COALESCE", "0") != "1" or not self.data.is_cuda or torch.cuda.is_current_stream_capturing():
            return False
        try:
            if dist.get_backend(self.group) != "nccl" or not hasattr(dist, "_coalescing_manager"):
                return False
            size = dist.get_world_size(self.group)
            a, b = torch.zeros(size * 4, device=self.dev), torch.zeros(size * 2, dtype=torch.int64, device=self.dev)
            r = dist.get_rank(self.group)
            with dist._coalescing_manager(group=self.group, device=self.dev, async_ops=True) as cm:
                dist.all_gather_into_tensor(a, a[4 * r:4 * r + 4], group=self.group)
                dist.all_gather_into_tensor(b, b[2 * r:2 * r + 2], group=self.group)
            cm.wait()
            torch.cuda.synchronize()
            return True
        except Exception as e:
            import warnings
            warnings.warn(f"vgan_amd: coalesced all-gather is not available on this stack ({type(e).__name__}: {e}); one launch per gather")
            return False

    def _loss_backward_update_sharded(self, all_rows_here=False):
        ops, n, nl, lo, d = self.ops, self.n, self.nl, self.lo, self.d
        dist = self._collect()
        works = []
        if all_rows_here:
            if self.bf3:
                ops.mmd_bf3_prepare(self.Z, 2 * n, d, self.Zh, self.Zl)
            self.colpart.zero_()
            ops.colmax_partial(self.S, 0, self.colpart[:ops.colmax_chunks(n) * d])
        else:
            works = self._exchange_front(dist)
        na = self.n_main

        def gram(t0, t1):
            if t1 <= t0:
                return
            if self.bf3:
                ops.mmd_gram_bf3(self.Zh, self.Zl, self.sqn, n, self.bw, self.tiles[t0:t1], self.Wh, self.Wl, n + lo, self.partial[t0:t1],
                                 tile=self.gram_tile, tail_ws=self.gram_tail_ws, rs_part=self.rs_part)
            else:
                ops.mmd_gram(self.Z, self.sqn, n, self.dp, self.bw, self.tiles[t0:t1], False, self.Wg, n + lo, self.partial[t0:t1])

        gram(0, na)
        for w in works:
            if w is not None:
                w.wait()
        gram(na, self.tiles.shape[0])
        if self._fin is None:
            self._fin = ops.finalize_job(self.partial, self.tiles, self.colpart, self.col_chunks, self.colkey, n, d,
                                         self.pen if self.rank == 0 else 0.0, self.stats, self.loss, self.loss_accum, self.accum_scale,
                                         self.step_counter)
        gstride = nl * self.dp
        if self.bf3:
            ops.mmd_backward_bf3_rm(self.Wh, self.Wl, self.Zh, self.Zl, 2 * n, self.Z, n + lo, nl, d, self.Z[lo:lo + nl], self.gU,
                                    self.bsplits, gstride, self._fin, mul_shift=self.center, tile=self.bwd_tile, rs_part=self.rs_part)
        else:
            ops.mmd_backward(self.Wg, self.Z, n + lo, nl, 2 * n, self.dp, self.Z[lo:lo + nl], self.gU, self.bsplits, gstride, self._fin,
                             mul_shift=self.center)
        ops.mask_backward(self.gU, self.S_own, self.colkey, self.pen, lo, self.dlogits, self.bsplits, gstride)
        self._generator_backward_update(dist)

    def _late_xx_job(self):
        if self._xx_m4 is None:
            ntx = self.tiles.shape[0] - self.n_main
            self._xx_m4 = self.ops.xx_job(self.Zh, self.Zl, self.sqn, self.tiles[self.n_main:], self.bw,
                                          self.partial[self.n_main:self.n_main + ntx])
        return self._xx_m4

    def _step_body(self):
        if self.front_sharded:
            self._forward_sharded()
            self._loss_backward_update_sharded()
        else:
            self._forward()
            self._loss_backward_update()

    def step(self):
        if not self.has_bw:
            if self.overlap:
                self._prefetch_x_operand()
            self._forward()
            self._calibrate()
            if self.overlap or self.xx_ride:
                self._xx_tiles()
                self._xx_primed = True
            if self.front_sharded:
                self._loss_backward_update_sharded(all_rows_here=True)
            else:
                self._loss_backward_update()
        elif self.use_graph and self.steps_done > 0:
            if self.graph is None:
                self._capture()
            if self.graph is not None:
                self.graph.replay()
            else:
                self._step_body()
        else:
            if self.overlap and not self._xx_primed:
                self._prefetch_xx()
            self._step_body()
        self.steps_done += 1

    def run_steps(self, count):
        count = int(count)
        if count > 1 and self.noise_mode != "device":
            raise ValueError("run_steps needs the device noise stream: host-provided noise is set per step (set_noise + step)")
        m = self.steps_per_graph
        while count > 0:
            blk = min(count, m)
            if (blk > 1 and self.use_graph and self.has_bw and self.steps_done > 0 and self.noise_mode == "device" and
                    self.graph is not None):
                g = self._block_graph(blk)
                if g is not None:
                    g.replay()
                    self.steps_done += blk
                    count -= blk
                    continue
            self.step()
            count -= 1

    def _block_graph(self, steps):
        g = self.graph_blocks.get(steps)
        if g is None and len(self.graph_blocks) < 4:
            g = self.graph_blocks[steps] = self._capture_graph(steps) or False
        if steps == self.steps_per_graph:
            self.graph_multi = g or None
        return g or None

    def _capture_graph(self, steps):
        torch.cuda.synchronize()
        g = torch.cuda.CUDAGraph()
        try:
            with torch.cuda.graph(g):
                for _ in range(steps):
                    self._step_body()
        except Exception as e:
            import warnings
            warnings.warn(f"vgan_amd: HIP-graph capture of {steps} training step(s) failed ({type(e).__name__}: {e}); running eager launches")
            torch.cuda.synchronize()
            g = None
        if self.exchange and self.world > 1:
            dist = self._collect()
            ok = torch.tensor([1 if g is not None else 0], dtype=torch.int32, device=self.dev)
            dist.all_reduce(ok, op=dist.ReduceOp.MIN, group=self.group)
            if int(ok.item()) == 0:
                g = None
        return g

    def _capture(self):
        self.graph = self._capture_graph(1)
        if self.graph is None:
            self.use_graph = False

    def generator_logits(self, z):
        ops = self.ops
        h = z.to(device=self.dev, dtype=torch.float32).contiguous()
        for k in range(4):
            y = torch.empty(h.shape[0], self.W[k].shape[0], dtype=torch.float32, device=self.dev)
            ops.linear_forward(h, self.W[k], self.b[k], y)
            h = y
        return h
```

Before: 9910 steps/s.

## Split-K the collapsed-chain backward GEMMs with ticketed in-kernel slab reduction

```diff
diff --git a/include/vgan_hip.h b/include/vgan_hip.h
--- a/include/vgan_hip.h
+++ b/include/vgan_hip.h
@@ -30,6 +30,9 @@
 int vgan_linear_backward_params_xx_supported(int n, int in, int out);
 int vgan_linear_backward_params_xx(const float* dy, int lddy, const float* x, int ldx, float* dW, int lddw, int n, int in,
                                    int out, const struct vgan_xx_job* xx, vgan_stream_t stream);
+int64_t vgan_linear_backward_params_ksplit_ws_bytes(int in, int out, int parts);
+int vgan_linear_backward_params_ksplit(const float* dy, int lddy, const float* x, int ldx, float* dW, int lddw, int n, int in,
+                                       int out, int parts, void* ws, int64_t ws_bytes, vgan_stream_t stream);
 int vgan_reduce_slabs(const float* src, int64_t slab_stride, int nslabs, float* dst, int64_t count,
                       vgan_stream_t stream);
 
@@ -188,6 +191,9 @@
 } vgan_grouped_extras;
 int vgan_gemm_grouped_ex(const vgan_gemm_problem* problems, int count, const vgan_grouped_extras* extras,
                          vgan_stream_t stream);
+int64_t vgan_gemm_grouped_ksplit_ws_bytes(const vgan_gemm_problem* problems, int count, const int32_t* kparts);
+int vgan_gemm_grouped_ksplit(const vgan_gemm_problem* problems, int count, const vgan_grouped_extras* extras,
+                             const int32_t* kparts, void* ws, int64_t ws_bytes, vgan_stream_t stream);
 
 typedef struct vgan_xx_job {
     const uint16_t* Dh;
diff --git a/v-gan_amd/csrc/gemm_core.hpp b/v-gan_amd/csrc/gemm_core.hpp
--- a/v-gan_amd/csrc/gemm_core.hpp
+++ b/v-gan_amd/csrc/gemm_core.hpp
@@ -509,6 +509,51 @@
     __device__ static __forceinline__ int col_of() { return threadIdx.x & 31; }
 };
 
+constexpr int kKSplitMaxParts = 8;
+constexpr int kKSplitSlabBytes = 32 * 32 * 4;
+static inline long ksplit_ticket_bytes(long tiles) { return (tiles * 4 + 255) / 256 * 256; }
+static inline int ksplit_kchunk(int k, int parts, int bk) { return ((k + parts - 1) / parts + bk - 1) / bk * bk; }
+
+struct KSplitWs {
+    float* slabs;
+    int* tickets;
+    int slab_bytes;
+};
+
+template <int NR, int NTH>
+__device__ __forceinline__ bool ksplit_finish(float (&o)[NR], const KSplitWs& ws, int slot, int slab0, int part, int parts, float* lds) {
+    static_assert(NR * NTH * 4 == kKSplitSlabBytes, "one 32x32 tile per workgroup");
+    const __amdgpu_buffer_rsrc_t slabs = __builtin_amdgcn_make_buffer_rsrc(ws.slabs, 0, ws.slab_bytes, 0x00020000);
+    constexpr int kCoherent = 17;
+    const int mine = slab0 + part * kKSplitSlabBytes + (int)threadIdx.x * 4;
+#pragma unroll
+    for (int rr = 0; rr < NR; ++rr) __builtin_amdgcn_raw_buffer_store_b32(__float_as_uint(o[rr]), slabs, mine + rr * NTH * 4, 0, kCoherent);
+    asm volatile("s_waitcnt vmcnt(0)" ::: "memory");
+    __syncthreads();
+    if (threadIdx.x == 0) {
+        const int old = __hip_atomic_fetch_add(ws.tickets + slot, 1, __ATOMIC_RELAXED, __HIP_MEMORY_SCOPE_AGENT);
+        if (old == parts - 1) __hip_atomic_store(ws.tickets + slot, 0, __ATOMIC_RELAXED, __HIP_MEMORY_SCOPE_AGENT);
+        lds[0] = old == parts - 1 ? 1.f : 0.f;
+    }
+    __syncthreads();
+    if (lds[0] == 0.f) return false;
+    float v[kKSplitMaxParts][NR];
+#pragma unroll
+    for (int q = 0; q < kKSplitMaxParts; ++q) {
+        const int theirs = slab0 + min(q, parts - 1) * kKSplitSlabBytes + (int)threadIdx.x * 4;
+#pragma unroll
+        for (int rr = 0; rr < NR; ++rr) v[q][rr] = __uint_as_float(__builtin_amdgcn_raw_buffer_load_b32(slabs, theirs + rr * NTH * 4, 0, kCoherent));
+    }
+#pragma unroll
+    for (int rr = 0; rr < NR; ++rr) {
+        float s = v[0][rr];
+#pragma unroll
+        for (int q = 1; q < kKSplitMaxParts; ++q) s = q < parts ? s + v[q][rr] : s;
+        o[rr] = s;
+    }
+    return true;
+}
+
 template <int WM, int WN>
 __device__ __forceinline__ void zero_acc(f32x16 (&acc)[WM][WN]) {
 #pragma unroll
diff --git a/v-gan_amd/csrc/grouped.hip b/v-gan_amd/csrc/grouped.hip
--- a/v-gan_amd/csrc/grouped.hip
+++ b/v-gan_amd/csrc/grouped.hip
@@ -238,6 +238,68 @@
     else tile_ks<MC, MC, 4, 16>(q, t, lds, x, qi);
 }
 
+struct GroupedKSplit {
+    KSplitWs ws;
+    int parts[VGAN_GEMM_MAX_GROUP], kchunk[VGAN_GEMM_MAX_GROUP];
+    int slot0[VGAN_GEMM_MAX_GROUP];
+    int slab0[VGAN_GEMM_MAX_GROUP];
+};
+
+template <int LA, int LB>
+__device__ __forceinline__ void tile_ks_split(const vgan_gemm_problem& q, int t, int part, int parts, int kchunk, const KSplitWs& ws, int slot,
+                                              int slab0, float* lds) {
+    using G = GemmTileKS<QKS, LA, LB, 4, 16>;
+    const int gx = (q.n + 31) / 32;
+    const int m0 = (t / gx) * 32, n0 = (t % gx) * 32;
+    const int k0 = part * kchunk, klen = min(kchunk, q.k - k0);
+    float o[G::NR];
+    if (klen > 0) {
+        const float* a = q.a + (LA == KC ? (long)k0 : (long)k0 * q.lda);
+        const float* b = q.b + (LB == KC ? (long)k0 : (long)k0 * q.ldb);
+        G::run(a, q.lda, b, q.ldb, m0, n0, q.m, q.n, klen, lds, o);
+    } else {
+#pragma unroll
+        for (int rr = 0; rr < G::NR; ++rr) o[rr] = 0.f;
+    }
+    if (!ksplit_finish<G::NR, G::NTH>(o, ws, slot, slab0, part, parts, lds)) return;
+    const int col = n0 + G::col_of();
+#pragma unroll
+    for (int rr = 0; rr < G::NR; ++rr) {
+        const int row = m0 + G::row_of(rr);
+        if (row < q.m && col < q.n) q.c[(long)row * q.ldc + col] = o[rr];
+    }
+}
+
+__global__ __launch_bounds__(1024, 1) void gemm_grouped_ks16_split_kernel(GroupedArgs g, GroupedExtras x, GroupedKSplit ks) {
+    constexpr int kLds = cmax(cmax(GemmTileKS<QKS, KC, MC, 4, 16>::kLdsFloats, GemmTileKS<QKS, MC, MC, 4, 16>::kLdsFloats),
+                              GemmTileKS<QKS, KC, KC, 4, 16>::kLdsFloats);
+    __shared__ __attribute__((aligned(16))) float lds[kLds];
+    if ((int)blockIdx.x >= g.tile_start[VGAN_GEMM_MAX_GROUP]) {
+        grouped_extra_jobs(x, blockIdx.x - g.tile_start[VGAN_GEMM_MAX_GROUP], g.count);
+        return;
+    }
+    int qi = 0;
+#pragma unroll
+    for (int i = 1; i < VGAN_GEMM_MAX_GROUP; ++i)
+        if (i < g.count && (int)blockIdx.x >= g.tile_start[i]) qi = i;
+    const vgan_gemm_problem& q = g.p[qi];
+    int t = blockIdx.x - g.tile_start[qi];
+    const int parts = ks.parts[qi];
+    if (parts <= 1) {
+        if (q.kind == VGAN_GEMM_NN) tile_ks<KC, MC, 4, 16>(q, t, lds, x, qi);
+        else if (q.kind == VGAN_GEMM_NT) tile_ks<KC, KC, 4, 16>(q, t, lds, x, qi);
+        else tile_ks<MC, MC, 4, 16>(q, t, lds, x, qi);
+        return;
+    }
+    const int per = (g.tile_start[qi + 1] - g.tile_start[qi]) / parts;
+    const int part = t / per;
+    t %= per;
+    const int slot = ks.slot0[qi] + t, slab0 = ks.slab0[qi] + t * parts * kKSplitSlabBytes, kc = ks.kchunk[qi];
+    if (q.kind == VGAN_GEMM_NN) tile_ks_split<KC, MC>(q, t, part, parts, kc, ks.ws, slot, slab0, lds);
+    else if (q.kind == VGAN_GEMM_NT) tile_ks_split<KC, KC>(q, t, part, parts, kc, ks.ws, slot, slab0, lds);
+    else tile_ks_split<MC, MC>(q, t, part, parts, kc, ks.ws, slot, slab0, lds);
+}
+
 }
 
 using namespace vgan;
@@ -247,9 +309,33 @@
     return (int)(g < 1 ? 1 : (g > 256 ? 256 : g));
 }
 
-extern "C" int vgan_gemm_grouped_ex(const vgan_gemm_problem* problems, int count, const vgan_grouped_extras* extras,
-                                    vgan_stream_t stream) {
+static int64_t ksplit_need(const vgan_gemm_problem* problems, int count, const int32_t* kparts) {
+    if (!problems || count < 1 || count > VGAN_GEMM_MAX_GROUP) return -1;
+    long split_tiles = 0, slabs = 0;
+    for (int i = 0; i < count; ++i) {
+        const int parts = kparts ? kparts[i] : 1;
+        if (parts < 1 || parts > kKSplitMaxParts || problems[i].m <= 0 || problems[i].n <= 0) return -1;
+        if (parts == 1) continue;
+        const long t32 = (long)((problems[i].m + 31) / 32) * ((problems[i].n + 31) / 32);
+        split_tiles += t32;
+        slabs += t32 * parts;
+    }
+    return split_tiles == 0 ? 0 : ksplit_ticket_bytes(split_tiles) + slabs * kKSplitSlabBytes;
+}
+
+static int grouped_launch(const vgan_gemm_problem* problems, int count, const vgan_grouped_extras* extras, const int32_t* kparts, void* ws,
+                          int64_t ws_bytes, vgan_stream_t stream) {
     VGAN_CHECK_ARG(problems && count >= 1 && count <= VGAN_GEMM_MAX_GROUP);
+    bool ksplit = false;
+    for (int i = 0; i < count && kparts != nullptr; ++i) {
+        VGAN_CHECK_ARG(kparts[i] >= 1 && kparts[i] <= kKSplitMaxParts);
+        VGAN_CHECK_ARG(kparts[i] == 1 || problems[i].splitk <= 1);
+        ksplit = ksplit || kparts[i] > 1;
+    }
+    if (ksplit) {
+        const int64_t need = ksplit_need(problems, count, kparts);
+        VGAN_CHECK_ARG(need > 0 && need < (1ll << 31) && ws != nullptr && aligned16(ws) && ws_bytes >= need);
+    }
     GroupedArgs g{};
     GroupedExtras x{};
     g.count = count;
@@ -333,15 +419,33 @@
         kmin = problems[i].k < kmin ? problems[i].k : kmin;
         t32 += ((problems[i].m + 31) / 32) * ((problems[i].n + 31) / 32);
     }
-    if (vec && kmin >= 96 && t32 <= 256 && !epi && x.noise_blocks == 0 && !any_split) {
-        int acc = 0;
+    const bool ks16 = vec && kmin >= 96 && t32 <= 256 && !epi && x.noise_blocks == 0 && !any_split;
+    VGAN_CHECK_ARG(!ksplit || ks16);
+    if (ks16) {
+        GroupedKSplit ks{};
+        int acc = 0, slots = 0, slab_bytes = 0;
         for (int i = 0; i < count; ++i) {
+            const int tiles_i = ((problems[i].m + 31) / 32) * ((problems[i].n + 31) / 32);
+            const int parts = ksplit ? kparts[i] : 1;
             g.ks[i] = 1;
             g.tile_start[i] = acc;
-            acc += ((problems[i].m + 31) / 32) * ((problems[i].n + 31) / 32);
+            acc += tiles_i * parts;
+            ks.parts[i] = parts;
+            if (parts > 1) {
+                ks.kchunk[i] = ksplit_kchunk(problems[i].k, parts, QKS);
+                ks.slot0[i] = slots;
+                ks.slab0[i] = slab_bytes;
+                slots += tiles_i;
+                slab_bytes += tiles_i * parts * kKSplitSlabBytes;
+            }
         }
         for (int i = count; i <= VGAN_GEMM_MAX_GROUP; ++i) g.tile_start[i] = acc;
-        hipLaunchKernelGGL(gemm_grouped_ks16_kernel, dim3(acc + surplus), dim3(1024), 0, (hipStream_t)stream, g, x);
+        if (ksplit) {
+            ks.ws = KSplitWs{reinterpret_cast<float*>(static_cast<char*>(ws) + ksplit_ticket_bytes(slots)), static_cast<int*>(ws), slab_bytes};
+            hipLaunchKernelGGL(gemm_grouped_ks16_split_kernel, dim3(acc + surplus), dim3(1024), 0, (hipStream_t)stream, g, x, ks);
+        } else {
+            hipLaunchKernelGGL(gemm_grouped_ks16_kernel, dim3(acc + surplus), dim3(1024), 0, (hipStream_t)stream, g, x);
+        }
         VGAN_CHECK_LAUNCH();
         return VGAN_OK;
     }
@@ -355,6 +459,21 @@
     return VGAN_OK;
 }
 
+extern "C" int vgan_gemm_grouped_ex(const vgan_gemm_problem* problems, int count, const vgan_grouped_extras* extras,
+                                    vgan_stream_t stream) {
+    return grouped_launch(problems, count, extras, nullptr, nullptr, 0, stream);
+}
+
+extern "C" int64_t vgan_gemm_grouped_ksplit_ws_bytes(const vgan_gemm_problem* problems, int count, const int32_t* kparts) {
+    const int64_t need = ksplit_need(problems, count, kparts);
+    return need < 0 ? 0 : need;
+}
+
+extern "C" int vgan_gemm_grouped_ksplit(const vgan_gemm_problem* problems, int count, const vgan_grouped_extras* extras,
+                                        const int32_t* kparts, void* ws, int64_t ws_bytes, vgan_stream_t stream) {
+    return grouped_launch(problems, count, extras, kparts, ws, ws_bytes, stream);
+}
+
 extern "C" int vgan_gemm_grouped(const vgan_gemm_problem* problems, int count, vgan_stream_t stream) {
     return vgan_gemm_grouped_ex(problems, count, nullptr, stream);
 }
diff --git a/v-gan_amd/csrc/linear.hip b/v-gan_amd/csrc/linear.hip
--- a/v-gan_amd/csrc/linear.hip
+++ b/v-gan_amd/csrc/linear.hip
@@ -122,6 +122,30 @@
     const int m0 = blockIdx.y * 32, n0 = blockIdx.x * 32;
     float o[G::NR];
     G::run(dy, lddy, x, ldx, m0, n0, out, in, n, lds, o);
+    const int col = n0 + G::col_of();
+#pragma unroll
+    for (int rr = 0; rr < G::NR; ++rr) {
+        const int row = m0 + G::row_of(rr);
+        if (row < out && col < in) dW[(long)row * lddw + col] = o[rr];
+    }
+}
+__global__ __launch_bounds__(1024, 1) void linear_bwd_params_ks_split_kernel(const float* __restrict__ dy, int lddy,
+                                                                            const float* __restrict__ x, int ldx, float* __restrict__ dW,
+                                                                            int lddw, int n, int in, int out, int kchunk, KSplitWs ws) {
+    using G = GemmTileKS<KSBK, MC, MC, 4, 16>;
+    __shared__ __attribute__((aligned(16))) float lds[G::kLdsFloats];
+    const int m0 = blockIdx.y * 32, n0 = blockIdx.x * 32;
+    const int part = blockIdx.z, parts = gridDim.z;
+    const int k0 = part * kchunk, klen = min(kchunk, n - k0);
+    float o[G::NR];
+    if (klen > 0) {
+        G::run(dy + (long)k0 * lddy, lddy, x + (long)k0 * ldx, ldx, m0, n0, out, in, klen, lds, o);
+    } else {
+#pragma unroll
+        for (int rr = 0; rr < G::NR; ++rr) o[rr] = 0.f;
+    }
+    const int tile = blockIdx.y * gridDim.x + blockIdx.x;
+    if (!ksplit_finish<G::NR, G::NTH>(o, ws, tile, tile * parts * kKSplitSlabBytes, part, parts, lds)) return;
     const int col = n0 + G::col_of();
 #pragma unroll
     for (int rr = 0; rr < G::NR; ++rr) {
@@ -248,6 +272,30 @@
     return VGAN_OK;
 }
 
+extern "C" int64_t vgan_linear_backward_params_ksplit_ws_bytes(int in, int out, int parts) {
+    if (in <= 0 || out <= 0 || parts <= 1 || parts > kKSplitMaxParts) return 0;
+    const long tiles = (long)((in + 31) / 32) * ((out + 31) / 32);
+    return ksplit_ticket_bytes(tiles) + tiles * parts * kKSplitSlabBytes;
+}
+
+extern "C" int vgan_linear_backward_params_ksplit(const float* dy, int lddy, const float* x, int ldx, float* dW, int lddw, int n, int in,
+                                                  int out, int parts, void* ws, int64_t ws_bytes, vgan_stream_t stream) {
+    VGAN_CHECK_ARG(parts >= 1 && parts <= kKSplitMaxParts);
+    if (parts == 1) return vgan_linear_backward_params(dy, lddy, x, ldx, 1, 0, dW, lddw, nullptr, n, in, out, 1, 0, stream);
+    VGAN_CHECK_ARG(dy && x && dW && n > 0 && in > 0 && out > 0 && lddy >= out && ldx >= in && lddw >= in);
+    VGAN_CHECK_ARG((out % 4 == 0) && (lddy % 4 == 0) && (in % 4 == 0) && (ldx % 4 == 0) && aligned16(dy) && aligned16(x));
+    const int64_t need = vgan_linear_backward_params_ksplit_ws_bytes(in, out, parts);
+    VGAN_CHECK_ARG(ws != nullptr && aligned16(ws) && ws_bytes >= need && need < (1ll << 31));
+    const int gx = (in + 31) / 32, gy = (out + 31) / 32;
+    VGAN_CHECK_ARG(gy <= 65535);
+    const long tb = ksplit_ticket_bytes((long)gx * gy);
+    const KSplitWs k{reinterpret_cast<float*>(static_cast<char*>(ws) + tb), static_cast<int*>(ws), (int)(need - tb)};
+    hipLaunchKernelGGL(linear_bwd_params_ks_split_kernel, dim3(gx, gy, parts), dim3(1024), 0, (hipStream_t)stream, dy, lddy, x, ldx, dW, lddw, n,
+                       in, out, ksplit_kchunk(n, parts, KSBK), k);
+    VGAN_CHECK_LAUNCH();
+    return VGAN_OK;
+}
+
 extern "C" int vgan_linear_backward_params_xx_supported(int n, int in, int out) {
     return (n >= 256 && in > 0 && out > 0 && in % 4 == 0 && out % 4 == 0 && use_ks(out, in, n)) ? 1 : 0;
 }
diff --git a/v-gan_amd/lib.py b/v-gan_amd/lib.py
--- a/v-gan_amd/lib.py
+++ b/v-gan_amd/lib.py
@@ -57,6 +57,8 @@
     "vgan_linear_forward": (_i, [_p, _i, _i, _i64, _p, _i, _p, _p, _i, _i, _i, _i, _p]),
     "vgan_linear_backward_input": (_i, [_p, _i, _p, _i, _p, _i, _i, _i, _i, _p]),
     "vgan_linear_backward_params": (_i, [_p, _i, _p, _i, _i, _i64, _p, _i, _p, _i, _i, _i, _i, _i64, _p]),
+    "vgan_linear_backward_params_ksplit_ws_bytes": (_i64, [_i, _i, _i]),
+    "vgan_linear_backward_params_ksplit": (_i, [_p, _i, _p, _i, _p, _i, _i, _i, _i, _i, _p, _i64, _p]),
     "vgan_linear_backward_params_xx_supported": (_i, [_i, _i, _i]),
     "vgan_linear_backward_params_xx": (_i, [_p, _i, _p, _i, _p, _i, _i, _i, _i, _p, _p]),
     "vgan_reduce_slabs": (_i, [_p, _i64, _i, _p, _i64, _p]),
@@ -95,6 +97,8 @@
     "vgan_adadelta_step_packed": (_i, [_p, _p, _p, _p, _p, _p, _i64, _f, _f, _f, _f, _f, _p, _i, _i, _i, _i, _u64, _p, _p]),
     "vgan_gemm_grouped": (_i, [_p, _i, _p]),
     "vgan_gemm_grouped_ex": (_i, [_p, _i, _p, _p]),
+    "vgan_gemm_grouped_ksplit_ws_bytes": (_i64, [_p, _i, _p]),
+    "vgan_gemm_grouped_ksplit": (_i, [_p, _i, _p, _p, _p, _i64, _p]),
     "vgan_mask_project_forward_bf3": (_i, [_p, _i, _p, _i, _p, _p, _i, _i, _p, _p, _i, _p, _p, _p, _i, _p, _p, _i, _i, _i, _p, _i, _p, _p, _p]),
     "vgan_mask_project_forward_bf3_ex": (_i, [_p, _i, _p, _i, _p, _p, _i, _i, _p, _p, _i, _p, _p, _p, _i, _p, _p, _i, _i, _i, _p, _i, _p, _p, _i, _p,
                                               _p]),
diff --git a/v-gan_amd/ops.py b/v-gan_amd/ops.py
--- a/v-gan_amd/ops.py
+++ b/v-gan_amd/ops.py
@@ -77,6 +77,21 @@
         _lib.check(self.lib.vgan_linear_backward_params(_ptr(dy), dy.stride(0), _ptr(x), x.stride(0), int(x_nslabs), int(x_slab_stride),
                                                         _ptr(dW), dW.stride(0), _ptr(db), n, kin, out, int(splits), int(slab_stride),
                                                         self._stream()), "vgan_linear_backward_params")
+
+    def linear_backward_params_ksplit_ws_bytes(self, kin, out, parts):
+        return int(self.lib.vgan_linear_backward_params_ksplit_ws_bytes(int(kin), int(out), int(parts)))
+
+    def ksplit_workspace(self, nbytes, device=None):
+        return torch.zeros(max(int(nbytes), 16) // 4 + 4, dtype=torch.int32, device=device or "cuda")
+
+    def linear_backward_params_ksplit(self, dy, x, dW, parts, ws):
+        _mat(dy, "dy"), _mat(x, "x"), _mat(dW, "dW")
+        n, out = dy.shape
+        kin = x.shape[1]
+        assert x.shape[0] == n and dW.shape == (out, kin)
+        _lib.check(self.lib.vgan_linear_backward_params_ksplit(_ptr(dy), dy.stride(0), _ptr(x), x.stride(0), _ptr(dW), dW.stride(0), n, kin, out,
+                                                               int(parts), _ptr(ws), 0 if ws is None else ws.numel() * ws.element_size(),
+                                                               self._stream()), "vgan_linear_backward_params_ksplit")
 
     def linear_backward_params_xx_supported(self, n, kin, out):
         return bool(self.lib.vgan_linear_backward_params_xx_supported(int(n), int(kin), int(out)))
@@ -127,6 +142,7 @@
                                                       ctypes.byref(chain) if chain is not None else None, self._stream()), "vgan_mask_project_forward")
 
     bf3_rebuild = True
+    chain_ksplit = True
 
     def xx_job(self, Dh, Dl, dsq, tiles, bw, partial):
         assert tiles.is_contiguous() and partial.is_contiguous() and Dh.stride(0) == Dl.stride(0)
@@ -365,8 +381,29 @@
     def mmd_backward_bf3_tile(self, nr, p, splits=1, tile=0):
         return int(self.lib.vgan_mmd_backward_bf3_tile(int(nr), int(p), int(splits), int(tile)))
 
-    def gemm_grouped(self, problems, copy=None, adadelta=None, noise=None, fold=None):
+    def gemm_grouped(self, problems, copy=None, adadelta=None, noise=None, fold=None, kparts=None, ksplit_ws=None):
         assert 1 <= len(problems) <= _lib.GEMM_MAX_GROUP
+        if kparts is not None and all(int(v) == 1 for v in kparts):
+            kparts = None
+        arr = self._gemm_problems(problems)
+        if kparts is None and copy is None and adadelta is None and noise is None and fold is None:
+            _lib.check(self.lib.vgan_gemm_grouped(arr, len(problems), self._stream()), "vgan_gemm_grouped")
+            return
+        x = self._grouped_extras(len(problems), copy, adadelta, noise, fold)
+        if kparts is not None:
+            assert len(kparts) == len(problems)
+            kp = (ctypes.c_int32 * len(problems))(*[int(v) for v in kparts])
+            _lib.check(self.lib.vgan_gemm_grouped_ksplit(arr, len(problems), ctypes.byref(x), kp, _ptr(ksplit_ws),
+                                                         0 if ksplit_ws is None else ksplit_ws.numel() * ksplit_ws.element_size(),
+                                                         self._stream()), "vgan_gemm_grouped_ksplit")
+            return
+        _lib.check(self.lib.vgan_gemm_grouped_ex(arr, len(problems), ctypes.byref(x), self._stream()), "vgan_gemm_grouped_ex")
+
+    def gemm_grouped_ksplit_ws_bytes(self, problems, kparts):
+        kp = (ctypes.c_int32 * len(problems))(*[int(v) for v in kparts])
+        return int(self.lib.vgan_gemm_grouped_ksplit_ws_bytes(self._gemm_problems(problems), len(problems), kp))
+
+    def _gemm_problems(self, problems):
         arr = (_lib.GemmProblem * len(problems))()
         for q, (kind, A, B, C, *rest) in zip(arr, problems):
             if kind == "NT2":
@@ -396,9 +433,9 @@
             assert k == k2 and tuple(C.shape) == (m, n), (kind, tuple(A.shape), tuple(B.shape), tuple(C.shape))
             q.a, q.b, q.c, q.kind, q.m, q.n, q.k = A.data_ptr(), B.data_ptr(), C.data_ptr(), code, m, n, k
             q.lda, q.ldb, q.ldc = A.stride(0), B.stride(0), C.stride(0)
-        if copy is None and adadelta is None and noise is None and fold is None:
-            _lib.check(self.lib.vgan_gemm_grouped(arr, len(problems), self._stream()), "vgan_gemm_grouped")
-            return
+        return arr
+
+    def _grouped_extras(self, nproblems, copy, adadelta, noise, fold):
         x = _lib.GroupedExtras()
         if copy is not None:
             src, dst = copy
@@ -413,7 +450,7 @@
             x.lr, x.rho, x.eps, x.weight_decay, x.grad_scale = (float(a["lr"]), float(a.get("rho", 0.9)), float(a.get("eps", 1e-6)),
                                                                 float(a.get("weight_decay", 0.0)), float(a.get("grad_scale", 1.0)))
             extra = a.get("extra_grad")
-            assert len(a["layers"]) == len(problems) + (1 if extra is not None else 0)
+            assert len(a["layers"]) == nproblems + (1 if extra is not None else 0)
             for L, (w, off_w, off_b, out, inp) in zip(x.layer, a["layers"]):
                 _mat(w, "w_packed")
                 L.w_packed, L.off_w, L.off_b, L.ldp, L.out, L.inp = w.data_ptr(), int(off_w), int(off_b), w.stride(0), int(out), int(inp)
@@ -427,7 +464,7 @@
             x.seed, x.step_counter = int(noise["seed"]) & 0xFFFFFFFFFFFFFFFF, noise["step_counter"].data_ptr()
         if fold is not None:
             x.fold = ctypes.addressof(fold)
-        _lib.check(self.lib.vgan_gemm_grouped_ex(arr, len(problems), ctypes.byref(x), self._stream()), "vgan_gemm_grouped_ex")
+        return x
 
     def mse_grad(self, target, pred, gscale, part, g):
         _mat(target, "target"), _mat(pred, "pred"), _mat(g, "g")
diff --git a/v-gan_amd/trainer.py b/v-gan_amd/trainer.py
--- a/v-gan_amd/trainer.py
+++ b/v-gan_amd/trainer.py
@@ -35,6 +35,20 @@
         if c < best_cost - 1e-9 and c <= cost(n_main) - 0.15:
             best, best_cost = k, c
     return best
+
+
+CHAIN_KPARTS_AUTO = 4
+
+
+def chain_kparts(want, tiles, k, chain_flops=False):
+    if want != "auto":
+        parts = int(want)
+        if parts not in (1, 2, 4, 8):
+            raise ValueError(f"VGAN_CHAIN_KPARTS must be auto, 1, 2, 4 or 8, got {want!r}")
+        return parts
+    if chain_flops or not (32 <= tiles <= 64 and k >= 768):
+        return 1
+    return CHAIN_KPARTS_AUTO
 
 
 class FlatParams:
@@ -280,6 +294,22 @@
             late = self.tiles.shape[0] - self.n_main
             bwd_wgs = ((d + 63) // 64) * ((nl + 63) // 64) * self.bsplits + 1
             self.xx_late_in_backward = (ops.mmd_backward_bf3_tile(nl, d, self.bsplits, self.bwd_tile) == 64 and late <= 512 - bwd_wgs)
+        self.m4_kparts = self.tn_kparts = 1
+        self.m4_ws = self.tn_ws = None
+        if self.mode == "collapsed" and getattr(ops, "chain_ksplit", False):
+            want_kp = os.environ.get("VGAN_CHAIN_KPARTS", "auto")
+            e = self.e
+            t32 = lambda rows, cols: ((rows + 31) // 32) * ((cols + 31) // 32)
+            if not (self.xx_in_m4 and not self.xx_late_in_backward):
+                self.m4_kparts = chain_kparts(want_kp, t32(dp, e[0]), nl, self.chain_flops)
+            tn_tiles = sum(t32(e[k], e[0]) for k in (3, 2, 1))
+            if not self.chain_flops and e[4] >= 96 and tn_tiles <= 256:
+                self.tn_kparts = chain_kparts(want_kp, tn_tiles, e[4])
+            if self.m4_kparts > 1:
+                self.m4_ws = ops.ksplit_workspace(ops.linear_backward_params_ksplit_ws_bytes(e[0], dp, self.m4_kparts), self.dev)
+            if self.tn_kparts > 1:
+                tn = [("TN", self.Wt[4], self.M[4], self.M[3]), ("TN", self.B3, self.M[4], self.M[2]), ("TN", self.B2, self.M[4], self.M[1])]
+                self.tn_ws = ops.ksplit_workspace(ops.gemm_grouped_ksplit_ws_bytes(tn, [self.tn_kparts] * 3), self.dev)
         plain_bf3 = (getattr(ops, "bf3_rebuild", False) and self.bf3 and self.fused_prepare and self.gram_tile == 64 and
                      self.rm_backward and world == 1 and not self.overlap and not self.front_sharded and
                      ops.mmd_backward_bf3_tile(nl, d, self.bsplits, self.bwd_tile) == 64)
@@ -486,6 +516,8 @@
         e, d = self.e, self.d
         if self.xx_in_m4 and not self.xx_late_in_backward:
             ops.linear_backward_params_xx(self.dlogits_pad, self.z_own, self.M[4][:self.dp], self._late_xx_job())
+        elif self.m4_kparts > 1:
+            ops.linear_backward_params_ksplit(self.dlogits_pad, self.z_own, self.M[4][:self.dp], self.m4_kparts, self.m4_ws)
         else:
             ops.linear_backward_params(self.dlogits_pad, self.z_own, self.M[4][:self.dp], None)
         if dist:
@@ -506,14 +538,15 @@
             ops.gemm_grouped([("NT", M[2], At[1], Gt[2])])
             ops.adadelta_step_packed(self.fp.flat, self.pmap, self.Gt_all, self.Wt_all, self.fp.sq, self.fp.acc, **adadelta, **fused_noise)
             return
+        tn_split = dict(kparts=[self.tn_kparts] * 3, ksplit_ws=self.tn_ws) if self.tn_kparts > 1 else {}
         if not self.fuse_update:
             ops.gemm_grouped([("TN", self.Wt[4], M[4], M[3]), ("TN", self.B3, M[4], M[2]), ("TN", self.B2, M[4], M[1])],
-                             fold=self._fold if self.xx_in_m4 else None)
+                             fold=self._fold if self.xx_in_m4 else None, **tn_split)
             ops.gemm_grouped([("NT", M[4], At[3], Gt[4]), ("NT", M[3], At[2], Gt[3]), ("NT", M[2], At[1], Gt[2])])
             ops.adadelta_step_packed(self.fp.flat, self.pmap, self.Gt_all, self.Wt_all, self.fp.sq, self.fp.acc, **adadelta, **fused_noise)
             return
         ops.gemm_grouped([("TN", self.Wt[4], M[4], M[3]), ("TN", self.B3, M[4], M[2]), ("TN", self.B2, M[4], M[1])],
-                         copy=(self.Wt[1], self.At1s), fold=self._fold if self.xx_in_m4 else None)
+                         copy=(self.Wt[1], self.At1s), fold=self._fold if self.xx_in_m4 else None, **tn_split)
         w, off = self.widths, self.fp.offsets
         layers = [(self.Wt[k], off[2 * (k - 1)], off[2 * (k - 1) + 1], w[k], w[k - 1]) for k in (4, 3, 2, 1)]
         ops.gemm_grouped([("NT", M[4], At[3], Gt[4]), ("NT", M[3], At[2], Gt[3]), ("NT", M[2], self.At1s, Gt[2])],
```

After: 10160 steps/s (median of 6 runs). 2.5% higher.
